# mightymightys/AttosecondRaytracing

Hardware: AMD Instinct MI355X
Metric: ray-surface intersections/s (higher is better)
Workload: dtype f64

## Files before the change

### attosecondraytracing_amd/ModuleProcessing.py

```python
import contextlib
import copy
import lzma
import os
import pickle
from datetime import datetime
from time import perf_counter

import numpy as np
import torch

from . import _abi
from . import _lib
from . import ModuleGeometry as mgeo
from . import ModuleMask as mmask
from . import ModuleOpticalElement as moe
from . import ModuleOpticalRay as mray
from . import ModuleSupport as msupp
from .bundle import RayBundle

DEFAULT_TRACE_MODE = os.environ.get("ART_TRACE_MODE", "chain")


_DESC_CACHE = {}
_DESC_F64_OFFSET = _abi.ArtElementDesc.fwd.offset
assert (_abi.ArtElementDesc.mp.offset - _DESC_F64_OFFSET) == 30 * 8 and _abi.ArtElementDesc.mp.size == 32


def element_descriptor(oe, IgnoreDefects=True, backend=None):
    key = (id(oe), bool(IgnoreDefects))
    h = hash(oe)
    hit = _DESC_CACHE.get(key)
    if hit is not None and hit[0] == h and hit[3] is oe:
        return hit[1], hit[2]
    d, keep = _build_descriptor(oe, IgnoreDefects, backend)
    if len(_DESC_CACHE) > 4096:
        _DESC_CACHE.clear()
    _DESC_CACHE[key] = (h, d, keep, oe)
    return d, keep


def _build_descriptor(oe, IgnoreDefects, backend):
    optic = oe.type
    kind = getattr(optic, "_abi_kind", None)
    tname = getattr(optic, "type", None)
    if kind is None or not isinstance(tname, str) or not ("Mirror" in tname or tname == "Mask"):
        raise NameError("I don`t recognize the type of optical element " + str(tname) + ".")
    d = _abi.ArtElementDesc()
    d.kind = int(kind)
    d.support_kind = int(optic.support._abi_kind)
    fwd, bwd = mgeo.frame_maps(oe.normal, oe.majoraxis)
    buf = np.frombuffer(d, dtype=np.float64, count=34, offset=_DESC_F64_OFFSET)
    buf[0:9] = fwd.reshape(9)
    buf[9:18] = bwd.reshape(9)
    buf[18:21] = oe.position
    buf[21:24] = optic.get_centre()
    sp = optic.support._abi_params()
    buf[24:24 + len(sp)] = sp
    mp_ = optic._abi_params()
    buf[30:30 + len(mp_)] = mp_
    d.nonfinite = bool(d.kind not in (_abi.ART_PLANE, _abi.ART_MASK)
                       and not (np.isfinite(buf[18:24]).all() and np.isfinite(buf[30:34]).all()))
    keep = None
    d.n_defects = 0
    d.n_grid = 0
    d.flags = 0
    d.zern = None
    d.grid = None
    d.grating = None
    if hasattr(optic, "lines_per_mm"):
        d.flags |= _abi.ART_FLAG_GRATING
        d.grating = optic
    if hasattr(optic, "DeformationList") and len(optic.DeformationList) > 0:
        be = backend or _lib.get_backend()
        keep = []
        zern, grids = optic._zernike_defects(), optic._grid_defects()
        if grids and not IgnoreDefects:
            grids[0].get_normal(None)
        if zern:
            table, n_tables, recurrence = optic._abi_defect_table()
            t = be.from_numpy(table)
            keep.append(t)
            d.zern = t.data_ptr()
            d.n_defects = n_tables
            if recurrence:
                d.flags |= _abi.ART_FLAG_ZERN_RECURRENCE
        if grids:
            arr = (_abi.ArtGridDefect * len(grids))()
            rect = np.asarray(optic.support._CircumRect(), dtype=float)
            for g, D in zip(arr, grids):
                half = np.array([max(abs(D._X[0]), abs(D._X[-1])), max(abs(D._Y[0]), abs(D._Y[-1]))])
                if (rect / 2 > half * (1 + 1e-12)).any():
                    raise ValueError(f"One of the requested xi is out of bounds: the mirror support ({rect[0]:g} x "
                                     f"{rect[1]:g} mm) is larger than the Fourrier map ({2 * half[0]:g} x {2 * half[1]:g} mm)")
                fields, dev = D._abi_grid(be)
                keep.append(dev)
                for k_, v_ in fields.items():
                    setattr(g, k_, v_)
            raw = np.frombuffer(bytes(arr), dtype=np.uint8).copy()
            t = be.from_numpy(raw)
            keep.append(t)
            d.grid = t.data_ptr()
            d.n_grid = len(grids)
        if not IgnoreDefects:
            d.flags |= _abi.ART_FLAG_PERTURBED_NORMAL
    return d, keep


def _as_bundle(rays, backend=None):
    if isinstance(rays, RayBundle):
        return rays
    return RayBundle.from_ray_list(rays, backend)


_CHAIN_MAX = 8
_STEPWISE_FLAGS = _abi.ART_FLAG_ZERN_RECURRENCE | _abi.ART_FLAG_GRATING


def _trace_one(be, desc, vin, vout, n, wavelength, grooves):
    if not desc.flags & _abi.ART_FLAG_GRATING:
        be.trace_element(desc, vin, vout, n)
        return grooves
    if wavelength is None:
        raise ValueError("tracing a Grating needs the wavelength of the ray bundle (RayBundle.wavelength is None)")
    G = desc.grating
    out = be.zeros(n)
    be.trace_grating(desc, G._groove_vector(), G.lines_per_mm, G.order, [wavelength], vin, [vout], n, grooves, out)
    return out


def _attach_readout(bundle, detector, path_centre, res):
    res.pop("bundle", None)
    bundle._fused_readout = (detector._readout_key(path_centre), bundle.version, res)


def _attach_sums(bundle, res):
    w = bundle.intensity
    bundle._fused_sums = (bundle.version, None if w is None else (w.data_ptr(), w._version), res)


def RayTracingCalculation(source_rays, optical_elements, IgnoreDefects=True, mode=None, history=True, detector=None,
                          path_centre=0.0, readout_lite=False, sums=False):
    if isinstance(history, str):
        if history != "lazy":
            raise ValueError("history must be True, False or 'lazy'")
        return LazyHistory(source_rays, optical_elements, IgnoreDefects, mode, detector, path_centre)
    src = _as_bundle(source_rays)
    be = src.backend
    n = src.n_slots
    m = len(optical_elements)
    if m == 0:
        return []
    descs, keep = [], []
    for oe in optical_elements:
        d, k = element_descriptor(oe, IgnoreDefects, be)
        descs.append(d)
        keep.append(k)
    mode = mode or DEFAULT_TRACE_MODE
    if any(d.flags & _STEPWISE_FLAGS for d in descs):
        mode = "element"
    bad = next((k for k, d in enumerate(descs) if d.nonfinite), None)
    if bad is not None:
        head = RayTracingCalculation(src, optical_elements[:bad], IgnoreDefects, mode, True) if bad else []
        if len(head[-1] if bad else src) > 0:
            raise np.linalg.LinAlgError("Array must not contain infs or NaNs")
        tail = RayBundle.allocate_many(n, m - bad, head[-1] if bad else src, be)
        prev = head[-1] if bad else src
        for b in tail:
            b.alive.zero_()
            b.parent = prev
            prev = b
        return (head + tail) if history else [None] * (m - 1) + [tail[-1]]
    if history:
        outs = RayBundle.allocate_many(n, m, src, be)
    else:
        outs = [None] * (m - 1) + [RayBundle.allocate(n, like=src, backend=be)]
    prev = src
    for b in outs:
        if b is not None:
            b.parent = prev
            b._keepalive = keep
            prev = b
    if mode == "chain":
        views = [b.view() if b is not None else _abi.ArtBundleView() for b in outs]
        if not history and m > _CHAIN_MAX:
            scratch = [RayBundle.allocate(n, like=src, backend=be) for _ in range(min(2, (m - 1) // _CHAIN_MAX))]
            for j, k in enumerate(range(_CHAIN_MAX - 1, m - 1, _CHAIN_MAX)):
                views[k] = scratch[j % len(scratch)].view()
            outs[-1]._keepalive = (keep, scratch)
        ro = None
        if detector is not None and 0 < n <= be.MAX_FUSED_READOUT_RAYS:
            detector._iscomplete()
            ro = be.new_chain_readout(detector._desc(), src.intensity, n, (0.0, 0.0, path_centre), lite=readout_lite)
        elif sums and detector is None and 0 < n <= be.MAX_FUSED_READOUT_RAYS and hasattr(be, "new_chain_sums"):
            ro = be.new_chain_sums(src.intensity, n)
        be.trace_chain(descs, src.view(), views, n, readout=ro)
        if ro is not None and ro.get("sums"):
            _attach_sums(outs[-1], ro)
        elif ro is not None:
            _attach_readout(outs[-1], detector, path_centre, ro)
    elif mode == "element":
        if not history and m > 1:
            cur = RayBundle.allocate(n, like=src, backend=be)
            g = _trace_one(be, descs[0], src.view(), cur.view(), n, src.wavelength, src.grooves)
            for k in range(1, m - 1):
                g = _trace_one(be, descs[k], cur.view(), cur.view(), n, src.wavelength, g)
            outs[-1].grooves = _trace_one(be, descs[m - 1], cur.view(), outs[-1].view(), n, src.wavelength, g)
        else:
            vin, g = src.view(), src.grooves
            for k in range(m):
                vout = outs[k].view()
                g = outs[k].grooves = _trace_one(be, descs[k], vin, vout, n, src.wavelength, g)
                vin = vout
    else:
        raise ValueError("mode must be 'chain' or 'element'")
    return outs


def RayTracingSpectral(source_rays, optical_elements, grating_index, Wavelengths, detector=None, IgnoreDefects=True):
    wls = [float(w) for w in np.atleast_1d(np.asarray(Wavelengths, dtype=float))]
    if not 1 <= len(wls) <= _abi.ART_GRATING_MAX_WAVELENGTHS:
        raise ValueError(f"Wavelengths: 1 to {_abi.ART_GRATING_MAX_WAVELENGTHS} values")
    if not all(np.isfinite(w) and w > 0 for w in wls):
        raise ValueError("Wavelengths must be finite and positive (mm)")
    src = _as_bundle(source_rays)
    be, n, k = src.backend, src.n_slots, int(grating_index)
    head = RayTracingCalculation(src, optical_elements[:k], IgnoreDefects, history=False)[-1] if k > 0 else src
    desc, _ = element_descriptor(optical_elements[k], IgnoreDefects, be)
    G = desc.grating
    if G is None:
        raise ValueError("RayTracingSpectral: the element at grating_index is no Grating")
    outs = [RayBundle.allocate(n, like=head, backend=be) for _ in wls]
    grooves = be.zeros(len(wls) * n).view(len(wls), n)
    keep = be.trace_grating(desc, G._groove_vector(), G.lines_per_mm, G.order, wls, head.view(), [b.view() for b in outs], n,
                            head.grooves, grooves)
    for j, b in enumerate(outs):
        b.parent, b._keepalive = head, keep
        b.wavelength, b.grooves = wls[j], grooves[j]
    tail = list(optical_elements[k + 1:])
    if not tail:
        return outs
    res = RayTracingCalculationMany(outs, [tail] * len(wls), IgnoreDefects, history=False,
                                    detectors=None if detector is None else [detector] * len(wls))
    return [r[-1] for r in res]


class _ParentResolver:
    __slots__ = ("hist", "bundle", "recipe")

    def __init__(self, hist, bundle):
        import weakref
        self.hist, self.bundle = weakref.ref(hist), weakref.ref(bundle)
        self.recipe = (hist._src, hist._els, hist._opts, hist._want, hist._scene_key)

    def __call__(self):
        h = self.hist()
        if h is None:
            b = self.bundle()
            if b is None:
                return
            src, els, (ign, mode, pc_), want, key = self.recipe
            h = LazyHistory(src, els, ign, mode, None, pc_, want, first=b)
            h._scene_key = key
        h._materialise()


class LazyHistory:

    def __init__(self, source, elements, IgnoreDefects=True, mode=None, detector=None, path_centre=0.0, want=-1, first=None):
        self._src, self._els = _as_bundle(source), list(elements)
        self._scene_key = (_hash_list_of_objects(self._els), hash(self._src))
        self._opts = (bool(IgnoreDefects), mode, path_centre)
        m = len(self._els)
        self._bundles = [None] * m
        self._full = m <= 1
        self.retraces = 0
        if m == 0:
            return
        self._want = want % m
        if first is None:
            first = RayTracingCalculation(self._src, self._els[:self._want + 1], IgnoreDefects, mode, False,
                                          detector if self._want == m - 1 else None, path_centre,
                                          sums=detector is None or self._want != m - 1)[-1]
        self._bundles[self._want] = first
        if not self._full:
            first._parent_resolver = _ParentResolver(self, first)

    def _materialise(self):
        if self._full:
            return
        if (_hash_list_of_objects(self._els), hash(self._src)) != self._scene_key:
            raise RuntimeError("lazy history: an optical element or the source bundle was modified after this history was "
                               "handed out; its remaining bundles can no longer be traced.  Ask for the full history "
                               "(get_output_rays() / history=True) before modifying the chain.")
        self._full = True
        ign, mode, pc_ = self._opts
        full = RayTracingCalculation(self._src, self._els, ign, mode, True, None, pc_)
        self.retraces += 1
        for k, b in enumerate(full):
            have = self._bundles[k]
            if have is None:
                self._bundles[k] = b
            else:
                live = b.alive.bool()
                if not (torch.equal(have.alive, b.alive)
                        and torch.equal(have.data[:, live].view(torch.int64), b.data[:, live].view(torch.int64))):
                    raise RuntimeError("lazy history: the re-trace differs from the bundle handed out earlier")
                have.parent = self._src if k == 0 else self._bundles[k - 1]
        for k in range(1, len(full)):
            if self._bundles[k] is full[k]:
                self._bundles[k].parent = self._bundles[k - 1]

    def __len__(self):
        return len(self._bundles)

    def __getitem__(self, i):
        if isinstance(i, slice):
            self._materialise()
            return self._bundles[i]
        m = len(self._bundles)
        if not -m <= i < m:
            raise IndexError("list index out of range")
        if self._bundles[i % m] is None:
            self._materialise()
        return self._bundles[i % m]

    def __iter__(self):
        self._materialise()
        return iter(self._bundles)

    def __getstate__(self):
        st = dict(self.__dict__)
        for b in st["_bundles"]:
            if b is not None and b._parent_resolver is not None:
                self._materialise()
                return dict(self.__dict__)
        return st


def RayTracingCalculationMany(source_rays_list, optical_elements_list, IgnoreDefects=True, history=True,
                              detectors=None, sums=False):
    with mgeo.frozen_hashes():
        return _RayTracingCalculationMany(source_rays_list, optical_elements_list, IgnoreDefects, history, detectors, sums)


def _RayTracingCalculationMany(source_rays_list, optical_elements_list, IgnoreDefects=True, history=True,
                               detectors=None, sums=False):
    sources = [_as_bundle(s) for s in source_rays_list]
    c = len(sources)
    if c != len(optical_elements_list):
        raise ValueError("need one element list per source bundle")
    if c == 0:
        return []
    m, n, be = len(optical_elements_list[0]), sources[0].n_slots, sources[0].backend
    descs, keep = [], []
    for els in optical_elements_list:
        for oe in els:
            d, k = element_descriptor(oe, IgnoreDefects, be)
            descs.append(d)
            keep.append(k)
    uniform = (m > 0 and n > 0 and all(len(els) == m for els in optical_elements_list)
               and all(s.n_slots == n and s.backend is be for s in sources) and not any(d.nonfinite for d in descs)
               and not any(d.flags & _STEPWISE_FLAGS for d in descs))
    if detectors is not None and len(detectors) != c:
        raise ValueError("need one detector per chain")
    if uniform and c > 1 and detectors is None and len({s.content_key() for s in sources}) == 1 \
            and sources[0].content_key()[0] != "bundle":
        L = 0
        while L < m and all(bytes(descs[ci * m + L]) == bytes(descs[L]) for ci in range(1, c)):
            L += 1
        if L > 0:
            head = RayTracingCalculation(sources[0], optical_elements_list[0][:L], IgnoreDefects, None, history,
                                         sums=sums and L == m)
            if L == m:
                return [list(head) for _ in range(c)]
            tails = RayTracingCalculationMany([head[-1]] * c, [els[L:] for els in optical_elements_list], IgnoreDefects,
                                              history, sums=sums)
            return [list(head) + t for t in tails]
    too_big = history and c * m * n * 65 > 4e9
    if c == 1 or not uniform or too_big:
        return [RayTracingCalculation(s, els, IgnoreDefects, None, history, None if detectors is None else detectors[k],
                                      sums=sums and detectors is None)
                for k, (s, els) in enumerate(zip(sources, optical_elements_list))]
    if history:
        grid = RayBundle.allocate_grid(n, c, m, sources, be)
    else:
        grid = [[None] * (m - 1) + [RayBundle.allocate(n, like=s, backend=be)] for s in sources]
    views, scratch = [], []
    for ci, outs in enumerate(grid):
        prev = sources[ci]
        for k, b in enumerate(outs):
            if b is None and (k + 1) % _CHAIN_MAX == 0:
                b = RayBundle.allocate(n, like=sources[ci], backend=be)
                scratch.append(b)
                views.append(b.view())
                continue
            if b is not None:
                b.parent = prev
                b._keepalive = (keep, scratch)
                prev = b
            views.append(b.view() if b is not None else _abi.ArtBundleView())
    ros = None
    if detectors is not None and n <= be.MAX_FUSED_READOUT_RAYS:
        areas = be.chain_readout_scratch(n, c)
        ros = []
        for d, s_, area in zip(detectors, sources, areas):
            d._iscomplete()
            ros.append(be.new_chain_readout(d._desc(), s_.intensity, n, scratch=area))
    elif sums and detectors is None and n <= be.MAX_FUSED_READOUT_RAYS and hasattr(be, "new_chain_sums"):
        ros = [be.new_chain_sums(s_.intensity, n, scratch=area) for s_, area in zip(sources, be.chain_readout_scratch(n, c))]
    host, dev = be.scene_alloc(c, m, transient=True)
    be.scene_pack(descs, [s.view() for s in sources], views, c, m, host, ros)
    be.scene_upload(host, dev)
    be.trace_scene(dev, host, n, segments=-(-m // 8))
    for ci, outs in enumerate(grid):
        outs[-1]._keepalive = (keep, scratch)
        if ros is not None and ros[ci].get("sums"):
            _attach_sums(outs[-1], ros[ci])
        elif ros is not None:
            _attach_readout(outs[-1], detectors[ci], 0.0, ros[ci])
    return grid


def _placement_source(SourceProperties, FirstOptic):
    from . import ModuleSource as msource

    Divergence = SourceProperties["Divergence"]
    SourceSize = SourceProperties["SourceSize"]
    RayNumber = SourceProperties["NumberRays"]
    Wavelength = SourceProperties["Wavelength"]
    SourcePosition = np.array([0, 0, 0])
    SourceDirection = np.array([1, 0, 0])
    if Divergence == 0:
        if SourceSize == 0:
            S0 = FirstOptic.support
            radius = 0.5 * min(S0.dimX, S0.dimY) if hasattr(S0, "dimX") else S0.radius
        else:
            radius = SourceSize / 2
        SourceRayList = msource.PlaneWaveDisk(SourcePosition, SourceDirection, radius, RayNumber,
                                              Wavelength=Wavelength)
    elif SourceSize == 0:
        SourceRayList = msource.PointSource(SourcePosition, SourceDirection, Divergence, RayNumber,
                                            Wavelength=Wavelength)
    else:
        SourceRayList = msource.ExtendedSource(SourcePosition, SourceDirection, SourceSize, Divergence, RayNumber,
                                               Wavelength=Wavelength)
    Source = msource.ApplyGaussianIntensityToRayList(SourceRayList, 1 / np.e ** 2)
    be = Source.backend
    if hasattr(be, "bundle_sums9") and Source.n_slots > 0:
        _attach_sums(Source, {"sums_dev": be.bundle_sums9(Source)})
    return Source


def _placeChains(SourceProperties, OpticsList, variants, Description):
    from . import ModuleOpticalChain as moc

    c = len(variants)
    Source = _placement_source(SourceProperties, OpticsList[0])
    be = Source.backend
    plain = not any(hasattr(O, "DeformationList") for O in OpticsList)
    guide_ctx = be.side_stream_context("guides") if (plain and hasattr(be, "side_stream_context")) else contextlib.nullcontext()
    with guide_ctx, mgeo.frozen_hashes():
        chains = _placeChainsOn(be, Source, OpticsList, variants, Description, c)
        if plain and hasattr(be, "side_stream_context"):
            torch.cuda.current_stream().synchronize()
    return chains


def _explain_lost_guide(one, element):
    G = element.type
    bare = moe.OpticalElement(G.Mirror, element.position, element.normal, element.majoraxis)
    hit = RayTracingCalculation(one, [bare])[-1]
    if len(hit) == 0:
        return
    u = one.data[3:6, 0].cpu().numpy()
    v = hit.data[3:6, 0].cpu().numpy()
    nrm = (u - v) / np.linalg.norm(u - v)
    fwd, _ = mgeo.frame_maps(element.normal, element.majoraxis)
    qx, qy = G._groove_vector()
    mlN = G.order * one.wavelength * G.lines_per_mm
    g = fwd.T @ (mlN * np.array([qx, qy, 0.0]))
    vt = (u - u.dot(nrm) * nrm) + (g - g.dot(nrm) * nrm)
    raise ValueError(f"Grating: the order m = {G.order} is evanescent for the guide ray at wavelength {one.wavelength:g} mm "
                     f"with {G.lines_per_mm:g} lines/mm: m*lambda*N = {mlN:.6g}, incidence "
                     f"{np.degrees(np.arccos(abs(u.dot(nrm)))):.6g} deg (sin = {np.sqrt(max(0.0, 1 - u.dot(nrm) ** 2)):.6g}), "
                     f"|v_t|^2 = {vt.dot(vt):.6g} > 1, so sqrt(1 - |v_t|^2) does not exist")


def _placeChainsOn(be, Source, OpticsList, variants, Description, c):
    from . import ModuleOpticalChain as moc
    plane_angles = [[np.deg2rad(a % 360) for a in v[2]] for v in variants]
    inc_angles = [[np.deg2rad(a % 360) for a in v[1]] for v in variants]
    centre = [np.array([0, 0, 0]) for _ in range(c)]
    central = [np.array([1, 0, 0]) for _ in range(c)]
    rot_axis = [np.array([0, 1, 0]) for _ in range(c)]
    elements = [[] for _ in range(c)]
    guides = be.from_numpy(np.tile(np.array([0.0, 0.0, 0.0, 1.0, 0.0, 0.0, 0.0, np.nan]), (c, 1)))
    guide_alive = be.from_numpy(np.ones(c, dtype=np.uint8))

    def advance(through, ready):
        descs = [d if d is not None else element_descriptor(oe, True, be)[0] for oe, d in zip(through, ready)]
        if any(d.nonfinite for d in descs):
            raise np.linalg.LinAlgError("Array must not contain infs or NaNs")
        slow = [j for j, d in enumerate(descs) if d.flags & _STEPWISE_FLAGS]
        if not slow:
            be.trace_guides(descs, guides, guide_alive)
            return
        host, al = guides.cpu().numpy(), guide_alive.cpu().numpy()
        for j in range(c):
            if not al[j]:
                continue
            one = RayBundle.from_arrays(host[j, 0:3], host[j, 3:6], wavelength=Source.wavelength, path0=host[j, 6], backend=be)
            out = RayTracingCalculation(one, [through[j]])[-1]
            if len(out) == 0:
                if descs[j].flags & _abi.ART_FLAG_GRATING:
                    _explain_lost_guide(one, through[j])
                al[j] = 0
            else:
                host[j] = out.data[:, 0].cpu().numpy()
        guides.copy_(be.from_numpy(host))
        guide_alive.copy_(be.from_numpy(al))

    optic_copies = [{} for _ in range(c)]
    open_mask = None
    for k, Optic in enumerate(OpticsList):
        if not ("Mirror" in Optic.type or Optic.type == "Mask"):
            raise NameError("I don`t recognize the type of optical element " + Optic.type + ".")
        convex = Optic.type in ("SphericalCX Mirror", "CylindricalCX Mirror")
        shareable = not hasattr(Optic, "DeformationList")
        groups, through, through_descs = {}, [], []
        for j in range(c):
            if convex:
                inc_angles[j][k] = np.pi - inc_angles[j][k]
            dist_ = variants[j][0][k]
            mine = optic_copies[j].get(id(Optic))
            if mine is None:
                mine = optic_copies[j][id(Optic)] = copy.deepcopy(Optic)
            key = (central[j].tobytes(), central[j].dtype.char, rot_axis[j].tobytes(), rot_axis[j].dtype.char, centre[j].tobytes(),
                   centre[j].dtype.char, type(dist_).__name__, float(dist_), plane_angles[j][k], inc_angles[j][k])
            g = groups.get(key)
            if g is None:
                ctr = central[j] * dist_ + centre[j]
                if abs(plane_angles[j][k] - np.pi) < 1e-10:
                    ra = -rot_axis[j]
                else:
                    ra = mgeo.RotationAroundAxis(central[j], -plane_angles[j][k], rot_axis[j])
                normal = mgeo.RotationAroundAxis(ra, -np.pi / 2 + inc_angles[j][k], mgeo._cross3(central[j], ra))
                major = mgeo._cross3(ra, normal)
                element = moe.OpticalElement(mine, ctr, normal, major)
                g = groups[key] = {"ctr": ctr, "ra": ra, "first": element, "desc": None, "guide": None}
                if Optic.type == "Mask":
                    if open_mask is None:
                        open_mask = mmask.Mask(msupp.SupportRoundHole(Radius=100, RadiusHole=100, CenterHoleX=0, CenterHoleY=0))
                    g["guide"] = moe.OpticalElement(open_mask, ctr, normal, major)
                if shareable:
                    d, keep = _build_descriptor(element, True, be)
                    g["desc"] = (hash(element), d, keep)
            else:
                element = moe.OpticalElement._like(g["first"], mine)
            centre[j], rot_axis[j] = g["ctr"], g["ra"]
            elements[j].append(element)
            if g["desc"] is not None:
                h, d, keep = g["desc"]
                if len(_DESC_CACHE) > 4096:
                    _DESC_CACHE.clear()
# ... 231 lines not shown
```

### attosecondraytracing_amd/ModuleSource.py

```python
import numpy as np


from . import _lib
from . import ModuleGeometry as mgeo
from .bundle import RayBundle

_EZ = np.array([0.0, 0.0, 1.0])


def _device_source(kind, size, S, Axis, n, n_total, Wavelength):
    be = _lib.get_backend()
    b = RayBundle.allocate(n, backend=be)
    b.wavelength = Wavelength
    b.number = None
    rot = mgeo.rotation_matrix(_EZ, np.asarray(Axis, dtype=float))
    be.make_source(kind, size, rot, np.asarray(S, dtype=float), 0, n, n_total, b.view())
    b.tag_content(("source", int(kind), float(size), np.asarray(S, dtype=float).tobytes(),
                   np.asarray(Axis, dtype=float).tobytes(), int(n), int(n_total), Wavelength))
    return b


def _Cone(Angle: float, NbRays: int, Wavelength=None):
    return _device_source(0, Angle, np.zeros(3), _EZ, NbRays, NbRays, Wavelength)


def PointSource(S, Axis, Divergence: float, NbRays: int, Wavelength=None):
    return _device_source(0, Divergence, S, Axis, NbRays, NbRays, Wavelength)


def PlaneWaveDisk(Centre, Axis, Radius: float, NbRays: int, Wavelength=None):
    return _device_source(1, Radius, Centre, Axis, NbRays - 1, NbRays, Wavelength)


def ExtendedSource(S, Axis, Diameter: float, Divergence: float, NbRays: int, Wavelength=None):
    n_src = min(max(30, int(250 * Diameter)), int(NbRays / 300))
    per = max(300, int(NbRays / n_src))
    be = _lib.get_backend()
    b = RayBundle.allocate(n_src * per, backend=be)
    b.wavelength = Wavelength
    b.number = None
    rot = mgeo.rotation_matrix(_EZ, np.asarray(Axis, dtype=float))
    be.make_extended_source(Diameter / 2, Divergence, n_src, per, rot, np.asarray(S, dtype=float), 0, n_src * per,
                            b.view())
    b.tag_content(("extended source", float(Diameter), float(Divergence), int(n_src), int(per),
                   np.asarray(S, dtype=float).tobytes(), np.asarray(Axis, dtype=float).tobytes(), Wavelength))
    b.rays_per_source = per
    return b


def PlaneWaveSquare(Centre, Axis, SideLength: float, NbRays: int, Wavelength=None):
    x = np.linspace(-SideLength / 2, SideLength / 2, int(np.sqrt(NbRays)))
    y = np.linspace(-SideLength / 2, SideLength / 2, int(np.sqrt(NbRays)))
    pts = [[0.0, 0.0, 0.0]]
    for i in x:
        for j in y:
            if abs(x) > 1e-4 and abs(y) > 1e-4:
                pts.append([i, j, 0.0])
    pts = np.asarray(pts, dtype=float)
    M = mgeo.rotation_matrix(_EZ, np.asarray(Axis, dtype=float))
    vec = np.tile(M @ _EZ, (len(pts), 1))
    b = RayBundle.from_arrays(pts @ M.T + np.asarray(Centre, dtype=float), vec, np.arange(len(pts)), None, Wavelength)
    return b


def ApplyGaussianIntensityToRayList(RayList, IntensityFraction=1 / np.e ** 2):
    if IntensityFraction >= 1 or IntensityFraction <= 0:
        print("When applying a Gaussian intensity profile to a ray list, the IntensityFraction should be between "
              "0 and 1! I'm setting it to 1/e^2.")
        IntensityFraction = 1 / np.e ** 2
    from . import ModuleProcessing as mp
    B = RayList if isinstance(RayList, RayBundle) else RayBundle.from_ray_list(RayList)
    before = B.content_key()
    if hasattr(B.backend, "gaussian_intensity_central") and B.n_slots > 0:
        B.intensity = B.backend.gaussian_intensity_central(B.view(), IntensityFraction, B.n_slots)
    else:
        axis = mp.FindCentralRay(B).vector
        B.intensity = B.backend.gaussian_intensity(B.view(), axis, IntensityFraction, B.n_slots)
    B.touch()
    if before[0] != "bundle":
        B.tag_content((before, "gaussian intensity", float(IntensityFraction)))
    return B
```

### attosecondraytracing_amd/_abi.py

```python
import ctypes as C

ART_ABI_VERSION = 14

ART_OK = 0
ART_ERR_BAD_ARG = -1
ART_ERR_UNSUPPORTED = -2
ART_ERR_HIP = -3
ART_ERR_NO_DEVICE = -4

ART_PLANE, ART_SPHERE, ART_PARABOLA, ART_TORUS, ART_ELLIPSOID, ART_CYLINDER, ART_MASK = range(7)
ART_SUP_ROUND, ART_SUP_ROUNDHOLE, ART_SUP_RECT, ART_SUP_RECTHOLE, ART_SUP_RECTRECTHOLE = range(5)

ART_FLAG_PERTURBED_NORMAL = 1
ART_FLAG_ZERN_RECURRENCE = 2
ART_FLAG_GRATING = 4
ART_ZERN_RECURRENCE_MAX_ORDER = 64

ART_ZERN_MAX_ORDER = 16
ART_ZERN_DIM = ART_ZERN_MAX_ORDER + 1
ART_ZERN_STRIDE = 2 + 3 * ART_ZERN_DIM * ART_ZERN_DIM
ART_MAX_DEFECTS = 16

c_double_p = C.POINTER(C.c_double)
c_uint8_p = C.POINTER(C.c_uint8)
# ... 120 lines not shown
        ("y0", C.c_double), ("dy", C.c_double),
        ("nx", C.c_int32), ("ny", C.c_int32),
        ("planes", C.c_int32),
        ("reserved", C.c_int32),
        ("shift", C.c_double * ART_FOCAL_MAX_PLANES),
    ]


ART_FOCAL_MAX_WAVENUMBERS = 1024


class ArtFocalSpectrumDesc(C.Structure):
    _fields_ = [
        ("f", ArtFocalDesc),
        ("dk", C.c_double),
        ("nk", C.c_int32),
        ("reserved", C.c_int32),
    ]


class ArtFocalChromaticDesc(C.Structure):
    _fields_ = [
        ("f", ArtFocalDesc),
        ("axis", C.c_double * 3),
        ("nk", C.c_int32),
        ("reserved", C.c_int32),
    ]


ART_WAVEFRONT_MAX_ORDER = 10
ART_WAVEFRONT_MAX_COLS = 68
ART_WAVEFRONT_DOUBLES = 2360


class ArtWavefrontJob(C.Structure):
    _fields_ = [
        ("det", ArtDetectorDesc),
        ("b", ArtBundleView),
        ("w", C.c_void_p),
        ("n", C.c_int64),
        ("ref", C.c_double * 3),
        ("L_ref", C.c_double),
        ("pupil", C.c_double * 3),
        ("order", C.c_int32),
        ("reserved", C.c_int32),
        ("opd", C.c_void_p),
        ("pupil_x", C.c_void_p),
        ("pupil_y", C.c_void_p),
        ("out", C.c_void_p),
    ]


ART_COATING_MAX_LAYERS = 256
ART_COATING_MAX_MATERIALS = 6
ART_POLARISATION_MAX_ELEMS = 64
ART_POLARISATION_DOUBLES = 16


class ArtCoatingMaterial(C.Structure):
    _fields_ = [("n", C.c_double), ("kappa", C.c_double)]


class ArtCoatingLayer(C.Structure):
    _fields_ = [("thickness", C.c_double), ("roughness", C.c_double), ("material", C.c_int32), ("reserved", C.c_int32)]


class ArtCoating(C.Structure):
    _fields_ = [
        ("ideal", C.c_int32),
        ("n_materials", C.c_int32),
        ("n_layers", C.c_int32),
        ("substrate", C.c_int32),
        ("roughness", C.c_double),
        ("reserved", C.c_double),
        ("materials", ArtCoatingMaterial * ART_COATING_MAX_MATERIALS),
        ("layers", ArtCoatingLayer * ART_COATING_MAX_LAYERS),
    ]


class ArtPolarisationJob(C.Structure):
    _fields_ = [
        ("views", C.c_void_p),
        ("coating", C.c_int32 * ART_POLARISATION_MAX_ELEMS),
        ("n_elems", C.c_int32),
        ("polarised", C.c_int32),
        ("n", C.c_int64),
        ("pol", C.c_double * 6),
        ("k", C.c_double),
        ("has_det", C.c_int32),
        ("reserved", C.c_int32),
        ("det", ArtDetectorDesc),
        ("w0", C.c_void_p),
        ("w", C.c_void_p),
        ("w_out", C.c_void_p),
        ("field", C.c_void_p),
        ("out", C.c_void_p),
    ]


ART_FOCAL_VECTOR_SCRATCH_DEFAULT = 1 << 29


class ArtFocalVectorSpectrumDesc(C.Structure):
    _fields_ = [
        ("s", ArtFocalSpectrumDesc),
        ("views", C.c_void_p),
        ("coating", C.c_int32 * ART_POLARISATION_MAX_ELEMS),
        ("n_elems", C.c_int32),
        ("n_coatings", C.c_int32),
        ("n", C.c_int64),
        ("pol", C.c_double * 6),
        ("w", C.c_void_p),
        ("materials", C.c_void_p),
        ("scratch_bound", C.c_int64),
    ]


class ArtFocalVectorChromaticDesc(C.Structure):
    _fields_ = [
        ("v", ArtFocalVectorSpectrumDesc),
        ("axis", C.c_double * 3),
    ]


ART_FOCAL_MAX_GROUPS = 1 << 20


class ArtFocalImageDesc(C.Structure):
    _fields_ = [
        ("f", ArtFocalDesc),
        ("groups", C.c_int32),
        ("reserved", C.c_int32),
        ("seg", C.c_void_p),
    ]


PROTOTYPES = {
    "art_abi_version": (C.c_int, []),
    "art_last_error": (C.c_char_p, []),
    "art_device_count": (C.c_int, []),
    "art_trace_element": (C.c_int, [C.POINTER(ArtElementDesc), C.POINTER(ArtBundleView), C.POINTER(ArtBundleView),
                                    C.c_int64, C.c_void_p]),
    "art_trace_grating": (C.c_int, [C.POINTER(ArtElementDesc), C.POINTER(ArtGratingDesc), c_double_p,
                                    C.POINTER(ArtBundleView), C.POINTER(ArtBundleView), C.c_int64, C.c_void_p]),
    "art_trace_chain": (C.c_int, [C.POINTER(ArtElementDesc), C.c_int32, C.POINTER(ArtBundleView),
                                  C.POINTER(ArtBundleView), C.c_int64, C.c_void_p]),
    "art_scene_bytes": (C.c_int64, [C.c_int32, C.c_int32]),
    "art_chain_readout_scratch_doubles": (C.c_int64, [C.c_int64]),
    "art_trace_chain_readout": (C.c_int, [C.POINTER(ArtElementDesc), C.c_int32, C.POINTER(ArtBundleView),
                                          C.POINTER(ArtBundleView), C.POINTER(ArtChainReadout), C.c_int64, C.c_void_p]),
    "art_scene_pack": (C.c_int, [C.POINTER(ArtElementDesc), C.c_int32, C.c_int32, C.POINTER(ArtBundleView),
                                 C.POINTER(ArtBundleView), C.POINTER(ArtChainReadout), C.c_void_p]),
    "art_trace_scene": (C.c_int, [C.c_void_p, C.c_void_p, C.c_int64, C.c_void_p]),
    "art_pack_rays": (C.c_int, [C.c_void_p, C.c_void_p, C.c_void_p, C.c_int64, C.POINTER(ArtBundleView), C.c_void_p]),
    "art_transform_bundle": (C.c_int, [c_double_p, c_double_p, C.c_int32, C.POINTER(ArtBundleView),
                                       C.POINTER(ArtBundleView), C.c_int64, C.c_void_p]),
    "art_detector": (C.c_int, [C.POINTER(ArtDetectorDesc), C.POINTER(ArtBundleView), C.c_int64, C.c_void_p,
                               C.c_void_p, C.c_void_p, C.c_void_p, C.c_void_p, C.c_void_p, C.c_void_p]),
    "art_detector_readout": (C.c_int, [C.POINTER(ArtDetectorDesc), C.POINTER(ArtBundleView), C.c_void_p, C.c_int64,
                                       C.c_double, C.c_double, C.c_double] + [C.c_void_p] * 9),
    "art_detector_scan_moments": (C.c_int, [C.POINTER(ArtDetectorDesc), C.POINTER(ArtBundleView), C.c_void_p,
                                            C.c_int64, C.c_double, C.c_double, C.c_void_p, C.c_void_p,
                                            C.c_void_p]),
    "art_histogram": (C.c_int, [C.POINTER(ArtHistogramDesc), C.POINTER(ArtBundleView), C.c_void_p, C.c_int64, C.c_int32,
                                C.c_void_p, C.c_void_p, C.c_void_p, C.c_void_p]),
    "art_focal_scratch_doubles": (C.c_int64, [C.c_int32, C.c_int32, C.c_int32, C.c_int64]),
    "art_focal_field": (C.c_int, [C.POINTER(ArtFocalDesc), C.POINTER(ArtBundleView), C.c_void_p, C.c_int64, C.c_void_p,
                                  C.c_void_p, C.c_void_p]),
    "art_focal_spectrum_scratch_doubles": (C.c_int64, [C.c_int32, C.c_int32, C.c_int32, C.c_int32, C.c_int64]),
    "art_focal_spectrum": (C.c_int, [C.POINTER(ArtFocalSpectrumDesc), C.POINTER(ArtBundleView), C.c_void_p, C.c_int64,
                                     C.c_void_p, C.c_void_p, C.c_void_p]),
    "art_focal_chromatic_scratch_doubles": (C.c_int64, [C.c_int32, C.c_int32, C.c_int32, C.c_int32, C.c_int64]),
    "art_focal_chromatic": (C.c_int, [C.POINTER(ArtFocalChromaticDesc), C.POINTER(ArtBundleView), C.POINTER(ArtBundleView),
                                      C.c_void_p, C.c_int64, C.c_void_p, c_double_p, C.c_void_p, C.c_void_p, C.c_void_p]),
    "art_wavefront_scratch_doubles": (C.c_int64, [C.POINTER(ArtWavefrontJob), C.c_int32]),
    "art_wavefront": (C.c_int, [C.c_void_p, C.POINTER(ArtWavefrontJob), C.c_int32, C.c_void_p, C.c_void_p]),
    "art_polarisation_scratch_doubles": (C.c_int64, [C.POINTER(ArtPolarisationJob), C.c_int32]),
    "art_polarisation": (C.c_int, [C.c_void_p, C.POINTER(ArtPolarisationJob), C.c_int32, C.c_void_p,
                                   C.POINTER(ArtCoating), C.c_int32, C.c_void_p, C.c_void_p]),
    "art_focal_vector_spectrum_scratch_doubles": (C.c_int64, [C.POINTER(ArtFocalVectorSpectrumDesc)]),
    "art_focal_vector_spectrum": (C.c_int, [C.POINTER(ArtFocalVectorSpectrumDesc), C.POINTER(ArtBundleView), C.c_void_p,
                                            C.POINTER(ArtCoating), C.POINTER(ArtCoatingMaterial), C.c_void_p,
                                            C.c_void_p, C.c_void_p]),
    "art_focal_vector_chromatic_scratch_doubles": (C.c_int64, [C.POINTER(ArtFocalVectorChromaticDesc)]),
    "art_focal_vector_chromatic": (C.c_int, [C.POINTER(ArtFocalVectorChromaticDesc), C.POINTER(ArtBundleView),
                                             C.POINTER(ArtBundleView), C.c_void_p, C.POINTER(ArtCoating),
                                             C.POINTER(ArtCoatingMaterial), C.c_void_p, c_double_p, C.c_void_p,
                                             C.c_void_p, C.c_void_p]),
    "art_focal_image_scratch_doubles": (C.c_int64, [C.c_int32, C.c_int32, C.c_int32, C.c_int32, C.c_int64]),
    "art_focal_image": (C.c_int, [C.POINTER(ArtFocalImageDesc), C.POINTER(ArtBundleView), C.c_void_p, C.c_int64,
                                  C.c_void_p, C.c_void_p, C.c_void_p]),
    "art_reduce_scratch_doubles": (C.c_int64, []),
    "art_detector_stats": (C.c_int, [C.c_void_p, C.c_void_p, C.c_void_p, C.c_void_p, C.c_void_p, C.c_int64,
                                     C.c_void_p, C.c_void_p, C.c_void_p]),
    "art_detector_moments": (C.c_int, [C.c_void_p, C.c_void_p, C.c_void_p, C.c_void_p, C.c_void_p, C.c_int64,
                                       C.c_double, C.c_double, C.c_double, C.c_void_p, C.c_void_p, C.c_void_p]),
    "art_bundle_sums": (C.c_int, [C.POINTER(ArtBundleView), C.c_void_p, C.c_int64, C.c_void_p, C.c_void_p,
                                  C.c_void_p]),
    "art_gaussian_intensity": (C.c_int, [C.POINTER(ArtBundleView), c_double_p, C.c_double, C.c_int64, C.c_void_p,
                                         C.c_void_p, C.c_void_p]),
    "art_gaussian_intensity_central": (C.c_int, [C.POINTER(ArtBundleView), C.c_double, C.c_int64, C.c_void_p, C.c_void_p,
                                                 C.c_void_p, C.c_void_p]),
    "art_bundle_max_angle": (C.c_int, [C.POINTER(ArtBundleView), c_double_p, C.c_int64, C.c_void_p, C.c_void_p,
                                       C.c_void_p]),
    "art_compact_scratch_ints": (C.c_int64, [C.c_int64]),
    "art_compact": (C.c_int, [C.c_void_p, C.c_int64, C.c_void_p, C.c_void_p, C.c_void_p, C.c_void_p]),
    "art_make_source": (C.c_int, [C.c_int32, C.c_double, c_double_p, c_double_p, C.c_int64, C.c_int64, C.c_int64,
                                  C.POINTER(ArtBundleView), C.c_void_p]),
    "art_make_source_strided": (C.c_int, [C.c_int32, C.c_double, c_double_p, c_double_p, C.c_int64, C.c_int64, C.c_int64,
                                          C.c_int64, C.POINTER(ArtBundleView), C.c_void_p]),
    "art_exchange_pack": (C.c_int, [C.c_void_p] * 6 + [C.c_int64, C.c_void_p, C.c_void_p]),
    "art_exchange_fold": (C.c_int, [C.c_void_p, C.c_int32, C.c_int64, C.c_void_p, C.c_void_p]),
    "art_survivor_bytes": (C.c_int64, [C.c_int64, C.c_int32]),
    "art_pack_survivors": (C.c_int, [C.c_void_p, C.c_int64] + [C.c_void_p] * 4 + [C.c_int64, C.c_int64, C.c_void_p,
                                                                                    C.c_void_p, C.c_int64, C.c_void_p]),
    "art_survivor_finish": (C.c_int, [C.c_void_p, C.c_int64, C.c_void_p, C.c_void_p, C.c_void_p]),
    "art_survivor_xheader": (C.c_int, [C.c_void_p, C.c_void_p, C.c_void_p, C.c_void_p]),
    "art_trace_guides": (C.c_int, [C.POINTER(ArtElementDesc), C.c_int32, C.c_void_p, C.c_void_p, C.c_void_p]),
    "art_analysis_scratch_doubles": (C.c_int64, [C.c_int32, C.c_int64]),
    "art_analyse_bundles": (C.c_int, [C.c_void_p, C.POINTER(ArtAnalysisJob), C.c_int32, C.c_int64, C.c_void_p, C.c_void_p,
                                      C.c_void_p]),
    "art_make_extended_source": (C.c_int, [C.c_double, C.c_double, C.c_int64, C.c_int64, c_double_p, c_double_p,
                                           C.c_int64, C.c_int64, C.POINTER(ArtBundleView), C.c_void_p]),
}


def bind(lib, prefix="art_"):
    fns = {}
    for name, (res, args) in PROTOTYPES.items():
        sym = name if prefix == "art_" else prefix + name[len("art_"):]
        f = getattr(lib, sym)
        f.restype = res
        f.argtypes = args
        fns[name] = f
    return fns
```

### attosecondraytracing_amd/_lib.py

```python
import ctypes as C
import os

import numpy as np
import torch

from . import _abi

_HERE = os.path.dirname(os.path.abspath(__file__))
LIB_PATH = os.path.join(_HERE, "libart_hip.so")

_BACKEND = None


class ArtError(RuntimeError):
    pass


class HipBackend:

    name = "hip"

    def __init__(self, path=LIB_PATH):
        if not os.path.exists(path):
            raise RuntimeError(
                f"{path} not found: the HIP extension has not been built. Run "
                "`python -c 'import __graft_entry__ as g; g.build()'` (needs hipcc). There is no CPU fallback.")
        self.lib = C.CDLL(path)
        self.fn = _abi.bind(self.lib)
        v = self.fn["art_abi_version"]()
        if v != _abi.ART_ABI_VERSION:
            raise RuntimeError(f"libart_hip.so ABI version {v} != expected {_abi.ART_ABI_VERSION}: rebuild it")
        if not torch.cuda.is_available():
            raise RuntimeError("No HIP device visible to PyTorch: ray tracing needs an MI355X (gfx950). "
                               "There is no CPU fallback.")
        n = self.fn["art_device_count"]()
        if n <= 0:
            raise RuntimeError("libart_hip.so found no gfx950 device (art_device_count() = %d: %s)"
                               % (n, self.last_error()))
        self.device = torch.device("cuda", torch.cuda.current_device())
        self._scratch = {}
        self._side_streams = {}
        self._scene_pool, self._scene_uploads = {}, {}
        self._job_pool = {}
        self.count_from, self.counted_launches = None, 0
        self.trace_events = None
        self.readout_events = None

    def last_error(self):
        return self.fn["art_last_error"]().decode("utf-8", "replace")

    def check(self, rc, what):
        if rc != 0:
            raise ArtError(f"{what} failed with code {rc}: {self.last_error()}")

    def stream_ptr(self):
        return C.c_void_p(torch.cuda.current_stream(self.device).cuda_stream)

    def synchronize(self):
        torch.cuda.current_stream(self.device).synchronize()

    def empty(self, n, dtype=torch.float64):
        return torch.empty(int(n), dtype=dtype, device=self.device)

    def zeros(self, n, dtype=torch.float64):
        return torch.zeros(int(n), dtype=dtype, device=self.device)

    def from_numpy(self, a, dtype=None):
        t = torch.from_numpy(np.ascontiguousarray(a))
        if dtype is not None:
            t = t.to(dtype)
        return t.to(self.device)

    def stream_key(self):
        return torch.cuda.current_stream(self.device).cuda_stream

    def side_stream_context(self, name):
        st = self._side_streams.get(name)
        if st is None:
            st = self._side_streams[name] = torch.cuda.Stream(device=self.device)
        return torch.cuda.stream(st)

    def scratch(self, key, n, dtype):
        key = (key, self.stream_key())
        t = self._scratch.get(key)
        if t is None or t.numel() < n or t.dtype != dtype:
            t = torch.empty(int(max(n, 1)), dtype=dtype, device=self.device)
            self._scratch[key] = t
        return t

    def _timed(self, call, sink="trace_events"):
        events = getattr(self, sink)
        if events is None:
            return call()
        e0, e1 = torch.cuda.Event(enable_timing=True), torch.cuda.Event(enable_timing=True)
        e0.record()
        rc = call()
        e1.record()
        events.append((e0, e1))
        return rc

    def trace_element(self, desc, view_in, view_out, n):
        sp = self.stream_ptr()
        self.check(self._timed(lambda: self.fn["art_trace_element"](C.byref(desc), C.byref(view_in),
                                                                    C.byref(view_out), n, sp)), "art_trace_element")

    def trace_grating(self, desc, q, lines_per_mm, order, wavelengths, view_in, views_out, n, grooves_in=None,
                      grooves_out=None):
        nw = len(wavelengths)
        wl_host = (C.c_double * nw)(*[float(w) for w in wavelengths])
        varr = (_abi.ArtBundleView * nw)(*views_out)
        wl_dev = self.from_numpy(np.array([float(w) for w in wavelengths], dtype=np.float64))
        v_dev = self.from_numpy(np.frombuffer(bytes(varr), dtype=np.uint8).copy())
        g = _abi.ArtGratingDesc()
        g.q[0], g.q[1] = float(q[0]), float(q[1])
        g.lines_per_mm, g.order, g.nw = float(lines_per_mm), int(order), nw
        g.wavelengths, g.outs = wl_dev.data_ptr(), v_dev.data_ptr()
        g.grooves_in = None if grooves_in is None else grooves_in.data_ptr()
        g.grooves_out = None if grooves_out is None else grooves_out.data_ptr()
        sp = self.stream_ptr()
        self.check(self._timed(lambda: self.fn["art_trace_grating"](C.byref(desc), C.byref(g), wl_host, varr,
                                                                    C.byref(view_in), n, sp)), "art_trace_grating")
        return wl_dev, v_dev

    def trace_chain(self, descs, view_in, views_out, n, readout=None):
        m = len(descs)
        if m > 1 or readout is not None:
            self.note_launches(n, -(-m // 8))
        darr = (_abi.ArtElementDesc * m)(*descs)
        varr = (_abi.ArtBundleView * m)(*views_out)
        sp = self.stream_ptr()
        if readout is None:
            self.check(self._timed(lambda: self.fn["art_trace_chain"](darr, m, C.byref(view_in), varr, n, sp)),
                       "art_trace_chain")
        else:
            ro = readout["struct"]
            self.check(self._timed(lambda: self.fn["art_trace_chain_readout"](darr, m, C.byref(view_in), varr,
                                                                              C.byref(ro), n, sp)),
                       "art_trace_chain_readout")

    MAX_FUSED_READOUT_RAYS = 1 << 28

    def new_chain_readout(self, ddesc, w, n, centres=(0.0, 0.0, 0.0), store=True, scratch=None, lite=False, targets=None):
        X = Y = opl = None
        if targets is not None:
            X, Y, opl = targets
            assert all(t.numel() >= n and t.dtype == torch.float64 and t.is_contiguous() for t in (X, Y, opl))
            store = True
        elif store:
            X, Y, opl = self.empty(n), self.empty(n), self.empty(n)
        out = self.empty(24)
        if scratch is None:
            scratch = self.scratch("chain_ro", self.fn["art_chain_readout_scratch_doubles"](n), torch.float64)
        ro = _abi.ArtChainReadout()
        ro.det = ddesc
        ro.w = None if w is None else w.data_ptr()
        ro.cx, ro.cy, ro.co = (float(v) for v in centres)
        ro.X, ro.Y, ro.opl = (None, None, None) if not store else (X.data_ptr(), Y.data_ptr(), opl.data_ptr())
        ro.scratch, ro.out24 = scratch.data_ptr(), out.data_ptr()
        ro.lite = 1 if lite else 0
        ro.sums = 0
        return {"struct": ro, "X": X, "Y": Y, "opl": opl, "P3": None, "stats_dev": out, "_keep": (w, scratch), "lite": bool(lite)}

    def new_chain_sums(self, w, n, scratch=None):
        out = self.empty(24)
        if scratch is None:
            scratch = self.scratch("chain_ro", self.fn["art_chain_readout_scratch_doubles"](n), torch.float64)
        ro = _abi.ArtChainReadout()
        ro.w = None if w is None else w.data_ptr()
        ro.X = ro.Y = ro.opl = None
        ro.scratch, ro.out24 = scratch.data_ptr(), out.data_ptr()
        ro.lite, ro.sums = 0, 1
        return {"struct": ro, "sums_dev": out, "_keep": (w, scratch), "sums": True}

    def chain_readout_scratch(self, n, count):
        per = int(self.fn["art_chain_readout_scratch_doubles"](n))
        t = torch.empty(per * count, dtype=torch.float64, device=self.device)
        return [t[k * per:(k + 1) * per] for k in range(count)]

    def scene_alloc(self, n_chains, n_elems, transient=False):
        nb = int(self.fn["art_scene_bytes"](n_chains, n_elems))
        if nb <= 0:
            raise ArtError("art_scene_bytes: bad chain or element count")
        if transient:
            pkey = (nb, self.stream_key())
            pair = self._scene_pool.get(pkey)
            if pair is None:
                pair = self._scene_pool[pkey] = (torch.empty(nb, dtype=torch.uint8, pin_memory=True),
                                                 torch.empty(nb, dtype=torch.uint8, device=self.device))
            ev = self._scene_uploads.pop(pair[0].data_ptr(), None)
            if ev is not None:
                ev.synchronize()
            return pair
        return (torch.empty(nb, dtype=torch.uint8, pin_memory=True),
                torch.empty(nb, dtype=torch.uint8, device=self.device))

    def scene_pack(self, descs, views_in, views_out, n_chains, n_elems, host_image, readouts=None):
        darr = (_abi.ArtElementDesc * (n_chains * n_elems))(*descs)
        iarr = (_abi.ArtBundleView * n_chains)(*views_in)
        oarr = (_abi.ArtBundleView * (n_chains * n_elems))(*views_out)
        rarr = None if readouts is None else (_abi.ArtChainReadout * n_chains)(*[r["struct"] for r in readouts])
        rc = self.fn["art_scene_pack"](darr, n_chains, n_elems, iarr, oarr, rarr, host_image.data_ptr())
        if rc < 0:
            self.check(rc, "art_scene_pack")
        return rc

    def scene_upload(self, host_image, dev_image):
        dev_image.copy_(host_image, non_blocking=True)
        ev = torch.cuda.Event()
        ev.record()
        self._scene_uploads[host_image.data_ptr()] = ev
        return ev

    def note_launches(self, n, k=1):
        if self.count_from is not None and n >= self.count_from:
            self.counted_launches += k

    def trace_scene(self, dev_image, host_image, n, segments=1):
        self.note_launches(n, segments)
        sp = self.stream_ptr()
        self.check(self._timed(lambda: self.fn["art_trace_scene"](dev_image.data_ptr(), host_image.data_ptr(), n, sp)),
                   "art_trace_scene")

    def pack_rays(self, points, vectors, path0, n, view):
        self.check(self.fn["art_pack_rays"](points.data_ptr(), vectors.data_ptr(),
                                            None if path0 is None else path0.data_ptr(), n, C.byref(view),
                                            self.stream_ptr()), "art_pack_rays")

    def transform_bundle(self, M, T, rotate_points, view_in, view_out, n):
        m = (C.c_double * 9)(*[float(v) for v in np.asarray(M).reshape(9)])
        t = (C.c_double * 3)(*[float(v) for v in np.asarray(T).reshape(3)])
        self.check(self.fn["art_transform_bundle"](m, t, int(bool(rotate_points)), C.byref(view_in), C.byref(view_out),
                                                   n, self.stream_ptr()), "art_transform_bundle")

    def detector(self, ddesc, view, n, p3=None, XY=None, opl=None):
        p = [t.data_ptr() for t in p3] if p3 is not None else [None, None, None]
        xy = [t.data_ptr() for t in XY] if XY is not None else [None, None]
        o = opl.data_ptr() if opl is not None else None
        self.check(self.fn["art_detector"](C.byref(ddesc), C.byref(view), n, p[0], p[1], p[2], xy[0], xy[1], o,
                                           self.stream_ptr()), "art_detector")

    def detector_readout(self, ddesc, view, w, n, centres=(0.0, 0.0, 0.0), p3=None, XY=None, opl=None, to_host=True):
        out = self.empty(24)
        p = [t.data_ptr() for t in p3] if (p3 is not None and n > 0) else [None, None, None]
        xy = [t.data_ptr() for t in XY] if (XY is not None and n > 0) else [None, None]
        sp, scratch = self.stream_ptr(), self._red_scratch()
        self.check(self._timed(lambda: self.fn["art_detector_readout"](
            C.byref(ddesc), C.byref(view), None if (w is None or n == 0) else w.data_ptr(), n, float(centres[0]),
            float(centres[1]), float(centres[2]), p[0], p[1], p[2], xy[0], xy[1],
            None if (opl is None or n == 0) else opl.data_ptr(), scratch.data_ptr(), out.data_ptr(), sp),
            "readout_events"), "art_detector_readout")
        return out.cpu().numpy() if to_host else out

    def detector_scan_moments(self, ddesc, view, w, n, co, span=0.0):
        if n == 0:
            return np.zeros(33)
        out = self.empty(33)
        self.check(self.fn["art_detector_scan_moments"](C.byref(ddesc), C.byref(view),
                                                        None if w is None else w.data_ptr(), n, float(co), float(span),
                                                        self._red_scratch().data_ptr(), out.data_ptr(),
                                                        self.stream_ptr()), "art_detector_scan_moments")
        return out.cpu().numpy()

    def histogram(self, hdesc, view, w, n, out=None, shift=None):
        from . import histogram as hist
        if shift is None:
            shift = hist.weight_shift(n, None if w is None else w[:n])
        hdesc.wshift = int(shift)
        if out is None:
            nbins = int(np.prod([hdesc.bins[k] for k in range(max(1, min(3, hdesc.ndim)))]))
            out = (self.empty(nbins, torch.int64), None if w is None else self.empty(nbins, torch.int64),
                   self.empty(4, torch.int64))
            accumulate = 0
        else:
            accumulate = 1
        counts, wsums, totals = out
        self.check(self.fn["art_histogram"](C.byref(hdesc), C.byref(view), None if (w is None or n == 0) else w.data_ptr(),
                                            n, accumulate, counts.data_ptr(), None if wsums is None else wsums.data_ptr(),
                                            totals.data_ptr(), self.stream_ptr()), "art_histogram")
        return counts, wsums, totals, shift

    def focal_field(self, fdesc, view, w, n):
        field = torch.empty((fdesc.planes, fdesc.ny, fdesc.nx), dtype=torch.complex128, device=self.device)
        ns = self.fn["art_focal_scratch_doubles"](fdesc.nx, fdesc.ny, fdesc.planes, n)
        if ns < 0:
            raise ArtError(f"art_focal_scratch_doubles failed with code {ns}: {self.last_error()}")
        scratch = self.scratch("focal", ns, torch.float64)
        self.check(self.fn["art_focal_field"](C.byref(fdesc), C.byref(view), None if (w is None or n == 0) else w.data_ptr(),
                                              n, scratch.data_ptr(), field.data_ptr(), self.stream_ptr()),
                   "art_focal_field")
        return field

    def focal_spectrum(self, sdesc, view, w, n):
        f = sdesc.f
        field = torch.empty((f.planes, sdesc.nk, f.ny, f.nx), dtype=torch.complex128, device=self.device)
        ns = self.fn["art_focal_spectrum_scratch_doubles"](f.nx, f.ny, f.planes, sdesc.nk, n)
        if ns < 0:
            raise ArtError(f"art_focal_spectrum_scratch_doubles failed with code {ns}: {self.last_error()}")
        scratch = self.scratch("focal", ns, torch.float64)
        self.check(self.fn["art_focal_spectrum"](C.byref(sdesc), C.byref(view), None if (w is None or n == 0) else
                                                 w.data_ptr(), n, scratch.data_ptr(), field.data_ptr(),
                                                 self.stream_ptr()), "art_focal_spectrum")
        return field

    def focal_chromatic(self, desc, final_view, source_view, w, n, table):
        table = np.ascontiguousarray(table, dtype=np.float64)
        if table.ndim != 2 or table.shape[1] != 4:
            raise ValueError("the chromatic table must have rows (k_j, c_j, z_j, 0)")
        f = desc.f
        desc.nk = nk = int(table.shape[0])
        ns = self.fn["art_focal_chromatic_scratch_doubles"](f.nx, f.ny, f.planes, nk, n)
        if ns < 0:
            raise ArtError(f"art_focal_chromatic_scratch_doubles failed with code {ns}: {self.last_error()}")
        field = torch.empty((f.planes, nk, f.ny, f.nx), dtype=torch.complex128, device=self.device)
        scratch = self.scratch("focal", ns, torch.float64)
        table_dev = self.from_numpy(table)
        self.check(self.fn["art_focal_chromatic"](C.byref(desc), C.byref(final_view), C.byref(source_view),
                                                  None if (w is None or n == 0) else w.data_ptr(), n,
                                                  table_dev.data_ptr(), table.ctypes.data_as(_abi.c_double_p),
                                                  scratch.data_ptr(), field.data_ptr(), self.stream_ptr()),
                   "art_focal_chromatic")
        return field

    def focal_image(self, fdesc, seg, groups, view, w, n):
        d = _abi.ArtFocalImageDesc()
        d.f = fdesc
        d.groups = int(groups)
        d.seg = seg.data_ptr()
        image = torch.empty((fdesc.planes, fdesc.ny, fdesc.nx), dtype=torch.float64, device=self.device)
        ns = self.fn["art_focal_image_scratch_doubles"](fdesc.nx, fdesc.ny, fdesc.planes, d.groups, n)
        if ns < 0:
            raise ArtError(f"art_focal_image_scratch_doubles failed with code {ns}: {self.last_error()}")
        scratch = self.scratch("focal", ns, torch.float64)
        self.check(self.fn["art_focal_image"](C.byref(d), C.byref(view), None if (w is None or n == 0) else w.data_ptr(),
                                              n, scratch.data_ptr(), image.data_ptr(), self.stream_ptr()),
                   "art_focal_image")
        return image

    def _red_scratch(self):
        return self.scratch("red", self.fn["art_reduce_scratch_doubles"](), torch.float64)

    def detector_stats(self, alive, X, Y, opl, w, n, to_host=True):
        out = self.empty(16)
        ptr = lambda t: None if (t is None or n == 0) else t.data_ptr()
        if n == 0:
            alive = self.zeros(1, torch.uint8)
        self.check(self.fn["art_detector_stats"](alive.data_ptr(), ptr(X), ptr(Y), ptr(opl), ptr(w), n,
                                                 self._red_scratch().data_ptr(), out.data_ptr(), self.stream_ptr()),
                   "art_detector_stats")
        return out.cpu().numpy() if to_host else out

    def detector_moments(self, alive, X, Y, opl, w, n, cx, cy, co):
        if n == 0:
            return np.zeros(8)
        out = self.empty(8)
        ptr = lambda t: None if t is None else t.data_ptr()
        self.check(self.fn["art_detector_moments"](alive.data_ptr(), ptr(X), ptr(Y), ptr(opl), ptr(w), n,
                                                   float(cx), float(cy), float(co), self._red_scratch().data_ptr(),
                                                   out.data_ptr(), self.stream_ptr()), "art_detector_moments")
        return out.cpu().numpy()

    def bundle_sums(self, view, w, n):
        if n == 0:
            return np.zeros(8)
        out = self.empty(8)
        self.check(self.fn["art_bundle_sums"](C.byref(view), None if w is None else w.data_ptr(), n,
                                              self._red_scratch().data_ptr(), out.data_ptr(), self.stream_ptr()),
                   "art_bundle_sums")
        return out.cpu().numpy()

    def gaussian_intensity(self, view, axis, fraction, n):
        w = self.empty(n)
        a = (C.c_double * 3)(*[float(v) for v in axis])
        self.check(self.fn["art_gaussian_intensity"](C.byref(view), a, float(fraction), n,
                                                     self._red_scratch().data_ptr(), w.data_ptr(), self.stream_ptr()),
                   "art_gaussian_intensity")
        return w

    def gaussian_intensity_central(self, view, fraction, n):
        w = self.empty(n)
        sums8 = self.empty(8)
        self.check(self.fn["art_gaussian_intensity_central"](C.byref(view), float(fraction), n, self._red_scratch().data_ptr(),
                                                             sums8.data_ptr(), w.data_ptr(), self.stream_ptr()),
                   "art_gaussian_intensity_central")
        return w

    def bundle_max_angle(self, view, axis, n):
        if n == 0:
            return 0.0, 0.0
        out = self.empty(2)
        a = (C.c_double * 3)(*[float(v) for v in axis])
        self.check(self.fn["art_bundle_max_angle"](C.byref(view), a, n, self._red_scratch().data_ptr(),
                                                   out.data_ptr(), self.stream_ptr()), "art_bundle_max_angle")
        o = out.cpu().numpy()
        return float(o[0]), float(o[1])

    def compact(self, alive, n):
        if n == 0:
            return torch.empty(0, dtype=torch.int64, device=self.device), 0
        ints = self.fn["art_compact_scratch_ints"](n)
        sc = self.scratch("compact", ints, torch.int32)
        idx = torch.empty(int(max(n, 1)), dtype=torch.int64, device=self.device)
        cnt = torch.zeros(1, dtype=torch.int64, device=self.device)
        self.check(self.fn["art_compact"](alive.data_ptr(), n, sc.data_ptr(), idx.data_ptr(), cnt.data_ptr(),
                                          self.stream_ptr()), "art_compact")
        c = int(cnt.cpu().item())
        return idx[:c], c

    def make_source(self, kind, size, rot, S, first, n, n_total, view, step=1):
        r = (C.c_double * 9)(*[float(v) for v in np.asarray(rot).reshape(9)])
        s = (C.c_double * 3)(*[float(v) for v in np.asarray(S).reshape(3)])
        self.check(self.fn["art_make_source_strided"](kind, float(size), r, s, first, int(step), n, n_total, C.byref(view),
                                                      self.stream_ptr()), "art_make_source_strided")

    def exchange_pack(self, stats, X, Y, opl, alive, slots, send):
        k = int(slots.numel())
        self.check(self.fn["art_exchange_pack"](stats.data_ptr(), X.data_ptr(), Y.data_ptr(), opl.data_ptr(),
                                                alive.data_ptr(), slots.data_ptr(), k, send.data_ptr(),
                                                self.stream_ptr()), "art_exchange_pack")

    def exchange_fold(self, recv, world, stride, out):
        self.check(self.fn["art_exchange_fold"](recv.data_ptr(), int(world), int(stride), out.data_ptr(),
                                                self.stream_ptr()), "art_exchange_fold")

    def survivor_bytes(self, count, dense=False):
        return int(self.fn["art_survivor_bytes"](int(count), 1 if dense else 0))

    def pack_survivors(self, alive, X, Y, opl, number, first, step, send):
        n = int(alive.numel())
        sc = self.scratch("compact", self.fn["art_compact_scratch_ints"](n), torch.int32)
        ptr = lambda t: None if (t is None or n == 0) else t.data_ptr()
        self.check(self.fn["art_pack_survivors"](ptr(alive), n, ptr(X), ptr(Y), ptr(opl), ptr(number), int(first),
                                                 int(step), sc.data_ptr(), send.data_ptr(), int(send.numel()),
                                                 self.stream_ptr()), "art_pack_survivors")

    def survivor_finish(self, stats_dev, n, send, xhdr=None):
        self.check(self.fn["art_survivor_finish"](stats_dev.data_ptr(), int(n), send.data_ptr(),
                                                  None if xhdr is None else xhdr.data_ptr(), self.stream_ptr()),
                   "art_survivor_finish")

    def survivor_xheader(self, send, stats_dev, xhdr):
        self.check(self.fn["art_survivor_xheader"](send.data_ptr(), None if stats_dev is None else stats_dev.data_ptr(),
                                                   xhdr.data_ptr(), self.stream_ptr()), "art_survivor_xheader")

    def trace_guides(self, descs, rays, alive):
        count = len(descs)
        sp = self.stream_ptr()
        for k0 in range(0, count, _abi.ART_GUIDES_MAX):
            m = min(_abi.ART_GUIDES_MAX, count - k0)
            darr = (_abi.ArtElementDesc * m)(*descs[k0:k0 + m])
            self.check(self.fn["art_trace_guides"](darr, m, rays.data_ptr() + 64 * k0, alive.data_ptr() + k0, sp),
                       "art_trace_guides")

    def _upload_table(self, arr, purpose=None):
        nb = C.sizeof(arr)
        pkey = (nb, self.stream_key()) if purpose is None else (purpose, nb, self.stream_key())
        pair = self._job_pool.get(pkey)
        if pair is None:
            pair = self._job_pool[pkey] = [torch.empty(nb, dtype=torch.uint8, pin_memory=True),
                                           torch.empty(nb, dtype=torch.uint8, device=self.device), None]
        host, dev, ev = pair
        if ev is not None:
            ev.synchronize()
        C.memmove(host.data_ptr(), C.addressof(arr), nb)
        dev.copy_(host, non_blocking=True)
        pair[2] = torch.cuda.Event()
        pair[2].record()
        return dev

    def wavefront(self, jobs):
        c = len(jobs)
        out = torch.empty((c, _abi.ART_WAVEFRONT_DOUBLES), dtype=torch.float64, device=self.device)
        for k, j in enumerate(jobs):
            j.out = out.data_ptr() + 8 * _abi.ART_WAVEFRONT_DOUBLES * k
        arr = (_abi.ArtWavefrontJob * c)(*jobs)
        ns = self.fn["art_wavefront_scratch_doubles"](arr, c)
        if ns < 0:
            raise ArtError(f"art_wavefront_scratch_doubles failed with code {ns}: {self.last_error()}")
        dev = self._upload_table(arr)
        scratch = self.scratch("wavefront", ns, torch.float64)
        self.check(self.fn["art_wavefront"](dev.data_ptr(), arr, c, scratch.data_ptr(), self.stream_ptr()), "art_wavefront")
        return out

    def polarisation(self, jobs, views, coatings):
        c = len(jobs)
        out = torch.empty((c, _abi.ART_POLARISATION_DOUBLES), dtype=torch.float64, device=self.device)
        blob = b"".join(bytes(v) for v in views) + b"".join(bytes(k) for k in coatings)
        dev = self._upload_table((C.c_char * len(blob)).from_buffer_copy(blob), "polarisation views")
        off = 0
        jarr = (_abi.ArtPolarisationJob * c)()
        for k, (j, v) in enumerate(zip(jobs, views)):
            jarr[k] = j
            jarr[k].views = dev.data_ptr() + off
            jarr[k].out = out.data_ptr() + 8 * _abi.ART_POLARISATION_DOUBLES * k
            off += C.sizeof(v)
        carr = (_abi.ArtCoating * max(len(coatings), 1))(*coatings)
        cdev = dev.data_ptr() + off if coatings else None
        ns = self.fn["art_polarisation_scratch_doubles"](jarr, c)
        if ns < 0:
            raise ArtError(f"art_polarisation_scratch_doubles failed with code {ns}: {self.last_error()}")
        jdev = self._upload_table(jarr)
        scratch = self.scratch("polarisation", ns, torch.float64)
        self.check(self.fn["art_polarisation"](jdev.data_ptr(), jarr, c, cdev, carr, len(coatings), scratch.data_ptr(),
                                               self.stream_ptr()), "art_polarisation")
        return out

    def focal_vector_tables(self, vdesc, views, coatings, materials):
        nk, nc = vdesc.s.nk, len(coatings)
        mats = np.ascontiguousarray(materials, dtype=np.float64)
        if mats.shape != (nk, nc, _abi.ART_COATING_MAX_MATERIALS, 2):
            raise ValueError(f"materials must be [nk, coatings, {_abi.ART_COATING_MAX_MATERIALS}, 2]")
        blob = bytes(views) + b"".join(bytes(k) for k in coatings) + mats.tobytes()
        dev = self._upload_table((C.c_char * len(blob)).from_buffer_copy(blob), "focal vector spectrum")
        vdesc.views = dev.data_ptr()
        vdesc.n_coatings = nc
        cdev = dev.data_ptr() + C.sizeof(views) if nc else None
        vdesc.materials = dev.data_ptr() + C.sizeof(views) + nc * C.sizeof(_abi.ArtCoating) if nc else None
        carr = (_abi.ArtCoating * max(nc, 1))(*coatings)
        marr = (_abi.ArtCoatingMaterial * max(mats.size // 2, 1)).from_buffer_copy(mats.tobytes() or bytes(16))
        return cdev, carr, marr

    def focal_vector_spectrum(self, vdesc, views, coatings, materials):
        f = vdesc.s.f
        field = torch.empty((f.planes, vdesc.s.nk, 3, f.ny, f.nx), dtype=torch.complex128, device=self.device)
        cdev, carr, marr = self.focal_vector_tables(vdesc, views, coatings, materials)
        ns = self.fn["art_focal_vector_spectrum_scratch_doubles"](C.byref(vdesc))
        if ns < 0:
            raise ArtError(f"art_focal_vector_spectrum_scratch_doubles failed with code {ns}: {self.last_error()}")
        scratch = self.scratch("focal vector", ns, torch.float64)
        self.check(self.fn["art_focal_vector_spectrum"](C.byref(vdesc), C.byref(views[vdesc.n_elems]), cdev, carr, marr,
                                                        scratch.data_ptr(), field.data_ptr(), self.stream_ptr()),
                   "art_focal_vector_spectrum")
        return field

    def focal_vector_chromatic(self, vcdesc, views, coatings, materials, table):
        table = np.ascontiguousarray(table, dtype=np.float64)
        if table.ndim != 2 or table.shape[1] != 4:
            raise ValueError("the chromatic table must have rows (k_j, c_j, z_j, 0)")
        v = vcdesc.v
        v.s.nk = nk = int(table.shape[0])
        f = v.s.f
        cdev, carr, marr = self.focal_vector_tables(v, views, coatings, materials)
        ns = self.fn["art_focal_vector_chromatic_scratch_doubles"](C.byref(vcdesc))
        if ns < 0:
            raise ArtError(f"art_focal_vector_chromatic_scratch_doubles failed with code {ns}: {self.last_error()}")
        field = torch.empty((f.planes, nk, 3, f.ny, f.nx), dtype=torch.complex128, device=self.device)
        scratch = self.scratch("focal vector", ns, torch.float64)
        table_dev = self.from_numpy(table)
        self.check(self.fn["art_focal_vector_chromatic"](C.byref(vcdesc), C.byref(views[v.n_elems]), C.byref(views[0]),
                                                         cdev, carr, marr, table_dev.data_ptr(),
                                                         table.ctypes.data_as(_abi.c_double_p), scratch.data_ptr(),
                                                         field.data_ptr(), self.stream_ptr()),
                   "art_focal_vector_chromatic")
        return field

    def analyse_bundles(self, jobs, n):
        c = len(jobs)
        arr = (_abi.ArtAnalysisJob * c)(*jobs)
        dev = self._upload_table(arr)
        out = torch.empty((c, _abi.ART_ANALYSIS_DOUBLES), dtype=torch.float64, device=self.device)
        scratch = self.scratch("analysis", self.fn["art_analysis_scratch_doubles"](c, int(n)), torch.float64)
        self.check(self.fn["art_analyse_bundles"](dev.data_ptr(), arr, c, int(n), scratch.data_ptr(), out.data_ptr(),
                                                  self.stream_ptr()), "art_analyse_bundles")
        return out

    def bundle_sums9(self, bundle):
        j = _abi.ArtAnalysisJob()
        j.b = bundle.view()
        j.w = None if bundle.intensity is None else bundle.intensity.data_ptr()
        j.mode = _abi.ART_JOB_SUMS
        return self.analyse_bundles([j], bundle.n_slots)[0]

    def make_extended_source(self, radius, divergence, n_points, per, rot, S, first, n, view):
        r = (C.c_double * 9)(*[float(v) for v in np.asarray(rot).reshape(9)])
        s = (C.c_double * 3)(*[float(v) for v in np.asarray(S).reshape(3)])
        self.check(self.fn["art_make_extended_source"](float(radius), float(divergence), int(n_points), int(per), r, s,
                                                       first, n, C.byref(view), self.stream_ptr()),
                   "art_make_extended_source")


def get_backend():
    global _BACKEND
    if _BACKEND is None:
        _BACKEND = HipBackend()
    return _BACKEND
```

### attosecondraytracing_amd/bundle.py

```python

import os

import numpy as np
import torch

from . import _abi
from . import _lib
from .ModuleOpticalRay import Ray

import itertools

ROW_OX, ROW_OY, ROW_OZ, ROW_DX, ROW_DY, ROW_DZ, ROW_PATH, ROW_INC = range(8)
_SERIAL = itertools.count(1)


class RayBundle:
    def __init__(self, data, alive, number=None, intensity=None, wavelength=None, parent=None, backend=None, grooves=None):
        self.data = data
        self.alive = alive
        self.number = number
        self.intensity = intensity
        self.wavelength = wavelength
        self.grooves = grooves
        self._parent = parent
        self._parent_resolver = None
        self._backend = backend or _lib.get_backend()
        self._index = None
        self._count = None
        self.version = 0
        self._serial = next(_SERIAL)
        self.path_head = None
        self._fused_readout = None
        self._fused_sums = None
        self._content = None

    @property
    def parent(self):
        if self._parent_resolver is not None:
            resolve, self._parent_resolver = self._parent_resolver, None
            resolve()
        return self._parent

    @parent.setter
    def parent(self, value):
        self._parent = value
        self._parent_resolver = None

    def fused_sums(self):
        fs = getattr(self, "_fused_sums", None)
        if fs is None or fs[0] != self.version:
            return None
        w = self.intensity
        if (None if w is None else (w.data_ptr(), w._version)) != fs[1]:
            return None
        return fs[2]["sums_dev"]

    def _share_parent(self, other):
        if self._parent_resolver is not None:
            import weakref
            wo = weakref.ref(other)

            def resolve(s=self, wo=wo):
                o = wo()
                if o is not None:
                    o._parent = s.parent
            other._parent_resolver = resolve

    @property
    def backend(self):
        if self._backend is None:
            be = _lib.get_backend()
            data, alive = self._rows(self.alive.numel(), be.device)
            data.copy_(self.data)
            alive.copy_(self.alive)
            self.data, self.alive = data, alive
            self.number = None if self.number is None else self.number.to(be.device)
            self.intensity = None if self.intensity is None else self.intensity.to(be.device)
            self.grooves = None if self.grooves is None else self.grooves.to(be.device)
            self._backend = be
        return self._backend

    def __getstate__(self):
        host = lambda t: None if t is None else t.detach().cpu().numpy()
        return {"data": host(self.data), "alive": host(self.alive), "number": host(self.number),
                "intensity": host(self.intensity), "wavelength": self.wavelength, "parent": self.parent,
                "version": self.version, "path_head": self.path_head, "grooves": host(self.grooves)}

    def __setstate__(self, st):
        t = lambda a: None if a is None else torch.from_numpy(np.ascontiguousarray(a))
        self.data, self.alive = t(st["data"]), t(st["alive"])
        self.number, self.intensity = t(st["number"]), t(st["intensity"])
        self._parent_resolver = None
        self.wavelength, self.parent, self.version = st["wavelength"], st["parent"], st["version"]
        self.path_head = st.get("path_head")
        self.grooves = t(st.get("grooves"))
        self._backend = None
        self._index = None
        self._count = None
        self._fused_readout = None
        self._fused_sums = None
        self._content = None
        self._serial = next(_SERIAL)

    @staticmethod
    def _pitch(n, unit=64):
        return max(unit, -(-int(n) // unit) * unit) + unit * int(os.environ.get("ART_PITCH_EXTRA", "0"))

    @classmethod
    def _rows(cls, n, device, count=None):
        n = int(n)
        pd, pa = cls._pitch(n), cls._pitch(n, 512)
        if count is None:
            return (torch.empty((8, pd), dtype=torch.float64, device=device)[:, :n],
                    torch.empty(pa, dtype=torch.uint8, device=device)[:n])
        lead = tuple(count) if isinstance(count, (tuple, list)) else (count,)
        return (torch.empty(lead + (8, pd), dtype=torch.float64, device=device)[..., :n],
                torch.empty(lead + (pa,), dtype=torch.uint8, device=device)[..., :n])

    @classmethod
    def allocate(cls, n, like=None, backend=None):
        be = backend or (like.backend if like is not None else _lib.get_backend())
        data, alive = cls._rows(n, be.device)
        if like is not None:
            return cls(data, alive, like.number, like.intensity, like.wavelength, like, be, like.grooves)
        return cls(data, alive, backend=be)

    @classmethod
    def allocate_many(cls, n, count, like, backend=None):
        be = backend or like.backend
        data, alive = cls._rows(n, be.device, count)
        return [cls(data[k], alive[k], like.number, like.intensity, like.wavelength, like, be, like.grooves)
                for k in range(count)]

    @classmethod
    def allocate_grid(cls, n, chains, count, likes, backend=None):
        be = backend or likes[0].backend
        data, alive = cls._rows(n, be.device, (chains, count))
        return [[cls(data[c, k], alive[c, k], likes[c].number, likes[c].intensity, likes[c].wavelength, likes[c], be,
                     likes[c].grooves)
                 for k in range(count)] for c in range(chains)]

    @classmethod
    def from_arrays(cls, point, vector, number=None, intensity=None, wavelength=None, path0=None, backend=None):
        be = backend or _lib.get_backend()
        point = np.ascontiguousarray(point, dtype=np.float64).reshape(-1, 3)
        vector = np.ascontiguousarray(vector, dtype=np.float64).reshape(-1, 3)
        n = point.shape[0]
        b = cls.allocate(n, backend=be)
        if n > 0:
            p0 = None
            if path0 is not None:
                p0 = be.from_numpy(np.broadcast_to(np.asarray(path0, dtype=np.float64), (n,)).copy())
            be.pack_rays(be.from_numpy(point), be.from_numpy(vector), p0, n, b.view())
        b.number = None if number is None else be.from_numpy(np.asarray(number, dtype=np.int64))
        b.intensity = None if intensity is None else be.from_numpy(np.asarray(intensity, dtype=np.float64))
        b.wavelength = wavelength
        return b

    @classmethod
    def from_ray_list(cls, rays, backend=None):
        rays = list(rays)
        pts = np.array([r.point for r in rays], dtype=np.float64).reshape(-1, 3)
        vec = np.array([r.vector for r in rays], dtype=np.float64).reshape(-1, 3)
        nums = [r.number for r in rays]
        number = None if any(v is None for v in nums) else np.array(nums, dtype=np.int64)
        ints = [r.intensity for r in rays]
        intensity = None if any(v is None for v in ints) else np.array(ints, dtype=np.float64)
        path0 = np.array([float(np.sum(r.path)) for r in rays])
        wl = rays[0].wavelength if rays else None
        b = cls.from_arrays(pts, vec, number, intensity, wl, path0, backend)
        k = {len(r.path) for r in rays}
        if len(k) == 1 and k != {1}:
            b.path_head = np.array([r.path for r in rays], dtype=np.float64)
        return b

    def _share_grouping(self, other):
        if hasattr(self, "rays_per_source"):
            other.rays_per_source = self.rays_per_source

    @property
    def n_slots(self):
        return int(self.alive.numel())

    def view(self):
        p = self.data.data_ptr()
        stride = self.data.stride(0) * 8
        v = _abi.ArtBundleView()
        v.ox, v.oy, v.oz = p, p + stride, p + 2 * stride
        v.dx, v.dy, v.dz = p + 3 * stride, p + 4 * stride, p + 5 * stride
        v.path, v.incidence = p + 6 * stride, p + 7 * stride
        v.alive = self.alive.data_ptr()
        return v

    def phase_path_view(self, wavelength=None):
        v = self.view()
        if self.grooves is None:
            return v, None
        wavelength = self.wavelength if wavelength is None else wavelength
        if wavelength is None:
            raise ValueError("a bundle that crossed a grating needs a wavelength for a coherent analysis")
        eff = torch.add(self.data[ROW_PATH], self.grooves, alpha=float(wavelength)).contiguous()
        v.path = eff.data_ptr()
        return v, eff

    def phase_ref_offset(self, wavelength=None):
        if self.grooves is None:
            return 0.0
        wavelength = self.wavelength if wavelength is None else wavelength
        alive = self.alive != 0
        cnt = int(alive.sum())
        if cnt == 0 or wavelength is None:
            return 0.0
        return float(wavelength) * float(torch.where(alive, self.grooves, 0.0).sum()) / cnt

    def slots(self, lo, hi):
        lo, hi = int(lo), int(hi)
        cut = lambda t: None if t is None else t[lo:hi]
        out = RayBundle(self.data[:, lo:hi], self.alive[lo:hi], cut(self.number), cut(self.intensity), self.wavelength, None,
                        self._backend, cut(self.grooves))
        if self.number is None and lo != 0:
            out.number = torch.arange(lo, hi, dtype=torch.int64, device=self.alive.device)
        return out

    def tag_content(self, key):
        self._content = (key, self.version)

    def content_key(self):
        if self._content is not None and self._content[1] == self.version:
            return self._content[0]
        return ("bundle", self._serial, self.version)

    def touch(self):
        self.version += 1
        self._index = None
        self._count = None

    def index(self):
        if self._index is None:
            self._index, self._count = self.backend.compact(self.alive, self.n_slots)
        return self._index

    def __len__(self):
        if self._count is None:
            self.index()
        return self._count

    def _gather(self, row):
        return self.data[row].index_select(0, self.index()).cpu().numpy()

    def points(self):
        idx = self.index()
        return self.data[0:3].index_select(1, idx).cpu().numpy().T.copy()

    def vectors(self):
        idx = self.index()
        return self.data[3:6].index_select(1, idx).cpu().numpy().T.copy()

    def paths_total(self):
        return self._gather(ROW_PATH)

    def incidences(self):
        return self._gather(ROW_INC)

    def numbers(self):
        idx = self.index()
        if self.number is None:
            return idx.cpu().numpy()
        return self.number.index_select(0, idx).cpu().numpy()

    def intensities(self):
        if self.intensity is None:
            return None
        return self.intensity.index_select(0, self.index()).cpu().numpy()

    def path_segments(self):
        idx = self.index()
        cum = []
        b = self
        while b is not None:
            b.backend
            cum.append(b.data[ROW_PATH].index_select(0, idx).cpu().numpy())
            b = b.parent
        cum = cum[::-1]
        head = self._head_segments(idx.cpu().numpy())
        segs = (list(head.T) if head is not None else [cum[0]]) + [cum[j] - cum[j - 1] for j in range(1, len(cum))]
        return np.stack(segs, axis=1)

    def _head_segments(self, slots):
        b = self
        while b.parent is not None:
            b = b.parent
        return None if b.path_head is None else b.path_head[slots]

    def _ray_at(self, slots):
        slots = np.atleast_1d(np.asarray(slots, dtype=np.int64))
        st = torch.from_numpy(slots).to(self.backend.device)
        cols = self.data.index_select(1, st).cpu().numpy()
        nums = slots if self.number is None else self.number.index_select(0, st).cpu().numpy()
        ints = None if self.intensity is None else self.intensity.index_select(0, st).cpu().numpy()
        cum = []
        b = self
        while b is not None:
            b.backend
            cum.append(b.data[ROW_PATH].index_select(0, st).cpu().numpy())
            b = b.parent
        cum = cum[::-1]
        head = self._head_segments(slots)
        rays = []
        for j in range(len(slots)):
            first = (float(cum[0][j]),) if head is None else tuple(float(v) for v in head[j])
            path = first + tuple(float(cum[k][j] - cum[k - 1][j]) for k in range(1, len(cum)))
            inc = cols[ROW_INC, j]
            rays.append(Ray(cols[0:3, j].copy(), cols[3:6, j].copy(), path, int(nums[j]), self.wavelength,
                            None if np.isnan(inc) else np.float64(inc),
                            None if ints is None else np.float64(ints[j])))
        return rays

    def __getitem__(self, i):
        idx = self.index()
        if isinstance(i, slice):
            sel = idx[i].cpu().numpy()
            return self._ray_at(sel) if len(sel) else []
        m = len(self)
        if i < 0:
            i += m
        if not 0 <= i < m:
            raise IndexError("list index out of range")
        return self._ray_at([int(idx[i].item())])[0]

    def __iter__(self):
        idx = self.index().cpu().numpy()
        for lo in range(0, len(idx), 4096):
            for r in self._ray_at(idx[lo:lo + 4096]):
                yield r

    def subset(self, positions):
        idx = self.index()
        pos = torch.as_tensor(np.asarray(positions, dtype=np.int64), device=self.backend.device)
        alive = torch.zeros_like(self.alive)
        alive[idx.index_select(0, pos)] = 1
        out = RayBundle(self.data, alive, self.number, self.intensity, self.wavelength, self._parent, self.backend, self.grooves)
        self._share_parent(out)
        out.path_head = self.path_head
        self._share_grouping(out)
        return out

    def transformed(self, M, T, rotate_points=True):
        out = RayBundle.allocate(self.n_slots, like=self, backend=self.backend)
        out._parent = self._parent
        self._share_parent(out)
        out.path_head = self.path_head
        self._share_grouping(out)
        self.backend.transform_bundle(M, T, rotate_points, self.view(), out.view(), self.n_slots)
        return out

    def copy(self):
        data, alive = self._rows(self.n_slots, self.data.device)
        data.copy_(self.data)
        alive.copy_(self.alive)
        out = RayBundle(data, alive, self.number, self.intensity, self.wavelength, self._parent, self.backend, self.grooves)
        self._share_parent(out)
        out.path_head = self.path_head
        self._share_grouping(out)
        out.tag_content(self.content_key())
        return out

    def alias(self):
        out = RayBundle(self.data, self.alive, self.number, self.intensity, self.wavelength, self._parent, self.backend,
                        self.grooves)
        self._share_parent(out)
        out.path_head = self.path_head
        self._share_grouping(out)
        out.tag_content(self.content_key())
        hit = getattr(self, "_sum_w", None)
        if hit is not None and hit[0] == self.version:
            out._sum_w = (out.version, hit[1])
        fs = self._fused_sums
        if fs is not None and fs[0] == self.version:
            out._fused_sums = (out.version, fs[1], fs[2])
        return out

    def __deepcopy__(self, memo):
        return self.copy()

    def __hash__(self):
        return hash((self._serial, self.version))
```

### attosecondraytracing_amd/csrc/art_kernels.hip

```cpp
#include <hip/hip_runtime.h>

#include <math.h>
#include <stdio.h>
#include <stdlib.h>
#include <string.h>
#include <type_traits>

#include "art_device.h"
#include "art_coating.h"
#include "art_scene.h"

#if defined(ART_ZERN_LDS) && !defined(ART_STORE_DIRECT)
#define ART_STORE_DIRECT 1
#endif

namespace {

constexpr int kBlock = 256;
constexpr int kMaxBlocks = 256 * 8;
constexpr int kReadoutBlocks = kMaxBlocks;

thread_local char g_err[512] = "";

int fail(int code, const char* msg) {
// ... 403 lines not shown
    double v = s[0];
    for (int j = 1; j < (int)((B ? B : blockDim.x) >> 6); ++j) v = fold_op(v, s[j], op_k);
    *out = v;
  }
}

template <int NS, int kU, int (*OP)(int)>
__global__ __launch_bounds__(kBlock) void k_fold_partials(const double* scratch, const int nblocks, double* out) {
  fold_range<kU, kBlock>(scratch + blockIdx.x, 0, nblocks, OP(blockIdx.x), out + blockIdx.x, NS);
}

__device__ __forceinline__ void readout_accumulate(double (&acc)[kReadoutSlots], const bool live, const double x,
                                                   const double y, const double o, const double wi, const bool has_w,
                                                   const double cx, const double cy, const double co) {
  const double ww = live ? (has_w ? wi : 1.0) : 0.0, one = live ? 1.0 : 0.0;
  const double xs = live ? x : 0.0, ys = live ? y : 0.0, os = live ? o : 0.0;
  acc[0] += one; acc[1] += os;
  acc[2] = fmin(acc[2], live ? x : INFINITY); acc[3] = fmax(acc[3], live ? x : -INFINITY);
  acc[4] = fmin(acc[4], live ? y : INFINITY); acc[5] = fmax(acc[5], live ? y : -INFINITY);
  acc[6] += xs; acc[7] += ys;
  acc[8] += ww; acc[9] = fma(ww, xs, acc[9]); acc[10] = fma(ww, ys, acc[10]); acc[11] = fma(ww, os, acc[11]);
  acc[12] = fmin(acc[12], live ? o : INFINITY); acc[13] = fmax(acc[13], live ? o : -INFINITY);
  const double ex = live ? x - cx : 0.0, ey = live ? y - cy : 0.0, eo = live ? o - co : 0.0;
  acc[16] = fma(ex, ex, acc[16]); acc[17] = fma(ey, ey, acc[17]); acc[18] = fma(eo, eo, acc[18]);
  acc[19] = fma(ww * ex, ex, acc[19]); acc[20] = fma(ww * ey, ey, acc[20]); acc[21] = fma(ww * eo, eo, acc[21]);
}
__device__ __forceinline__ void readout_single(double (&acc)[kReadoutSlots], const bool live, const double x,
                                               const double y, const double o, const double wi, const bool has_w,
                                               const double cx, const double cy, const double co) {
  const double ww = live ? (has_w ? wi : 1.0) : 0.0;
  const double xs = live ? x : 0.0, ys = live ? y : 0.0, os = live ? o : 0.0;
  acc[0] = live ? 1.0 : 0.0; acc[1] = os;
  acc[2] = live ? x : INFINITY; acc[3] = live ? x : -INFINITY;
  acc[4] = live ? y : INFINITY; acc[5] = live ? y : -INFINITY;
  acc[6] = xs; acc[7] = ys;
  acc[8] = ww; acc[9] = ww * xs; acc[10] = ww * ys; acc[11] = ww * os;
  acc[12] = live ? o : INFINITY; acc[13] = live ? o : -INFINITY;
  acc[14] = 0.0; acc[15] = 0.0;
  const double ex = live ? x - cx : 0.0, ey = live ? y - cy : 0.0, eo = live ? o - co : 0.0;
  acc[16] = ex * ex; acc[17] = ey * ey; acc[18] = eo * eo;
  acc[19] = ww * ex * ex; acc[20] = ww * ey * ey; acc[21] = ww * eo * eo;
  acc[22] = 0.0; acc[23] = 0.0;
}
__device__ __forceinline__ void readout_single_lite(double (&acc)[kReadoutSlots], const bool live, const double x,
                                                    const double y, const double o) {
  acc[0] = live ? 1.0 : 0.0; acc[1] = live ? o : 0.0;
  acc[2] = live ? x : INFINITY; acc[3] = live ? x : -INFINITY;
  acc[4] = live ? y : INFINITY; acc[5] = live ? y : -INFINITY;
  acc[12] = live ? o : INFINITY; acc[13] = live ? o : -INFINITY;
}
__device__ __forceinline__ void readout_accumulate_lite(double (&acc)[kReadoutSlots], const bool live, const double x,
                                                        const double y, const double o) {
  acc[0] += live ? 1.0 : 0.0; acc[1] += live ? o : 0.0;
  acc[2] = fmin(acc[2], live ? x : INFINITY); acc[3] = fmax(acc[3], live ? x : -INFINITY);
  acc[4] = fmin(acc[4], live ? y : INFINITY); acc[5] = fmax(acc[5], live ? y : -INFINITY);
  acc[12] = fmin(acc[12], live ? o : INFINITY); acc[13] = fmax(acc[13], live ? o : -INFINITY);
}

struct ElemArg {
  ArtElementDesc e[1];
};

#ifdef ART_ZERN_LDS
constexpr bool kDefectLoop = true;
__device__ __forceinline__ void stage_tables(const double* src, double* dst, int doubles) {
  for (int j = threadIdx.x; j < doubles; j += kBlock) dst[j] = src[j];
}
#else
constexpr bool kDefectLoop = false;
#endif

template <int KIND, bool DEFECT>
__global__ __launch_bounds__(kBlock) void k_trace_element(const ElemArg ea, const ArtBundleView in,
                                                          const ArtBundleView out, const int64_t n, const int xmap) {
  const ArtElementDesc& e = ea.e[blockIdx.y];
  const double* zern = e.zern;
#ifdef ART_ZERN_LDS
  __shared__ double s_zern[DEFECT ? 4 * ART_ZERN_STRIDE : 2];
  if (DEFECT) {
    stage_tables(e.zern, s_zern, e.n_defects * ART_ZERN_STRIDE);
    __syncthreads();
    zern = s_zern;
  }
#endif
  const BundleRsrc bi = make_rsrc(in, n), bo = make_rsrc(out, n);
  const int64_t stride = (int64_t)gridDim.x * kBlock;
  int64_t i = tile_of(blockIdx.x, gridDim.x, xmap) * kBlock + threadIdx.x;
  do {
    art::Ray r;
    r.inc = 0.0;
    uint8_t a;
    load_slot(bi, i, r, a);
    bool ok = a != 0;
#ifdef ART_DIAG_NOCOMPUTE
    r.path += e.mp[0];
#else
    if (ok) ok = art::trace_ray<KIND, DEFECT>(e, zern, r);
#endif
    store_slot(bo, i, r, ok);
    i += stride;
  } while (DEFECT && kDefectLoop && i < n);
}

__global__ __launch_bounds__(kBlock) void k_trace_element_zrec(const ElemArg ea, const ArtBundleView in,
                                                               const ArtBundleView out, const int64_t n) {
  const ArtElementDesc& e = ea.e[blockIdx.y];
  const BundleRsrc bi = make_rsrc(in, n), bo = make_rsrc(out, n);
  const int64_t i = (int64_t)blockIdx.x * kBlock + threadIdx.x;
  art::Ray r;
  r.inc = 0.0;
  uint8_t a;
  load_slot(bi, i, r, a);
  bool ok = a != 0;
  if (ok) ok = art::trace_ray<ART_KIND_DYN, true, true>(e, e.zern, r);
  store_slot(bo, i, r, ok);
}

__global__ __launch_bounds__(kBlock) void k_trace_grating(const ElemArg ea, const ArtGratingDesc g, const ArtBundleView in,
                                                          const int64_t n) {
  const ArtElementDesc& e = ea.e[blockIdx.y];
  const BundleRsrc bi = make_rsrc(in, n);
  const int64_t i = (int64_t)blockIdx.x * kBlock + threadIdx.x;
  const unsigned o8 = (unsigned)i * 8u, nb8 = (unsigned)(n * 8);
  art::Ray r;
  r.inc = 0.0;
  uint8_t a;
  load_slot(bi, i, r, a);
  const double g_in = ld_f64(rsrc_of(g.grooves_in, g.grooves_in ? nb8 : 0u), o8);
  art::GratingHit h = {};
  bool hit = a != 0;
  if (hit) hit = art::grating_hit<ART_KIND_DYN>(e, r, g.q[0], g.q[1], g.lines_per_mm, h);
  const double g_out = g_in + (double)g.order * h.G;
  const art::zuni_t wl = ART_ZUNI(g.wavelengths);
  typedef const uint64_t __attribute__((address_space(4)))* uview_t;
  const uview_t vp = (uview_t)(const void*)g.outs;
  static_assert(sizeof(ArtBundleView) == 9 * sizeof(uint64_t), "ArtBundleView is nine pointers");
  for (int j = 0; j < g.nw; ++j) {
    const double sc = (double)g.order * wl[j] * g.lines_per_mm;
    ArtBundleView v;
    v.ox = (double*)vp[9 * j + 0]; v.oy = (double*)vp[9 * j + 1]; v.oz = (double*)vp[9 * j + 2];
    v.dx = (double*)vp[9 * j + 3]; v.dy = (double*)vp[9 * j + 4]; v.dz = (double*)vp[9 * j + 5];
    v.path = (double*)vp[9 * j + 6]; v.incidence = (double*)vp[9 * j + 7]; v.alive = (uint8_t*)vp[9 * j + 8];
    art::Ray o;
    const bool ok = art::grating_diffract(e, h, sc * g.q[0], sc * g.q[1], r.path, o) && hit;
    store_slot(make_rsrc(v, n), i, o, ok);
    double* go = g.grooves_out ? g.grooves_out + (int64_t)j * n : nullptr;
    st_f64(rsrc_of(go, go ? nb8 : 0u), ok ? o8 : kDropOffset, g_out);
  }
}

using art::ChainArgs;
using art::kChainMax;

#ifndef ART_STORE_DIRECT
__device__ __forceinline__ void store_tile_lds4(const ArtBundleView& v, const int64_t n, const int64_t first,
                                                const int64_t tile0, const unsigned t, const art::Ray& r, const bool ok,
                                                double (*s_out)[kBlock], uint8_t* s_al) {
  s_out[0][t] = r.ox; s_out[1][t] = r.oy; s_out[2][t] = r.oz;
  s_out[3][t] = r.dx; s_out[4][t] = r.dy; s_out[5][t] = r.dz;
  s_out[6][t] = r.path; s_out[7][t] = r.inc;
  s_al[t] = (uint8_t)(ok ? 1 : 0);
  const unsigned nb = (unsigned)(v.alive != nullptr ? n : 0);
  __builtin_amdgcn_raw_buffer_store_b8((uint8_t)(ok ? 1 : 0), rsrc_of(v.alive + first, nb), (int)(unsigned)(tile0 + t), 0,
                                       ART_ST_AUX);
  __syncthreads();
  const int w = __builtin_amdgcn_readfirstlane((int)(t >> 6)), l = (int)(t & 63);
  double* const* rows = &v.ox;
  bool keep[2];
#pragma unroll
  for (int h = 0; h < 2; ++h) keep[h] = (s_al[h * 128 + 2 * l] | s_al[h * 128 + 2 * l + 1]) != 0;
#pragma unroll
  for (int js = 0; js < 2; ++js) {
    const int j = 2 * w + js;
    const __amdgpu_buffer_rsrc_t rs = rsrc_of(rows[j] + first, nb * 8u);
#pragma unroll
    for (int h = 0; h < 2; ++h) {
      const int s0 = h * 128 + 2 * l;
      st_2f64(rs, keep[h] ? (unsigned)(tile0 + s0) * 8u : kDropOffset, s_out[j][s0], s_out[j][s0 + 1]);
    }
  }
  __syncthreads();
}
#endif

__device__ __forceinline__ void tail_partial(const ChainArgs& a, const double tot[3], double (*s_part)[kReadoutSlots],
                                             const unsigned lane, const unsigned bx, const unsigned nbx) {
  if ((lane & 7) == 0) {
    const int stat = (lane & 63) >> 3, w = lane >> 6;
    s_part[w][stat] = tot[0];
    s_part[w][8 + stat] = tot[1];
    if (stat < 6) s_part[w][16 + stat] = tot[2];
  }
  asm volatile("s_waitcnt lgkmcnt(0)\n\ts_barrier" ::: "memory");
#ifdef ART_DIAG_RO_NOSCRATCH
  if (tot[0] + tot[1] + tot[2] == -1.2345e300) {
#else
  if (lane < kUsedSlots) {
#endif
    double v = s_part[0][lane];
#pragma unroll
    for (int j = 1; j < kBlock / 64; ++j) {
      const double q = s_part[j][lane];
      v = (lane < 16) ? v + q : (lane < 19 ? fmin(v, q) : fmax(v, q));
    }
    a.ro.scratch[(int64_t)lane * nbx + bx] = v;
  }
}

template <bool DEFECT, int KIND1 = ART_KIND_DYN>
__device__ __forceinline__ void chain_body(const ChainArgs& a, const int64_t first, const int64_t n, const int xmap,
                                           double* s_zern, const unsigned bx, const unsigned nbx, const bool keep_in = false) {
#ifdef ART_ZERN_LDS
  if (DEFECT) {
    int off = 0;
    for (int k = 0; k < a.n_elems; ++k) {
      stage_tables(a.e[k].zern, s_zern + off, a.e[k].n_defects * ART_ZERN_STRIDE);
      off += a.e[k].n_defects * ART_ZERN_STRIDE;
    }
    __syncthreads();
  }
#endif
  __shared__ double s_w[kBlock];
  __shared__ __attribute__((aligned(16))) double s_red[(kBlock / 64) * 8 * kTileStride];
#ifndef ART_STORE_DIRECT
  double (*s_out)[kBlock] = reinterpret_cast<double (*)[kBlock]>(s_red);
  static_assert(sizeof(double) * 8 * kBlock <= sizeof(double) * (kBlock / 64) * 8 * kTileStride, "staging tile fits");
  __shared__ uint8_t s_al[kBlock];
#endif
  __shared__ double s_part[kBlock / 64][kReadoutSlots];
  const int64_t tile = tile_of(bx, nbx, xmap);
  const BundleRsrc bi = make_rsrc(a.in, n, first);
  const int64_t stride = (int64_t)nbx * kBlock;
  int64_t i0 = tile * kBlock + threadIdx.x;
  do {
    unsigned slot = (unsigned)i0;
    asm volatile("" : "+v"(slot));
    const int64_t i = slot;
    const unsigned lane = slot & (kBlock - 1);
    art::Ray r;
    r.inc = 0.0;
    uint8_t al;
    if (keep_in) load_slot_keep(bi, i, r, al);
    else load_slot(bi, i, r, al);
    s_w[lane] = ld_f64(rsrc_of(const_cast<double*>(a.ro.w) + first,
                                      ((a.flags & art::kFlagReadout) && a.ro.w && !a.ro.lite) ? (unsigned)(n * 8) : 0u),
                       (unsigned)i * 8u);
    bool ok = al != 0;
    const double* zk = s_zern;
    int k = 0;
    do {
#ifdef ART_DIAG_NOCOMPUTE
      r.path += a.e[k].mp[0];
#else
#ifdef ART_ZERN_LDS
      if (ok) ok = art::trace_ray_dyn<DEFECT>(a.e[k], zk, r);
      zk += a.e[k].n_defects * ART_ZERN_STRIDE;
#else
      if (KIND1 != ART_KIND_DYN) {
        if (ok) ok = art::trace_ray<(KIND1 < 0 ? 0 : KIND1), DEFECT>(a.e[0], a.e[0].zern, r);
      } else {
        if (ok) ok = art::trace_ray_dyn<DEFECT>(a.e[k], a.e[k].zern, r);
      }
#endif
#endif
#ifndef ART_STORE_DIRECT
      store_tile_lds4(a.out[k], n, first, (int64_t)(slot - lane), lane, r, ok, s_out, s_al);
#else
      store_slot(make_rsrc(a.out[k], a.out[k].alive != nullptr ? n : 0, first), i, r, ok);
#endif
    } while (KIND1 == ART_KIND_DYN && ++k < a.n_elems);
    if (a.flags & art::kFlagReadout) {
      if (a.ro.sums) {
        double v[8];
        sums_values(v, ok, r, a.ro.w ? s_w[lane ^ ((unsigned)a.flags >> 30)] : 1.0);
        const double tot = run_sums8(v, s_red + (lane >> 6) * (8 * kTileStride), lane & 63);
        tile_sums_store(tot, __ballot(ok), &s_part[0][0], lane, a.ro.scratch, (n + kBlock - 1) / kBlock, tile);
      } else {
      double acc[kReadoutSlots];
      double Ix, Iy, Iz, x = 0.0, y = 0.0, o = 0.0;
      if (ok) art::detector_ray(a.ro.det, r, Ix, Iy, Iz, x, y, o);
      const unsigned nb8 = (unsigned)(n * 8);
      const unsigned o8 = ok ? (unsigned)i * 8u : kDropOffset;
#ifndef ART_DIAG_RO_NOXYO
      st_f64(rsrc_of(a.ro.X + first, a.ro.X ? nb8 : 0u), o8, x);
      st_f64(rsrc_of(a.ro.Y + first, a.ro.Y ? nb8 : 0u), o8, y);
      st_f64(rsrc_of(a.ro.opl + first, a.ro.opl ? nb8 : 0u), o8, o);
#endif
      double tot[3];
      if (a.ro.lite) {
        readout_single_lite(acc, ok, x, y, o);
        wave_reduce_lite(acc, s_red + (lane >> 6) * (8 * kTileStride), lane & 63, tot);
      } else {
      readout_single(acc, ok, x, y, o, s_w[lane ^ ((unsigned)a.flags >> 30)], a.ro.w != nullptr, a.ro.cx, a.ro.cy,
                     a.ro.co);
#ifdef ART_DIAG_RO_NOREDUCE
      tot[0] = acc[0] + acc[1] + acc[6] + acc[7] + acc[8] + acc[9] + acc[10] + acc[11];
      tot[1] = acc[16] + acc[17] + acc[18] + acc[19] + acc[20] + acc[21];
      tot[2] = acc[2] + acc[3] + acc[4] + acc[5] + acc[12] + acc[13];
#else
      wave_reduce24(acc, s_red + (lane >> 6) * (8 * kTileStride), lane & 63, tot);
#endif
      }
      tail_partial(a, tot, s_part, lane, bx, nbx);
      }
    }
    i0 += stride;
  } while (DEFECT && kDefectLoop && i0 < n);
}

template <bool DEFECT>
__device__ __forceinline__ void chain_body2(const ChainArgs& a, const int64_t first, const int64_t n, const int xmap,
                                            const unsigned bx, const unsigned nbx, const bool keep_in = false) {
  __shared__ double s_w[2][kBlock];
  __shared__ __attribute__((aligned(16))) double s_red[(kBlock / 64) * 8 * kTileStride];
  __shared__ double s_part[kBlock / 64][kReadoutSlots];
  const int64_t tile = tile_of(bx, nbx, xmap);
  const BundleRsrc bi = make_rsrc(a.in, n, first);
  unsigned pair = (unsigned)(tile * kBlock + threadIdx.x);
  asm volatile("" : "+v"(pair));
  const unsigned lane = pair & (kBlock - 1);
  const unsigned o16 = pair * 16u, o2 = pair * 2u;
  art::Ray r[2];
  bool ok[2];
  {
    D2 ox, oy, oz, dx, dy, dz, pa;
    if (keep_in) {
      ox = ld_2f64_keep(bi.ox, o16); oy = ld_2f64_keep(bi.oy, o16); oz = ld_2f64_keep(bi.oz, o16);
      dx = ld_2f64_keep(bi.dx, o16); dy = ld_2f64_keep(bi.dy, o16); dz = ld_2f64_keep(bi.dz, o16);
      pa = ld_2f64_keep(bi.path, o16);
    } else {
      ox = ld_2f64(bi.ox, o16); oy = ld_2f64(bi.oy, o16); oz = ld_2f64(bi.oz, o16);
      dx = ld_2f64(bi.dx, o16); dy = ld_2f64(bi.dy, o16); dz = ld_2f64(bi.dz, o16);
      pa = ld_2f64(bi.path, o16);
    }
    unsigned al2 = __builtin_amdgcn_raw_buffer_load_b16(bi.alive, (int)o2, 0, ART_LD_AUX);
    if (n & 1) al2 |= __builtin_amdgcn_raw_buffer_load_b8(bi.alive, (o2 + 1u == (unsigned)n) ? (int)o2 : (int)kDropOffset, 0, ART_LD_AUX);
    ok[0] = (al2 & 0xffu) != 0;
    ok[1] = (al2 & 0xff00u) != 0;
    const D2 wv = ld_2f64(rsrc_of(const_cast<double*>(a.ro.w) + first,
                                  ((a.flags & art::kFlagReadout) && a.ro.w && !a.ro.lite) ? (unsigned)(n * 8) : 0u), o16);
    s_w[0][lane] = wv.a; s_w[1][lane] = wv.b;
    r[0].ox = ox.a; r[0].oy = oy.a; r[0].oz = oz.a; r[0].dx = dx.a; r[0].dy = dy.a; r[0].dz = dz.a; r[0].path = pa.a;
    r[1].ox = ox.b; r[1].oy = oy.b; r[1].oz = oz.b; r[1].dx = dx.b; r[1].dy = dy.b; r[1].dz = dz.b; r[1].path = pa.b;
    r[0].inc = 0.0; r[1].inc = 0.0;
  }
  int k = 0;
  do {
#pragma unroll
    for (int h = 0; h < 2; ++h)
      if (ok[h]) ok[h] = art::trace_ray_dyn<DEFECT>(a.e[k], a.e[k].zern, r[h]);
    const ArtBundleView& v = a.out[k];
    const unsigned nb = (unsigned)(v.alive != nullptr ? n : 0);
    const unsigned off = (ok[0] || ok[1]) ? o16 : kDropOffset;
    st_2f64(rsrc_of(v.ox + first, nb * 8u), off, r[0].ox, r[1].ox);
    st_2f64(rsrc_of(v.oy + first, nb * 8u), off, r[0].oy, r[1].oy);
    st_2f64(rsrc_of(v.oz + first, nb * 8u), off, r[0].oz, r[1].oz);
    st_2f64(rsrc_of(v.dx + first, nb * 8u), off, r[0].dx, r[1].dx);
    st_2f64(rsrc_of(v.dy + first, nb * 8u), off, r[0].dy, r[1].dy);
    st_2f64(rsrc_of(v.dz + first, nb * 8u), off, r[0].dz, r[1].dz);
    st_2f64(rsrc_of(v.path + first, nb * 8u), off, r[0].path, r[1].path);
    st_2f64(rsrc_of(v.incidence + first, nb * 8u), off, r[0].inc, r[1].inc);
    const __amdgpu_buffer_rsrc_t ra = rsrc_of(v.alive + first, nb);
    __builtin_amdgcn_raw_buffer_store_b16((unsigned short)((ok[0] ? 1u : 0u) | (ok[1] ? 0x100u : 0u)), ra, (int)o2, 0, ART_ST_AUX);
    if (n & 1)
      __builtin_amdgcn_raw_buffer_store_b8((uint8_t)(ok[0] ? 1 : 0), ra, (o2 + 1u == (unsigned)n) ? (int)o2 : (int)kDropOffset, 0, ART_ST_AUX);
  } while (++k < a.n_elems);
  if ((a.flags & art::kFlagReadout) && a.ro.sums) {
    const unsigned li = lane ^ ((unsigned)a.flags >> 30);
    double v0[8], v1[8], totA, totB;
    sums_values(v0, ok[0], r[0], a.ro.w ? s_w[0][li] : 1.0);
    sums_values(v1, ok[1], r[1], a.ro.w ? s_w[1][li] : 1.0);
    run_sums8_pairs(v0, v1, s_red + (lane >> 6) * (8 * kTileStride), lane & 63, totA, totB);
    static_assert(sizeof(s_part) >= sizeof(double) * 8 * kSumRows, "eight runs fit the partial area");
    tile_sums_store_pairs(totA, totB, __ballot(ok[0]), __ballot(ok[1]), &s_part[0][0], lane, a.ro.scratch,
                          (n + kBlock - 1) / kBlock, tile);
  } else if (a.flags & art::kFlagReadout) {
    double acc[kReadoutSlots];
    double Ix, Iy, Iz, x[2] = {0.0, 0.0}, y[2] = {0.0, 0.0}, o[2] = {0.0, 0.0};
#pragma unroll
    for (int h = 0; h < 2; ++h)
      if (ok[h]) art::detector_ray(a.ro.det, r[h], Ix, Iy, Iz, x[h], y[h], o[h]);
    const unsigned nb8 = (unsigned)(n * 8);
    const unsigned off = (ok[0] || ok[1]) ? o16 : kDropOffset;
    st_2f64(rsrc_of(a.ro.X + first, a.ro.X ? nb8 : 0u), off, x[0], x[1]);
    st_2f64(rsrc_of(a.ro.Y + first, a.ro.Y ? nb8 : 0u), off, y[0], y[1]);
    st_2f64(rsrc_of(a.ro.opl + first, a.ro.opl ? nb8 : 0u), off, o[0], o[1]);
    const unsigned li = lane ^ ((unsigned)a.flags >> 30);
    double tot[3];
    if (a.ro.lite) {
      readout_single_lite(acc, ok[0], x[0], y[0], o[0]);
      readout_accumulate_lite(acc, ok[1], x[1], y[1], o[1]);
      wave_reduce_lite(acc, s_red + (lane >> 6) * (8 * kTileStride), lane & 63, tot);
    } else {
      readout_single(acc, ok[0], x[0], y[0], o[0], s_w[0][li], a.ro.w != nullptr, a.ro.cx, a.ro.cy, a.ro.co);
      readout_accumulate(acc, ok[1], x[1], y[1], o[1], s_w[1][li], a.ro.w != nullptr, a.ro.cx, a.ro.cy, a.ro.co);
      wave_reduce24(acc, s_red + (lane >> 6) * (8 * kTileStride), lane & 63, tot);
    }
    tail_partial(a, tot, s_part, lane, bx, nbx);
  }
}

constexpr int kFoldChunks = 64;
constexpr int64_t kFoldDirect = 65536;
__device__ __forceinline__ double* fold_mid(double* scratch, const int64_t nparts) {
  return scratch + (int64_t)kReadoutSlots * nparts;
}
__device__ __forceinline__ int fold_row_of(const int slot) {
  int row = 0;
#pragma unroll
  for (int k = 0; k < kUsedSlots; ++k) row = (slot == k) ? row_of_slot(k) : row;
  return row;
}
__device__ __forceinline__ void fold_stage1(double* scratch, const int64_t nparts) {
  if (blockIdx.x >= kUsedSlots) return;
  const int64_t per = (nparts + kFoldChunks - 1) / kFoldChunks;
  const int64_t lo = (int64_t)blockIdx.y * per, hi = (lo + per < nparts) ? lo + per : nparts;
  fold_range(scratch + (int64_t)fold_row_of(blockIdx.x) * nparts, lo, hi, stat_op(blockIdx.x),
             fold_mid(scratch, nparts) + blockIdx.x * kFoldChunks + blockIdx.y);
}
__device__ __forceinline__ void fold_stage2(double* scratch, const int64_t nparts, double* out24, const int direct) {
  if (blockIdx.x >= kUsedSlots) {
    if (threadIdx.x == 0) out24[blockIdx.x] = 0.0;
    return;
  }
  if (direct) {
    fold_range(scratch + (int64_t)fold_row_of(blockIdx.x) * nparts, 0, nparts, stat_op(blockIdx.x), out24 + blockIdx.x);
    return;
  }
  fold_range(fold_mid(scratch, nparts) + blockIdx.x * kFoldChunks, 0, kFoldChunks, stat_op(blockIdx.x), out24 + blockIdx.x);
}
__global__ __launch_bounds__(kFoldBlock) void k_chain_readout_fold1(const ChainArgs* __restrict__ tab, const int64_t nparts) {
  fold_stage1(tab[blockIdx.z].ro.scratch, nparts);
}
__global__ __launch_bounds__(kFoldBlock) void k_chain_readout_fold2(const ChainArgs* __restrict__ tab, const int64_t nparts,
                                                                    const int direct) {
  fold_stage2(tab[blockIdx.z].ro.scratch, nparts, tab[blockIdx.z].ro.out24, direct);
}
__global__ __launch_bounds__(kFoldBlock) void k_chain_readout_fold1_one(double* scratch, const int64_t nparts) {
  fold_stage1(scratch, nparts);
}
__global__ __launch_bounds__(kFoldBlock) void k_chain_readout_fold2_one(double* scratch, double* out24, const int64_t nparts,
                                                                        const int direct) {
  fold_stage2(scratch, nparts, out24, direct);
}

inline int fold_threads(int64_t nparts) { return nparts <= 4096 ? kBlock : kFoldBlock; }

__device__ __forceinline__ void sums_fold1(double* rows, const int64_t ntiles) {
  const int64_t per = (ntiles + kFoldChunks - 1) / kFoldChunks;
  const int64_t lo = (int64_t)blockIdx.y * per, hi = (lo + per < ntiles) ? lo + per : ntiles;
  fold_range(rows + (int64_t)blockIdx.x * ntiles, lo < hi ? lo : hi, hi, RSUM,
             rows + (int64_t)kSumRows * ntiles + blockIdx.x * kFoldChunks + blockIdx.y);
}
__device__ __forceinline__ void sums_fold2(double* rows, const int64_t ntiles, double* out, const int direct) {
  if (direct) fold_range(rows + (int64_t)blockIdx.x * ntiles, 0, ntiles, RSUM, out + blockIdx.x);
  else fold_range(rows + (int64_t)kSumRows * ntiles + blockIdx.x * kFoldChunks, 0, kFoldChunks, RSUM, out + blockIdx.x);
}
__global__ __launch_bounds__(kFoldBlock) void k_chain_sums_fold1(const ChainArgs* __restrict__ tab, const int64_t ntiles) {
  sums_fold1(tab[blockIdx.z].ro.scratch, ntiles);
}
__global__ __launch_bounds__(kFoldBlock) void k_chain_sums_fold2(const ChainArgs* __restrict__ tab, const int64_t ntiles,
                                                                 const int direct) {
  sums_fold2(tab[blockIdx.z].ro.scratch, ntiles, tab[blockIdx.z].ro.out24, direct);
  if (blockIdx.x == 0 && threadIdx.x < kReadoutSlots - kSumRows) tab[blockIdx.z].ro.out24[kSumRows + threadIdx.x] = 0.0;
}
__global__ __launch_bounds__(kFoldBlock) void k_chain_sums_fold1_one(double* scratch, const int64_t ntiles) {
  sums_fold1(scratch, ntiles);
}
__global__ __launch_bounds__(kFoldBlock) void k_chain_sums_fold2_one(double* scratch, double* out24, const int64_t ntiles,
                                                                     const int direct) {
  sums_fold2(scratch, ntiles, out24, direct);
  if (blockIdx.x == 0 && threadIdx.x < kReadoutSlots - kSumRows) out24[kSumRows + threadIdx.x] = 0.0;
}
void launch_fold(const bool sums, const ChainArgs* seg, const int n_chains, double* scratch, double* out24,
                 const int64_t nparts, hipStream_t s) {
  const int direct = nparts <= kFoldDirect;
  const unsigned rows = sums ? kSumRows : kReadoutSlots, z = seg ? n_chains : 1;
  if (!direct) {
    if (seg) hipLaunchKernelGGL(sums ? k_chain_sums_fold1 : k_chain_readout_fold1, dim3(rows, kFoldChunks, z), dim3(kFoldBlock),
                                0, s, seg, nparts);
    else hipLaunchKernelGGL(sums ? k_chain_sums_fold1_one : k_chain_readout_fold1_one, dim3(rows, kFoldChunks), dim3(kFoldBlock),
                            0, s, scratch, nparts);
  }
  const dim3 g2(rows, 1, z), b2(direct ? fold_threads(nparts) : kBlock);
  if (seg) hipLaunchKernelGGL(sums ? k_chain_sums_fold2 : k_chain_readout_fold2, g2, b2, 0, s, seg, nparts, direct);
  else hipLaunchKernelGGL(sums ? k_chain_sums_fold2_one : k_chain_readout_fold2_one, g2, b2, 0, s, scratch, out24, nparts, direct);
}

template <bool DEFECT, int WAVES>
__global__ __launch_bounds__(kBlock, WAVES) void k_trace_chain(const ChainArgs, const int64_t n, const int xmap) {
  extern __shared__ __attribute__((aligned(16))) double s_dyn[];
  typedef const ChainArgs __attribute__((address_space(4)))* kernarg_t;
  chain_body<DEFECT>(*(const ChainArgs*)(kernarg_t)__builtin_amdgcn_kernarg_segment_ptr(), 0, n, xmap, s_dyn, blockIdx.x,
                     gridDim.x);
}

template <bool DEFECT, int WAVES>
// ... 2021 lines not shown
  if (e && e[0] == 'x') return 4;
  return shared_in ? 4 : 0;
}
inline bool scene_keep(const int64_t n, const bool xcd_grouped) {
  const char* e = getenv("ART_SCENE_KEEP");
  if (e && (e[0] == '0' || e[0] == '1')) return e[0] == '1';
  return xcd_grouped || n * 57 <= ((int64_t)256 << 20);
}
inline size_t chain_dyn_lds() {
  static const size_t v = [] {
    const char* e = getenv("ART_CHAIN_DYN_LDS");
    const long x = e ? atol(e) : 0;
    return (size_t)(x < 0 ? 0 : (x > 100000 ? 100000 : x));
  }();
  return v;
}

inline int special_waves() {
  const char* e = getenv("ART_CHAIN_SPECIAL");
  if (e && e[0] == '0') return 0;
  const char* w = getenv("ART_CHAIN_SPECIAL_WAVES");
  return (w && atoi(w) == 5) ? 5 : 4;
}
inline bool special_kind(const int kind) { return kind == ART_PLANE || kind == ART_SPHERE || kind == ART_PARABOLA; }
static_assert(ART_PLANE == 0 && ART_SPHERE == 1 && ART_PARABOLA == 2, "special kinds index the dispatchers' tables");

enum class Body { kSpecial, kDefect, kTwoRay, kOneRay };
struct BodyChoice {
  Body body;
  int waves;
  int kind;
};
BodyChoice choose_body(const bool defects, const bool has_mask, const int kind1) {
  if (defects) {
    const int sw = special_kind(kind1) ? special_waves() : 0;
    if (sw) return {Body::kSpecial, sw, kind1};
    return {Body::kDefect, 4, ART_KIND_DYN};
  }
  if (chain_rpl(has_mask) == 2) return {Body::kTwoRay, 4, ART_KIND_DYN};
  return {Body::kOneRay, chain_waves() == 6 ? 6 : 5, ART_KIND_DYN};
}

void launch_chain_body(const BodyChoice& c, const ChainArgs& a, const int64_t n, const int tiles, const int xm,
                       const size_t zern_lds, hipStream_t s) {
  typedef void (*K)(const ChainArgs, const int64_t, const int);
  const K special[2][3] = {{k_trace_chain1<ART_PLANE, 4>, k_trace_chain1<ART_SPHERE, 4>, k_trace_chain1<ART_PARABOLA, 4>},
                           {k_trace_chain1<ART_PLANE, 5>, k_trace_chain1<ART_SPHERE, 5>, k_trace_chain1<ART_PARABOLA, 5>}};
  const K k = (c.body == Body::kSpecial) ? special[c.waves - 4][c.kind]
              : (c.body == Body::kDefect) ? k_trace_chain<true, 4>
              : (c.body == Body::kTwoRay) ? k_trace_chain2<false, 4>
              : (c.waves == 6) ? k_trace_chain<false, 6> : k_trace_chain<false, 5>;
  const bool loop = kDefectLoop && c.body == Body::kDefect;
  const size_t lds = (c.body == Body::kSpecial) ? 0 : (c.body == Body::kDefect ? zern_lds : chain_dyn_lds());
  hipLaunchKernelGGL(k, dim3(loop ? grid_for(n) : tiles), dim3(kBlock), lds, s, a, n, loop ? 0 : xm);
}
void launch_scene_body(const BodyChoice& c, const dim3 g, const ChainArgs* seg, const int64_t first, const int64_t n,
                       const int xarg, const int shape, hipStream_t s) {
  typedef void (*K)(const ChainArgs*, const int64_t, const int64_t, const int, const int);
  const K special[2][3] = {{k_trace_scene1<ART_PLANE, 4>, k_trace_scene1<ART_SPHERE, 4>, k_trace_scene1<ART_PARABOLA, 4>},
                           {k_trace_scene1<ART_PLANE, 5>, k_trace_scene1<ART_SPHERE, 5>, k_trace_scene1<ART_PARABOLA, 5>}};
  const K k = (c.body == Body::kSpecial) ? special[c.waves - 4][c.kind]
              : (c.body == Body::kDefect) ? k_trace_scene<true, 4>
              : (c.body == Body::kTwoRay) ? k_trace_scene2<false, 4>
              : (c.waves == 6) ? k_trace_scene<false, 6> : k_trace_scene<false, 5>;
  hipLaunchKernelGGL(k, g, dim3(kBlock), 0, s, seg, first, n, xarg, shape);
}

}

extern "C" {

int art_abi_version(void) { return ART_ABI_VERSION; }

const char* art_last_error(void) { return g_err; }

int art_device_count(void) {
  int n = 0;
  hipError_t e = hipGetDeviceCount(&n);
  if (e != hipSuccess) {
    (void)hipGetLastError();
    return fail_hip(e, "hipGetDeviceCount");
  }
  int good = 0;
  for (int i = 0; i < n; ++i) {
    hipDeviceProp_t p;
    if (hipGetDeviceProperties(&p, i) == hipSuccess && strncmp(p.gcnArchName, "gfx950", 6) == 0) ++good;
  }
  return good;
}

int art_trace_element(const ArtElementDesc* e, const ArtBundleView* in, const ArtBundleView* out, int64_t n,
                      void* stream) {
  int rc = check_elem(e);
  if (rc) return rc;
  if (e->flags & ART_FLAG_GRATING) return fail(ART_ERR_UNSUPPORTED, kGratingRefusal);
  if (n < 0) return fail(ART_ERR_BAD_ARG, "negative ray count");
  if (n == 0) return ART_OK;
  if (!view_ok(in) || !view_ok(out)) return fail(ART_ERR_BAD_ARG, "bundle view has a NULL array");
  hipStream_t s = (hipStream_t)stream;
  ArtElementDesc ec = *e;
  art::prepare_element(ec);
  per_launch(n, [&](const int64_t off, const int64_t m) {
    const ArtBundleView vi = view_at(*in, off), vo = view_at(*out, off);
    if (ec.flags & ART_FLAG_ZERN_RECURRENCE) {
      ElemArg ea;
      ea.e[0] = ec;
      hipLaunchKernelGGL(k_trace_element_zrec, dim3(grid_stream(m)), dim3(kBlock), 0, s, ea, vi, vo, m);
      return ART_OK;
    }
    switch (ec.kind) {
      case ART_PLANE: launch_element<ART_PLANE>(ec, vi, vo, m, s); break;
      case ART_SPHERE: launch_element<ART_SPHERE>(ec, vi, vo, m, s); break;
      case ART_PARABOLA: launch_element<ART_PARABOLA>(ec, vi, vo, m, s); break;
      case ART_TORUS: launch_element<ART_TORUS>(ec, vi, vo, m, s); break;
      case ART_ELLIPSOID: launch_element<ART_ELLIPSOID>(ec, vi, vo, m, s); break;
      case ART_CYLINDER: launch_element<ART_CYLINDER>(ec, vi, vo, m, s); break;
      default: launch_element<ART_MASK>(ec, vi, vo, m, s); break;
    }
    return ART_OK;
  });
  return launched("art_trace_element launch");
}

int art_trace_grating(const ArtElementDesc* e, const ArtGratingDesc* g, const double* wavelengths_host,
                      const ArtBundleView* outs_host, const ArtBundleView* in, int64_t n, void* stream) {
  int rc = check_elem(e);
  if (rc) return rc;
  if (e->kind == ART_MASK) return fail(ART_ERR_BAD_ARG, "art_trace_grating: a mask cannot be a grating");
  if (e->n_defects > 0 || e->n_grid > 0) return fail(ART_ERR_BAD_ARG, "art_trace_grating: mirrors with defects are not supported as substrates");
  if (!g || !wavelengths_host || !outs_host) return fail(ART_ERR_BAD_ARG, "art_trace_grating: NULL argument");
  if (!(fabs(g->q[0] * g->q[0] + g->q[1] * g->q[1] - 1.0) <= 1e-12)) return fail(ART_ERR_BAD_ARG, "art_trace_grating: q must be a unit vector");
  if (!(isfinite(g->lines_per_mm) && g->lines_per_mm >= 0.0)) return fail(ART_ERR_BAD_ARG, "art_trace_grating: lines_per_mm must be finite and >= 0");
  if (g->nw < 1 || g->nw > ART_GRATING_MAX_WAVELENGTHS) return fail(ART_ERR_BAD_ARG, "art_trace_grating: nw must be in 1..ART_GRATING_MAX_WAVELENGTHS");
  for (int j = 0; j < g->nw; ++j)
    if (!(isfinite(wavelengths_host[j]) && wavelengths_host[j] > 0.0)) return fail(ART_ERR_BAD_ARG, "art_trace_grating: every wavelength must be finite and > 0");
  if (n < 0) return fail(ART_ERR_BAD_ARG, "negative ray count");
  if (n > kMaxRaysPerLaunchHw) return fail(ART_ERR_UNSUPPORTED, "art_trace_grating: more rays than one launch covers");
  if (n == 0) return ART_OK;
  if (!g->wavelengths || !g->outs) return fail(ART_ERR_BAD_ARG, "art_trace_grating: device arrays of wavelengths / views missing");
  if (!view_ok(in)) return fail(ART_ERR_BAD_ARG, "bundle view has a NULL array");
  for (int j = 0; j < g->nw; ++j) {
    if (!view_ok(&outs_host[j])) return fail(ART_ERR_BAD_ARG, "an output view has a NULL array");
    if (g->nw > 1 && (outs_host[j].ox == in->ox || outs_host[j].alive == in->alive))
      return fail(ART_ERR_BAD_ARG, "art_trace_grating: an output may alias the input only when nw == 1");
  }
  ElemArg ea;
  ea.e[0] = *e;
  art::prepare_element(ea.e[0]);
  hipLaunchKernelGGL(k_trace_grating, dim3(grid_stream(n)), dim3(kBlock), 0, (hipStream_t)stream, ea, *g, *in, n);
  return launched("art_trace_grating launch");
}

static int trace_chain_impl(const ArtElementDesc* elems, int32_t n_elems, const ArtBundleView* in,
                            const ArtBundleView* outs, const ArtChainReadout* ro, int64_t n, void* stream) {
  if (!elems || !outs || n_elems <= 0) return fail(ART_ERR_BAD_ARG, "empty chain");
  if (n < 0) return fail(ART_ERR_BAD_ARG, "negative ray count");
  for (int k = 0; k < n_elems; ++k) {
    int rc = check_elem(&elems[k]);
    if (rc) return rc;
    if (elems[k].flags & ART_FLAG_ZERN_RECURRENCE)
      return fail(ART_ERR_UNSUPPORTED, "an element carries Zernike tables in the recurrence layout: trace it with art_trace_element");
    if (elems[k].flags & ART_FLAG_GRATING) return fail(ART_ERR_UNSUPPORTED, kGratingRefusal);
  }
  hipStream_t s = (hipStream_t)stream;
  if (ro) {
    if (!art::readout_ok(*ro)) return fail(ART_ERR_BAD_ARG, "read-out: scratch/out24 missing, X/Y/opl partially NULL, or outputs / lite with sums");
    if (n > max_rays_per_launch()) return fail(ART_ERR_UNSUPPORTED, "fused read-out: more rays than one launch covers");
#ifdef ART_ZERN_LDS
    return fail(ART_ERR_UNSUPPORTED, "ART_ZERN_LDS comparison build: no fused read-out");
#endif
  }
  if (n == 0) {
    if (ro) {
      launch_fold(ro->sums, nullptr, 1, ro->scratch, ro->out24, 0, s);
      return launched("art_trace_chain_readout launch");
    }
    return ART_OK;
  }
  if (!view_ok(in)) return fail(ART_ERR_BAD_ARG, "input bundle view has a NULL array");
  for (int k = 0; k < n_elems; ++k)
    if (outs[k].alive != nullptr && !view_ok(&outs[k])) return fail(ART_ERR_BAD_ARG, "history view partially NULL");
  if (!view_ok(&outs[n_elems - 1])) return fail(ART_ERR_BAD_ARG, "the last output view is mandatory");
  if (n_elems == 1 && !ro) return art_trace_element(&elems[0], in, &outs[0], n, stream);
  for (int k0 = 0; k0 < n_elems; k0 += kChainMax) {
    const int m = (n_elems - k0 < kChainMax) ? n_elems - k0 : kChainMax;
    if (!view_ok(&outs[k0 + m - 1])) return fail(ART_ERR_BAD_ARG, "chains longer than 8 need a view every 8th element");
  }
  const int rc = per_launch(n, [&](const int64_t off, const int64_t cnt) {
    ArtBundleView cur = view_at(*in, off);
    for (int k0 = 0; k0 < n_elems; k0 += kChainMax) {
      ChainArgs a;
      memset(&a, 0, sizeof(a));
      const int m = (n_elems - k0 < kChainMax) ? n_elems - k0 : kChainMax;
      a.n_elems = m;
      a.in = cur;
      bool has_mask = false;
      for (int k = 0; k < m; ++k) {
        a.e[k] = elems[k0 + k];
        art::prepare_element(a.e[k]);
        a.out[k] = view_at(outs[k0 + k], off);
        if (a.e[k].n_defects > 0 || a.e[k].n_grid > 0) a.flags |= art::kFlagDefects;
        has_mask = has_mask || a.e[k].kind == ART_MASK;
      }
      const bool tail = ro && k0 + m == n_elems;
      if (tail) {
        a.ro = *ro;
        a.flags |= art::kFlagReadout;
      }
      size_t lds = 0;
#ifdef ART_ZERN_LDS
      lds = zern_lds_bytes(a);
      if (lds > 64 * 1024) return fail(ART_ERR_UNSUPPORTED, "ART_ZERN_LDS build: Zernike tables of one fused launch exceed 64 KiB");
#endif
      const BodyChoice c = choose_body((a.flags & art::kFlagDefects) != 0, has_mask,
                                       (!kDefectLoop && m == 1) ? a.e[0].kind : ART_KIND_DYN);
      const int xm = xcd_map();
      const int tiles = grid_stream_mapped(c.body == Body::kTwoRay ? (cnt + 1) / 2 : cnt, xm);
      launch_chain_body(c, a, cnt, tiles, xm, lds, s);
      if (tail) launch_fold(ro->sums, nullptr, 1, ro->scratch, ro->out24, ro->sums ? analysis_tiles(cnt) : tiles, s);
      cur = a.out[m - 1];
    }
    return ART_OK;
  });
  return rc ? rc : launched("art_trace_chain launch");
}

int art_trace_chain(const ArtElementDesc* elems, int32_t n_elems, const ArtBundleView* in, const ArtBundleView* outs,
                    int64_t n, void* stream) {
  return trace_chain_impl(elems, n_elems, in, outs, nullptr, n, stream);
}

int64_t art_chain_readout_scratch_doubles(int64_t n) {
  if (n < 0) n = 0;
  if (n > kMaxRaysPerLaunchHw) n = kMaxRaysPerLaunchHw;
  return (((n + kBlock - 1) / kBlock + 1024) + kFoldChunks) * kReadoutSlots;
}

int art_trace_chain_readout(const ArtElementDesc* elems, int32_t n_elems, const ArtBundleView* in,
                            const ArtBundleView* outs, const ArtChainReadout* readout, int64_t n, void* stream) {
  if (!readout) return fail(ART_ERR_BAD_ARG, "read-out descriptor is NULL");
  return trace_chain_impl(elems, n_elems, in, outs, readout, n, stream);
}

int64_t art_scene_bytes(int32_t n_chains, int32_t n_elems) {
  if (n_chains <= 0 || n_elems <= 0) return 0;
  return art::scene_bytes(n_chains, n_elems);
}

int art_scene_pack(const ArtElementDesc* elems, int32_t n_chains, int32_t n_elems, const ArtBundleView* ins,
                   const ArtBundleView* outs, const ArtChainReadout* readouts, void* image) {
  const char* msg = "";
  const int rc = art::scene_pack(elems, n_chains, n_elems, ins, outs, readouts, image, &msg);
  if (rc < 0) return fail(rc, msg);
  return rc;
}

int art_trace_scene(const void* image_dev, const void* image_host, int64_t n, void* stream) {
  if (!image_dev || !image_host) return fail(ART_ERR_BAD_ARG, "scene image is NULL");
  art::SceneHeader h;
  memcpy(&h, image_host, sizeof(h));
  if (h.magic != art::kSceneMagic) return fail(ART_ERR_BAD_ARG, "host image was not written by art_scene_pack");
  const int32_t n_chains = h.n_chains, n_elems = h.n_elems, flags = h.flags;
  if (n_chains <= 0 || n_chains > 65535 || n_elems <= 0 || h.n_segments != art::scene_segments(n_elems) ||
      (flags & ~(art::kFlagDefects | art::kFlagReadout | art::kFlagMask | art::kFlagSharedIn | art::kFlagSums)))
    return fail(ART_ERR_BAD_ARG, "scene header is corrupt");
  if (n < 0) return fail(ART_ERR_BAD_ARG, "negative ray count");
#ifdef ART_ZERN_LDS
  if (flags & 1) return fail(ART_ERR_UNSUPPORTED, "ART_ZERN_LDS build: scenes with defects go through art_trace_chain");
#endif
  if ((flags & art::kFlagReadout) && n > max_rays_per_launch())
    return fail(ART_ERR_UNSUPPORTED, "fused read-out: more rays than one launch covers");
  hipStream_t s = (hipStream_t)stream;
  const ChainArgs* tab = art::scene_table(image_dev);
  const int S = art::scene_segments(n_elems);
  const bool sums = (flags & art::kFlagSums) != 0, tails = sums || (flags & art::kFlagReadout);
  if (n == 0) {
    if (tails) launch_fold(sums, tab + (int64_t)(S - 1) * n_chains, n_chains, nullptr, nullptr, 0, s);
    return ART_OK;
  }
  int kind1 = ART_KIND_DYN;
  if ((flags & 1) && n_elems == 1) {
    const ChainArgs* ht = art::scene_table(image_host);
    kind1 = ht[0].e[0].kind;
    for (int c = 1; c < n_chains; ++c) kind1 = (ht[c].e[0].kind == kind1) ? kind1 : ART_KIND_DYN;
  }
  const BodyChoice c = choose_body((flags & 1) != 0, (flags & art::kFlagMask) != 0 ||
                                   ((flags & art::kFlagSharedIn) != 0 && n_chains > 1 && S == 1), kind1);
  per_launch(n, [&](const int64_t off, const int64_t cnt) {
    const int xm = xcd_map();
    const int tiles = grid_stream_mapped(c.body == Body::kTwoRay ? (cnt + 1) / 2 : cnt, xm);
    for (int sg = 0; sg < S; ++sg) {
      const ChainArgs* seg = tab + (int64_t)sg * n_chains;
      int tr = scene_order((flags & art::kFlagSharedIn) != 0 && sg == 0 && n_chains > 1);
      const int tiles8 = (tiles + 7) / 8 * 8;
      if (tr == 4 && (int64_t)tiles8 * n_chains >= ((int64_t)1 << 24)) tr = 1;
      if (tr == 1 && tiles > 65535) tr = 0;
      if (tr && scene_keep(cnt, (tr & 4) != 0)) tr |= 2;
      if (tr & 4) tr |= n_chains << 8;
      const dim3 g = (tr & 4) ? dim3((unsigned)(tiles8 * n_chains)) : ((tr & 1) ? dim3(n_chains, tiles) : dim3(tiles, n_chains));
      const int xarg = (tr & 4) ? tiles : xm;
      launch_scene_body(c, g, seg, off, cnt, xarg, tr, s);
      if (tails && sg == S - 1) launch_fold(sums, seg, n_chains, nullptr, nullptr, sums ? analysis_tiles(cnt) : tiles, s);
    }
    return ART_OK;
  });
  return launched("art_trace_scene launch");
}

int art_pack_rays(const double* points, const double* vectors, const double* path0, int64_t n, const ArtBundleView* out,
                  void* stream) {
  if (n < 0) return fail(ART_ERR_BAD_ARG, "negative ray count");
  if (n == 0) return ART_OK;
  if (!points || !vectors || !view_ok(out)) return fail(ART_ERR_BAD_ARG, "NULL argument");
  hipLaunchKernelGGL(k_pack_rays, dim3(grid_for(n)), dim3(kBlock), 0, (hipStream_t)stream, points, vectors, path0, n,
                     *out);
  return launched("art_pack_rays launch");
}

int art_transform_bundle(const double M[9], const double T[3], int32_t rotate_points, const ArtBundleView* in,
                         const ArtBundleView* out, int64_t n, void* stream) {
  if (!M || !T) return fail(ART_ERR_BAD_ARG, "NULL matrix or translation");
  if (n < 0) return fail(ART_ERR_BAD_ARG, "negative ray count");
  if (n == 0) return ART_OK;
  if (!view_ok(in) || !view_ok(out)) return fail(ART_ERR_BAD_ARG, "bundle view has a NULL array");
  ArtDetectorDesc mt;
  memset(&mt, 0, sizeof(mt));
  memcpy(mt.rot, M, 9 * sizeof(double));
  memcpy(mt.centre, T, 3 * sizeof(double));
  hipLaunchKernelGGL(k_transform, dim3(grid_stream(n)), dim3(kBlock), 0, (hipStream_t)stream, mt, (int)rotate_points, *in,
                     *out, n);
  return launched("art_transform_bundle launch");
}

int art_detector(const ArtDetectorDesc* d, const ArtBundleView* b, int64_t n, double* p3x, double* p3y, double* p3z,
                 double* X, double* Y, double* opl, void* stream) {
  if (!d) return fail(ART_ERR_BAD_ARG, "detector descriptor is NULL");
  if (n == 0) return ART_OK;
  if (!view_ok(b)) return fail(ART_ERR_BAD_ARG, "bundle view has a NULL array");
  if ((p3x || p3y || p3z) && !(p3x && p3y && p3z)) return fail(ART_ERR_BAD_ARG, "p3x/p3y/p3z must be all set or all NULL");
  if ((X || Y) && !(X && Y)) return fail(ART_ERR_BAD_ARG, "X/Y must be both set or both NULL");
  if (n < 0) return fail(ART_ERR_BAD_ARG, "negative ray count");
  if (n == 0) return ART_OK;
  hipLaunchKernelGGL(k_detector, dim3(grid_for(n)), dim3(kBlock), 0, (hipStream_t)stream, *d, *b, n, p3x, p3y, p3z, X,
                     Y, opl);
  return launched("art_detector launch");
}

int art_detector_readout(const ArtDetectorDesc* d, const ArtBundleView* b, const double* w, int64_t n, double cx,
                         double cy, double co, double* p3x, double* p3y, double* p3z, double* X, double* Y,
                         double* opl, double* scratch, double* out24, void* stream) {
  if (!d || !scratch || !out24) return fail(ART_ERR_BAD_ARG, "descriptor/scratch/out24 must not be NULL");
  if ((p3x || p3y || p3z) && !(p3x && p3y && p3z)) return fail(ART_ERR_BAD_ARG, "p3x/p3y/p3z must be all set or all NULL");
  if ((X || Y) && !(X && Y)) return fail(ART_ERR_BAD_ARG, "X/Y must be both set or both NULL");
  if (n < 0) return fail(ART_ERR_BAD_ARG, "negative ray count");
  hipStream_t s = (hipStream_t)stream;
  if (n == 0) {
    return fold_partials<kReadoutSlots, stat_op>(scratch, 0, out24, s, "art_detector_readout launch");
  }
  if (!view_ok(b)) return fail(ART_ERR_BAD_ARG, "bundle view has a NULL array");
  const int64_t chunk = max_rays_per_launch();
  const int64_t launches = (n + chunk - 1) / chunk;
  if (launches > 8) return fail(ART_ERR_UNSUPPORTED, "more than 2^31 rays in one read-out");
  int nb_total = 0;
  per_launch(n, [&](const int64_t off, const int64_t m) {
    const int64_t want = ((m + 1) / 2 + kBlock - 1) / kBlock;
    const int64_t cap = readout_block_cap(launches);
    const int nb = (int)(want < 1 ? 1 : (want > cap ? cap : want));
    const ArtBundleView v = view_at(*b, off);
    hipLaunchKernelGGL(k_detector_readout, dim3(nb), dim3(kBlock), 0, s, *d, v, w ? w + off : nullptr, m, cx, cy, co,
                       p3x ? p3x + off : nullptr, p3y ? p3y + off : nullptr, p3z ? p3z + off : nullptr,
                       X ? X + off : nullptr, Y ? Y + off : nullptr, opl ? opl + off : nullptr,
                       scratch + (int64_t)nb_total * kReadoutSlots);
    nb_total += nb;
    return ART_OK;
  });
  return fold_partials<kReadoutSlots, stat_op>(scratch, nb_total, out24, s, "art_detector_readout launch");
}

int art_detector_scan_moments(const ArtDetectorDesc* d, const ArtBundleView* b, const double* w, int64_t n, double co,
                              double span, double* scratch, double* out32, void* stream) {
  if (!d || !scratch || !out32) return fail(ART_ERR_BAD_ARG, "descriptor/scratch/out32 must not be NULL");
  if (n < 0) return fail(ART_ERR_BAD_ARG, "negative ray count");
  hipStream_t s = (hipStream_t)stream;
  if (n == 0) {
    hipError_t e0 = hipMemsetAsync(out32, 0, kScanSlots * sizeof(double), s);
    if (e0 != hipSuccess) return fail_hip(e0, "hipMemsetAsync");
    return ART_OK;
  }
  if (!view_ok(b)) return fail(ART_ERR_BAD_ARG, "bundle view has a NULL array");
  const int nb = red_blocks(n);
  if (w) hipLaunchKernelGGL(k_scan_moments_partial<true>, dim3(nb), dim3(kBlock), 0, s, *d, *b, w, n, co, span, scratch);
  else hipLaunchKernelGGL(k_scan_moments_partial<false>, dim3(nb), dim3(kBlock), 0, s, *d, *b, w, n, co, span, scratch);
  return fold_partials<kScanSlots, sum_op>(scratch, nb, out32, s, "art_detector_scan_moments launch");
}

int art_histogram(const ArtHistogramDesc* h, const ArtBundleView* b, const double* w, int64_t n, int32_t accumulate,
                  int64_t* counts, int64_t* wsums, int64_t* totals4, void* stream) {
#pragma clang fp contract(off)
  if (!h) return fail(ART_ERR_BAD_ARG, "histogram descriptor is NULL");
  if (h->source != ART_HIST_DETECTOR && h->source != ART_HIST_FRAME) return fail(ART_ERR_BAD_ARG, "unknown histogram source");
  if (h->ndim < 1 || h->ndim > 3) return fail(ART_ERR_BAD_ARG, "histogram ndim must be 1, 2 or 3");
  HistArg a;
  memset(&a, 0, sizeof(a));
  a.map = h->map;
  a.delay_centre = h->delay_centre;
// ... 890 lines not shown
```

### attosecondraytracing_amd/csrc/art_scene.h

```cpp
#pragma once
#include <stdint.h>
#include <string.h>

#include "art_device.h"

namespace art {

constexpr int kChainMax = 8;

struct ChainArgs {
  ArtElementDesc e[kChainMax];
  ArtBundleView out[kChainMax];
  ArtBundleView in;
  ArtChainReadout ro;
  int32_t n_elems;
  int32_t flags;
};
constexpr int kFlagDefects = 1, kFlagReadout = 2;
constexpr int kFlagMask = 4;
constexpr int kFlagSharedIn = 8;
constexpr int kFlagSums = 16;

inline bool readout_ok(const ArtChainReadout& r) {
  const int outs = (r.X != nullptr) + (r.Y != nullptr) + (r.opl != nullptr);
  if (r.sums && (outs != 0 || r.lite)) return false;
  return r.scratch && r.out24 && (outs == 0 || outs == 3);
}

constexpr uint32_t kSceneMagic = 0x41525453u;
struct SceneHeader {
  uint32_t magic;
  int32_t n_chains, n_elems, n_segments, flags;
  int32_t reserved[11];
};
static_assert(sizeof(SceneHeader) == 64, "scene header is 64 bytes");

inline int scene_segments(int n_elems) { return (n_elems + kChainMax - 1) / kChainMax; }
inline int64_t scene_bytes(int n_chains, int n_elems) {
  return (int64_t)sizeof(SceneHeader) + (int64_t)scene_segments(n_elems) * n_chains * (int64_t)sizeof(ChainArgs);
}
inline const ChainArgs* scene_table(const void* image) {
  return reinterpret_cast<const ChainArgs*>(static_cast<const char*>(image) + sizeof(SceneHeader));
}

inline bool scene_view_ok(const ArtBundleView& v) {
  return v.ox && v.oy && v.oz && v.dx && v.dy && v.dz && v.path && v.incidence && v.alive;
}

inline int scene_pack(const ArtElementDesc* elems, int n_chains, int n_elems, const ArtBundleView* ins,
                      const ArtBundleView* outs, const ArtChainReadout* ros, void* image, const char** err) {
  static const char* none = "";
  *err = none;
  if (!elems || !ins || !outs || !image) { *err = "NULL argument"; return ART_ERR_BAD_ARG; }
  if (n_chains <= 0 || n_chains > 65535) { *err = "n_chains must be in 1..65535"; return ART_ERR_BAD_ARG; }
  if (n_elems <= 0) { *err = "empty chain"; return ART_ERR_BAD_ARG; }
  const int S = scene_segments(n_elems);
  SceneHeader h;
  memset(&h, 0, sizeof(h));
  h.magic = kSceneMagic; h.n_chains = n_chains; h.n_elems = n_elems; h.n_segments = S;
  ChainArgs* tab = reinterpret_cast<ChainArgs*>(static_cast<char*>(image) + sizeof(SceneHeader));
  for (int c = 0; c < n_chains; ++c) {
    if (!scene_view_ok(ins[c])) { *err = "input bundle view has a NULL array"; return ART_ERR_BAD_ARG; }
    for (int s = 0; s < S; ++s) {
      ChainArgs& a = tab[(int64_t)s * n_chains + c];
      memset(&a, 0, sizeof(a));
      const int k0 = s * kChainMax;
      const int m = (n_elems - k0 < kChainMax) ? n_elems - k0 : kChainMax;
      a.n_elems = m;
      a.in = (s == 0) ? ins[c] : outs[(int64_t)c * n_elems + k0 - 1];
      for (int k = 0; k < m; ++k) {
        const ArtElementDesc& e = elems[(int64_t)c * n_elems + k0 + k];
        if (e.kind < 0 || e.kind >= ART_NUM_KINDS) { *err = "unknown optic kind"; return ART_ERR_BAD_ARG; }
        if (e.support_kind < 0 || e.support_kind > ART_SUP_RECTRECTHOLE) { *err = "unknown support kind"; return ART_ERR_BAD_ARG; }
        if (e.n_defects < 0 || e.n_defects > ART_MAX_DEFECTS || e.n_grid < 0 || e.n_grid > ART_MAX_DEFECTS) {
          *err = "too many defects on one mirror"; return ART_ERR_UNSUPPORTED;
        }
        if ((e.n_defects > 0 || e.n_grid > 0) && e.kind == ART_MASK) { *err = "a mask cannot carry defects"; return ART_ERR_BAD_ARG; }
        if ((e.n_defects > 0 && !e.zern) || (e.n_grid > 0 && !e.grid)) { *err = "defect count > 0 but its table is NULL"; return ART_ERR_BAD_ARG; }
        if (e.flags & ART_FLAG_ZERN_RECURRENCE) { *err = "an element carries Zernike tables in the recurrence layout: trace it with art_trace_element"; return ART_ERR_UNSUPPORTED; }
        if (e.flags & ART_FLAG_GRATING) { *err = "an element is a grating: trace it with art_trace_grating"; return ART_ERR_UNSUPPORTED; }
        a.e[k] = e;
        prepare_element(a.e[k]);
        if (e.n_defects > 0 || e.n_grid > 0) { a.flags |= kFlagDefects; h.flags |= kFlagDefects; }
        if (e.kind == ART_MASK) h.flags |= kFlagMask;
        const ArtBundleView& o = outs[(int64_t)c * n_elems + k0 + k];
        if (o.alive != nullptr && !scene_view_ok(o)) { *err = "history view partially NULL"; return ART_ERR_BAD_ARG; }
        a.out[k] = o;
      }
      if (ros && s == S - 1) {
        if (!readout_ok(ros[c])) { *err = "read-out: scratch/out24 missing, X/Y/opl partially NULL, or outputs / lite with sums"; return ART_ERR_BAD_ARG; }
        if ((ros[c].sums != 0) != (ros[0].sums != 0)) { *err = "read-outs of one scene must all be read-outs or all sums"; return ART_ERR_BAD_ARG; }
        a.ro = ros[c];
        a.flags |= kFlagReadout;
        h.flags |= kFlagReadout;
        if (ros[c].sums) h.flags |= kFlagSums;
      }
      if (!scene_view_ok(a.out[m - 1])) {
        *err = (s == S - 1) ? "the last output view is mandatory" : "chains longer than 8 need a view every 8th element";
        return ART_ERR_BAD_ARG;
      }
    }
  }
  bool shared = n_chains > 1;
  for (int c = 1; c < n_chains && shared; ++c) shared = memcmp(&ins[c], &ins[0], sizeof(ArtBundleView)) == 0;
  if (shared) h.flags |= kFlagSharedIn;
  memcpy(image, &h, sizeof(h));
  return h.flags;
}

}
```

### attosecondraytracing_amd/graph.py

```python
import torch


class CapturedStep:

    def __init__(self, fn, warmup=3):
        side = torch.cuda.Stream()
        side.wait_stream(torch.cuda.current_stream())
        with torch.cuda.stream(side):
            for _ in range(warmup):
                fn()
        torch.cuda.current_stream().wait_stream(side)
        self.graph = torch.cuda.CUDAGraph()
        with torch.cuda.graph(self.graph):
            self.outputs = fn()

    def replay(self):
        self.graph.replay()
        return self.outputs


class SceneProgram:

    def __init__(self, sources, element_lists, IgnoreDefects=True, post=None, capture=True, detectors=None, history=True,
                 placement_tries=None, readout_lite=False, readout_targets=None, outputs=None):
# ... 39 lines not shown
        if capture and self.be.name == "hip" and not self._stepwise:
            side = torch.cuda.Stream()
            side.wait_stream(torch.cuda.current_stream())
            with torch.cuda.stream(side):
                for _ in range(2):
                    self._launch()
            torch.cuda.current_stream().wait_stream(side)
            self.graph = torch.cuda.CUDAGraph()
            counted = getattr(self.be, "counted_launches", 0)
            with torch.cuda.graph(self.graph):
                self._launch()
            if hasattr(self.be, "counted_launches"):
                self.be.counted_launches = counted

    def _alloc_outputs(self):
        from .bundle import RayBundle
        if self._history:
            return RayBundle.allocate_grid(self.n, self.c, self.m, self.sources, self.be)
        return [[None] * (self.m - 1) + [RayBundle.allocate(self.n, like=s, backend=self.be)] for s in self.sources]

    def _bind(self, outputs):
        self.outputs = outputs
        for ci, outs in enumerate(outputs):
            prev = self.sources[ci]
            for b in outs:
                if b is not None:
                    b.parent = prev
                    prev = b
        self._views_out = [b.view() if b is not None else self._abi.ArtBundleView() for outs in outputs for b in outs]

    def _time_launch(self, reps=2):
        seg = -(-self.m // 8)
        self.be.trace_scene(self.dev, self.host, self.n, segments=seg)
        e0, e1 = torch.cuda.Event(enable_timing=True), torch.cuda.Event(enable_timing=True)
        e0.record()
        for _ in range(reps):
            self.be.trace_scene(self.dev, self.host, self.n, segments=seg)
        e1.record()
        e1.synchronize()
        return e0.elapsed_time(e1) / reps

    @staticmethod
    def _placement_budget(free):
        import os
        cap = float(os.environ.get("ART_PLACEMENT_MEM_CAP", "0.25"))
        return int(cap * free) if cap < 1.0 else int(min(cap, free))

    def _tune_placement(self, element_lists, tries):
        import time
        rows = sum(b is not None for outs in self.outputs for b in outs)
        nbytes = rows * 65 * self.n
        if nbytes < (64 << 20) or tries <= 1:
            return
        free, _ = torch.cuda.mem_get_info()
        budget = self._placement_budget(free)
        asked, tries = tries, max(1, min(tries, 1 + budget // max(nbytes, 1)))
        if tries <= 1:
            self.placement = {"tries": 1, "asked": asked, "chosen": 0, "note": "memory cap: no room for a second candidate"}
            return
        t0 = time.perf_counter()
        while time.perf_counter() - t0 < 0.08:
            self._time_launch(reps=4)
        spacer = max(0, min(8 << 30, (budget - (tries - 1) * nbytes) // (tries - 1)))
        spacer = spacer if spacer >= (256 << 20) else 0
        pool, spacers, oom = [self.outputs], [], False
        for _ in range(tries - 1):
            try:
                if spacer:
                    spacers.append(torch.empty(spacer, dtype=torch.uint8, device=self.be.device))
                pool.append(self._alloc_outputs())
            except torch.OutOfMemoryError:
                oom = True
                break
        del spacers
        times = [float("inf")] * len(pool)
        passes = 0
        for order in (range(len(pool)), reversed(range(len(pool)))):
            for j in order:
                self._bind(pool[j])
                self.update(element_lists)
                times[j] = min(times[j], self._time_launch(reps=3))
            passes += 1
            if max(times) < 1.03 * min(times):
                break
        best = min(range(len(pool)), key=times.__getitem__)
        if times[0] < 1.03 * times[best]:
            best = 0
        self._bind(pool[best])
        self.update(element_lists)
        self.placement = {"tries": len(pool), "asked": asked, "launch_ms": [round(t, 4) for t in times], "chosen": best,
                          "gain_vs_first": round(times[0] / times[best], 4), "passes": passes,
                          "spacer_bytes": spacer, "budget_bytes": budget, "allocation_failed": oom}
        del pool

    def set_detectors(self, detectors):
        if self.readouts is None and getattr(self, "_signature", None) is not None:
            raise ValueError("this SceneProgram was built without detectors")
        self.detectors = list(detectors)
        if self.readouts is None:
            self.readouts = []
            for ci, (d, s, area) in enumerate(zip(self.detectors, self.sources, self._ro_scratch)):
                d._iscomplete()
                kw = {} if (self._ro_targets is None or self._ro_targets[ci] is None) else {"targets": self._ro_targets[ci]}
                self.readouts.append(self.be.new_chain_readout(d._desc(), s.intensity, self.n, scratch=area,
                                                               lite=self._readout_lite, **kw))
        else:
            for d, ro in zip(self.detectors, self.readouts):
                d._iscomplete()
                ro["struct"].det = d._desc()
                ro.pop("stats", None)

    def _structure(self, element_lists, descs):
        return (len(element_lists), len(element_lists[0]), tuple(d.kind for d in descs),
                tuple((d.n_defects > 0 or d.n_grid > 0) for d in descs))

    def matches(self, sources, element_lists, kwargs=None):
        kwargs = kwargs or {}
        if set(kwargs) - {"IgnoreDefects"} or bool(kwargs.get("IgnoreDefects", True)) != self.IgnoreDefects:
            return False
        if len(sources) != self.c or any(a is not b for a, b in zip(sources, self.sources)):
            return False
        if len(element_lists) != self.c or any(len(e) != self.m for e in element_lists):
            return False
        descs = [self._mp.element_descriptor(oe, self.IgnoreDefects, self.be)[0] for els in element_lists for oe in els]
        return (self._structure(element_lists, descs) == self._signature and not any(d.nonfinite for d in descs)
                and any(d.flags & self._mp._STEPWISE_FLAGS for d in descs) == self._stepwise)

    def update(self, element_lists):
        descs, keep = [], []
        for els in element_lists:
            for oe in els:
                d, k = self._mp.element_descriptor(oe, self.IgnoreDefects, self.be)
                if d.nonfinite:
                    raise ValueError("an element has non-finite parameters")
                descs.append(d)
                keep.append(k)
        sig = self._structure(element_lists, descs)
        if self._signature is not None and sig != self._signature:
            raise ValueError("SceneProgram.update: the optics changed (kinds / counts / defects); build a new program")
        self._signature = sig
        stepwise = any(d.flags & self._mp._STEPWISE_FLAGS for d in descs)
        if stepwise and (not self._history or self.readouts is not None):
            raise ValueError("a SceneProgram with a Zernike defect above order 16 or a grating is traced element by element: it needs "
                             "history=True and cannot carry fused read-outs (detectors=None; Detector.readout works)")
        if self._stepwise is not None and stepwise != self._stepwise:
            raise ValueError("SceneProgram.update: the optics changed (a Zernike order crossed 16, or a grating); build a new program")
        self._stepwise = stepwise
        if stepwise:
            self._descs, self._keep = descs, keep
            for outs in self.outputs:
                for b in outs:
                    b.touch()
            return
        if self._uploaded is not None:
            self._uploaded.synchronize()
        self.flags = self.be.scene_pack(descs, self._views_in, self._views_out, self.c, self.m, self.host, self.readouts)
        self._uploaded = self.be.scene_upload(self.host, self.dev)
        self._keep = keep
        for outs in self.outputs:
            for b in outs:
                if b is not None:
                    b.touch()

    def _mark(self):
        for ci, outs in enumerate(self.outputs):
            for b in outs:
                if b is not None:
                    b.touch()
            if self.readouts is not None:
                self.readouts[ci].pop("stats", None)
                self._mp._attach_readout(outs[-1], self.detectors[ci], 0.0, self.readouts[ci])

    def _launch(self):
        if self._stepwise:
            for ci in range(self.c):
                vin, src = self._views_in[ci], self.sources[ci]
                g = src.grooves
                for k in range(self.m):
                    vout = self._views_out[ci * self.m + k]
                    g = self._mp._trace_one(self.be, self._descs[ci * self.m + k], vin, vout, self.n, src.wavelength, g)
                    self.outputs[ci][k].grooves = g
                    vin = vout
        else:
            self.be.trace_scene(self.dev, self.host, self.n, segments=-(-self.m // 8))
        self._mark()
        if self.post is not None:
            self.post_result = self.post(self.outputs)

    def run(self):
        if self.graph is not None:
            self.graph.replay()
            if hasattr(self.be, "note_launches"):
                self.be.note_launches(self.n, -(-self.m // 8))
            self._mark()
        else:
            self._launch()
        return self.outputs
```

### include/art_hip.h

```cpp
#ifndef ART_HIP_H
#define ART_HIP_H

#include <stdint.h>

#ifdef __cplusplus
extern "C" {
#endif

#define ART_ABI_VERSION 14

#define ART_OK 0
#define ART_ERR_BAD_ARG (-1)
#define ART_ERR_UNSUPPORTED (-2)
#define ART_ERR_HIP (-3)
#define ART_ERR_NO_DEVICE (-4)

enum ArtOpticKind {
  ART_PLANE = 0,
  ART_SPHERE = 1,
  ART_PARABOLA = 2,
  ART_TORUS = 3,
  ART_ELLIPSOID = 4,
  ART_CYLINDER = 5,
  ART_MASK = 6,
  ART_NUM_KINDS = 7
};

enum ArtSupportKind {
  ART_SUP_ROUND = 0,
  ART_SUP_ROUNDHOLE = 1,
  ART_SUP_RECT = 2,
  ART_SUP_RECTHOLE = 3,
  ART_SUP_RECTRECTHOLE = 4
};

#define ART_FLAG_PERTURBED_NORMAL 1u
#define ART_FLAG_ZERN_RECURRENCE 2u
#define ART_FLAG_GRATING 4u

#define ART_ZERN_RECURRENCE_MAX_ORDER 64
#define ART_ZERN_MAX_ORDER 16
#define ART_ZERN_DIM (ART_ZERN_MAX_ORDER + 1)
#define ART_ZERN_STRIDE (2 + 3 * ART_ZERN_DIM * ART_ZERN_DIM)
#define ART_MAX_DEFECTS 16

typedef struct ArtGridDefect {
  const double* h;
  int32_t nx, ny;
  double x0, y0, dx, dy;
} ArtGridDefect;

typedef struct ArtElementDesc {
  int32_t kind;
  int32_t support_kind;
  int32_t n_defects;
  uint32_t flags;
  double fwd[9];
  double bwd[9];
  double pos[3];
  double centre[3];
  double sp[6];
  double mp[4];
  const double* zern;
  const ArtGridDefect* grid;
  int32_t n_grid;
  int32_t reserved;
} ArtElementDesc;

typedef struct ArtBundleView {
  double* ox; double* oy; double* oz;
  double* dx; double* dy; double* dz;
  double* path;
  double* incidence;
  uint8_t* alive;
} ArtBundleView;

typedef struct ArtDetectorDesc {
  double centre[3];
  double normal[3];
  double rot[9];
} ArtDetectorDesc;

int art_abi_version(void);
const char* art_last_error(void);
int art_device_count(void);

int art_trace_element(const ArtElementDesc* e, const ArtBundleView* in, const ArtBundleView* out,
                      int64_t n, void* stream);

#define ART_GRATING_MAX_WAVELENGTHS 1024
typedef struct ArtGratingDesc {
  double q[2];
  double lines_per_mm;
  int32_t order;
  int32_t nw;
  const double* wavelengths;
  const ArtBundleView* outs;
  double* grooves_in;
  double* grooves_out;
} ArtGratingDesc;
int art_trace_grating(const ArtElementDesc* e, const ArtGratingDesc* g, const double* wavelengths_host,
                      const ArtBundleView* outs_host, const ArtBundleView* in, int64_t n, void* stream);

int art_trace_chain(const ArtElementDesc* elems, int32_t n_elems, const ArtBundleView* in,
                    const ArtBundleView* outs, int64_t n, void* stream);

typedef struct ArtChainReadout {
  ArtDetectorDesc det;
  const double* w;
  double cx, cy, co;
  double* X;
  double* Y;
  double* opl;
  double* scratch;
  double* out24;
  int32_t lite;
  int32_t sums;
} ArtChainReadout;
int64_t art_chain_readout_scratch_doubles(int64_t n);
int art_trace_chain_readout(const ArtElementDesc* elems, int32_t n_elems, const ArtBundleView* in,
                            const ArtBundleView* outs, const ArtChainReadout* readout, int64_t n, void* stream);

int64_t art_scene_bytes(int32_t n_chains, int32_t n_elems);
int art_scene_pack(const ArtElementDesc* elems, int32_t n_chains, int32_t n_elems, const ArtBundleView* ins,
                   const ArtBundleView* outs, const ArtChainReadout* readouts, void* image_host);
int art_trace_scene(const void* image_dev, const void* image_host, int64_t n, void* stream);

int art_pack_rays(const double* points, const double* vectors, const double* path0, int64_t n,
                  const ArtBundleView* out, void* stream);

int art_transform_bundle(const double M[9], const double T[3], int32_t rotate_points, const ArtBundleView* in,
                         const ArtBundleView* out, int64_t n, void* stream);

int art_detector(const ArtDetectorDesc* d, const ArtBundleView* b, int64_t n,
                 double* p3x, double* p3y, double* p3z, double* X, double* Y, double* opl, void* stream);

int art_detector_readout(const ArtDetectorDesc* d, const ArtBundleView* b, const double* w, int64_t n, double cx,
                         double cy, double co, double* p3x, double* p3y, double* p3z, double* X, double* Y,
                         double* opl, double* scratch, double* out24, void* stream);

int art_detector_scan_moments(const ArtDetectorDesc* d, const ArtBundleView* b, const double* w, int64_t n, double co,
                              double span, double* scratch, double* out33, void* stream);

enum ArtHistSource { ART_HIST_DETECTOR = 0, ART_HIST_FRAME = 1 };
enum ArtHistAxis { ART_HAXIS_X = 0, ART_HAXIS_Y = 1, ART_HAXIS_DELAY = 3 };
#define ART_HIST_MAX_BINS (1 << 24)
typedef struct ArtHistogramDesc {
  int32_t source, ndim;
  int32_t axis[3];
  int32_t bins[3];
  int32_t wshift;
  int32_t reserved;
  double lo[3], hi[3];
  double delay_centre;
  ArtDetectorDesc map;
} ArtHistogramDesc;
int art_histogram(const ArtHistogramDesc* h, const ArtBundleView* b, const double* w, int64_t n, int32_t accumulate,
                  int64_t* counts, int64_t* wsums, int64_t* totals4, void* stream);

#define ART_FOCAL_MAX_PIXELS 2048
#define ART_FOCAL_MAX_PLANES 64
typedef struct ArtFocalDesc {
  ArtDetectorDesc det;
  double k;
  double L_ref;
  double x0, dx;
  double y0, dy;
  int32_t nx, ny;
  int32_t planes;
  int32_t reserved;
  double shift[ART_FOCAL_MAX_PLANES];
} ArtFocalDesc;
int64_t art_focal_scratch_doubles(int32_t nx, int32_t ny, int32_t planes, int64_t n);
int art_focal_field(const ArtFocalDesc* f, const ArtBundleView* b, const double* w, int64_t n, double* scratch,
                    double* field, void* stream);

#define ART_FOCAL_MAX_WAVENUMBERS 1024
typedef struct ArtFocalSpectrumDesc {
  ArtFocalDesc f;
  double dk;
  int32_t nk;
  int32_t reserved;
} ArtFocalSpectrumDesc;
int64_t art_focal_spectrum_scratch_doubles(int32_t nx, int32_t ny, int32_t planes, int32_t nk, int64_t n);
int art_focal_spectrum(const ArtFocalSpectrumDesc* s, const ArtBundleView* b, const double* w, int64_t n,
                       double* scratch, double* field, void* stream);

typedef struct ArtFocalChromaticDesc {
  ArtFocalDesc f;
  double axis[3];
  int32_t nk;
  int32_t reserved;
} ArtFocalChromaticDesc;
int64_t art_focal_chromatic_scratch_doubles(int32_t nx, int32_t ny, int32_t planes, int32_t nk, int64_t n);
int art_focal_chromatic(const ArtFocalChromaticDesc* d, const ArtBundleView* b, const ArtBundleView* src, const double* w,
                        int64_t n, const double* table_dev, const double* table_host, double* scratch, double* field,
                        void* stream);

#define ART_WAVEFRONT_MAX_ORDER 10
#define ART_WAVEFRONT_MAX_COLS 68
#define ART_WAVEFRONT_DOUBLES 2360
typedef struct ArtWavefrontJob {
  ArtDetectorDesc det;
  ArtBundleView b;
  const double* w;
  int64_t n;
  double ref[3];
  double L_ref;
  double pupil[3];
  int32_t order;
  int32_t reserved;
  double* opd;
  double* pupil_x;
  double* pupil_y;
  double* out;
} ArtWavefrontJob;
int64_t art_wavefront_scratch_doubles(const ArtWavefrontJob* jobs_host, int32_t n_jobs);
int art_wavefront(const ArtWavefrontJob* jobs_dev, const ArtWavefrontJob* jobs_host, int32_t n_jobs, double* scratch,
                  void* stream);

#define ART_COATING_MAX_LAYERS 256
#define ART_COATING_MAX_MATERIALS 6
#define ART_POLARISATION_MAX_ELEMS 64
#define ART_POLARISATION_DOUBLES 16
typedef struct ArtCoatingMaterial {
  double n;
  double kappa;
} ArtCoatingMaterial;
typedef struct ArtCoatingLayer {
  double thickness;
  double roughness;
  int32_t material;
  int32_t reserved;
} ArtCoatingLayer;
typedef struct ArtCoating {
  int32_t ideal;
  int32_t n_materials;
  int32_t n_layers;
  int32_t substrate;
  double roughness;
  double reserved;
  ArtCoatingMaterial materials[ART_COATING_MAX_MATERIALS];
  ArtCoatingLayer layers[ART_COATING_MAX_LAYERS];
} ArtCoating;
typedef struct ArtPolarisationJob {
  const ArtBundleView* views;
  int32_t coating[ART_POLARISATION_MAX_ELEMS];
  int32_t n_elems;
  int32_t polarised;
  int64_t n;
  double pol[6];
  double k;
  int32_t has_det;
  int32_t reserved;
  ArtDetectorDesc det;
  const double* w0;
  const double* w;
  double* w_out;
  double* field;
  double* out;
} ArtPolarisationJob;
int64_t art_polarisation_scratch_doubles(const ArtPolarisationJob* jobs_host, int32_t n_jobs);
int art_polarisation(const ArtPolarisationJob* jobs_dev, const ArtPolarisationJob* jobs_host, int32_t n_jobs,
                     const ArtCoating* coatings_dev, const ArtCoating* coatings_host, int32_t n_coatings, double* scratch,
                     void* stream);

#define ART_FOCAL_VECTOR_SCRATCH_DEFAULT ((int64_t)1 << 29)
typedef struct ArtFocalVectorSpectrumDesc {
  ArtFocalSpectrumDesc s;
  const ArtBundleView* views;
  int32_t coating[ART_POLARISATION_MAX_ELEMS];
  int32_t n_elems;
  int32_t n_coatings;
  int64_t n;
  double pol[6];
  const double* w;
  const ArtCoatingMaterial* materials;
  int64_t scratch_bound;
} ArtFocalVectorSpectrumDesc;
// ... 95 lines not shown
```

Measured before the change: 62.75 billion.

## Skip loading source rows that are uniform across all rays in the first chain kernel

Sources now record which of their seven input rows (origin, direction, path) hold the same value for every ray, for example the common origin of a point source or the shared direction of a plane wave. Every write path invalidates that record. When the record is valid, the chain and scene kernels receive a mask and the constant values. They give those rows a zero-size buffer resource and substitute the constants, cutting global-memory reads for the first element. In exchange it adds bookkeeping across bundles and graphs, a host sync to read the values back when a source is created, and a risk of stale uniform state if some write path is missed.

```diff
diff --git a/attosecondraytracing_amd/ModuleProcessing.py b/attosecondraytracing_amd/ModuleProcessing.py
--- a/attosecondraytracing_amd/ModuleProcessing.py
+++ b/attosecondraytracing_amd/ModuleProcessing.py
@@ -138,6 +138,10 @@
     bundle._fused_sums = (bundle.version, None if w is None else (w.data_ptr(), w._version), res)
 
 
+def _uniform_rows(be, src):
+    return src.uniform_rows() if getattr(be, "elides_uniform_rows", False) else None
+
+
 def RayTracingCalculation(source_rays, optical_elements, IgnoreDefects=True, mode=None, history=True, detector=None,
                           path_centre=0.0, readout_lite=False, sums=False):
     if isinstance(history, str):
@@ -193,7 +197,8 @@
             ro = be.new_chain_readout(detector._desc(), src.intensity, n, (0.0, 0.0, path_centre), lite=readout_lite)
         elif sums and detector is None and 0 < n <= be.MAX_FUSED_READOUT_RAYS and hasattr(be, "new_chain_sums"):
             ro = be.new_chain_sums(src.intensity, n)
-        be.trace_chain(descs, src.view(), views, n, readout=ro)
+        u = _uniform_rows(be, src)
+        be.trace_chain(descs, src.view(), views, n, readout=ro, **({} if u is None else {"uniform": u}))
         if ro is not None and ro.get("sums"):
             _attach_sums(outs[-1], ro)
         elif ro is not None:
@@ -409,7 +414,9 @@
     elif sums and detectors is None and n <= be.MAX_FUSED_READOUT_RAYS and hasattr(be, "new_chain_sums"):
         ros = [be.new_chain_sums(s_.intensity, n, scratch=area) for s_, area in zip(sources, be.chain_readout_scratch(n, c))]
     host, dev = be.scene_alloc(c, m, transient=True)
-    be.scene_pack(descs, [s.view() for s in sources], views, c, m, host, ros)
+    us = [_uniform_rows(be, s) for s in sources]
+    be.scene_pack(descs, [s.view() for s in sources], views, c, m, host, ros,
+                  **({} if all(u is None for u in us) else {"uniforms": us}))
     be.scene_upload(host, dev)
     be.trace_scene(dev, host, n, segments=-(-m // 8))
     for ci, outs in enumerate(grid):
diff --git a/attosecondraytracing_amd/ModuleSource.py b/attosecondraytracing_amd/ModuleSource.py
--- a/attosecondraytracing_amd/ModuleSource.py
+++ b/attosecondraytracing_amd/ModuleSource.py
@@ -76,7 +76,9 @@
     else:
         axis = mp.FindCentralRay(B).vector
         B.intensity = B.backend.gaussian_intensity(B.view(), axis, IntensityFraction, B.n_slots)
+    rows = B._uniform_record()
     B.touch()
+    B._adopt_uniform(rows)
     if before[0] != "bundle":
         B.tag_content((before, "gaussian intensity", float(IntensityFraction)))
     return B
diff --git a/attosecondraytracing_amd/_abi.py b/attosecondraytracing_amd/_abi.py
--- a/attosecondraytracing_amd/_abi.py
+++ b/attosecondraytracing_amd/_abi.py
@@ -296,6 +296,12 @@
     "art_scene_pack": (C.c_int, [C.POINTER(ArtElementDesc), C.c_int32, C.c_int32, C.POINTER(ArtBundleView),
                                  C.POINTER(ArtBundleView), C.POINTER(ArtChainReadout), C.c_void_p]),
     "art_trace_scene": (C.c_int, [C.c_void_p, C.c_void_p, C.c_int64, C.c_void_p]),
+    "art_trace_chain_uniform": (C.c_int, [C.POINTER(ArtElementDesc), C.c_int32, C.POINTER(ArtBundleView),
+                                          C.POINTER(ArtBundleView), C.c_uint32, c_double_p, C.c_int64, C.c_void_p]),
+    "art_trace_chain_readout_uniform": (C.c_int, [C.POINTER(ArtElementDesc), C.c_int32, C.POINTER(ArtBundleView),
+                                                  C.POINTER(ArtBundleView), C.POINTER(ArtChainReadout), C.c_uint32,
+                                                  c_double_p, C.c_int64, C.c_void_p]),
+    "art_scene_set_uniform": (C.c_int, [C.c_void_p, C.c_int32, C.c_uint32, c_double_p]),
     "art_pack_rays": (C.c_int, [C.c_void_p, C.c_void_p, C.c_void_p, C.c_int64, C.POINTER(ArtBundleView), C.c_void_p]),
     "art_transform_bundle": (C.c_int, [c_double_p, c_double_p, C.c_int32, C.POINTER(ArtBundleView),
                                        C.POINTER(ArtBundleView), C.c_int64, C.c_void_p]),
@@ -369,10 +375,12 @@
 }
 
 
-def bind(lib, prefix="art_"):
+def bind(lib, prefix="art_", missing_ok=False):
     fns = {}
     for name, (res, args) in PROTOTYPES.items():
         sym = name if prefix == "art_" else prefix + name[len("art_"):]
+        if missing_ok and not hasattr(lib, sym):
+            continue
         f = getattr(lib, sym)
         f.restype = res
         f.argtypes = args
diff --git a/attosecondraytracing_amd/_lib.py b/attosecondraytracing_amd/_lib.py
--- a/attosecondraytracing_amd/_lib.py
+++ b/attosecondraytracing_amd/_lib.py
@@ -11,6 +11,20 @@
 
 _BACKEND = None
 
+UNIFORM_POINT, UNIFORM_PLANE, UNIFORM_EXTENDED = 0b1000111, 0b1111000, 0b1000000
+
+
+def _owner(view):
+    ref = getattr(view, "_owner", None)
+    return None if ref is None else ref()
+
+
+def _written(*views):
+    for v in views:
+        b = _owner(v)
+        if b is not None:
+            b._drop_uniform()
+
 
 class ArtError(RuntimeError):
     pass
@@ -19,14 +33,16 @@
 class HipBackend:
 
     name = "hip"
-
-    def __init__(self, path=LIB_PATH):
+    elide_shared_input = False
+
+    def __init__(self, path=LIB_PATH, diagnostic=False):
         if not os.path.exists(path):
             raise RuntimeError(
                 f"{path} not found: the HIP extension has not been built. Run "
                 "`python -c 'import __graft_entry__ as g; g.build()'` (needs hipcc). There is no CPU fallback.")
         self.lib = C.CDLL(path)
-        self.fn = _abi.bind(self.lib)
+        self.fn = _abi.bind(self.lib, missing_ok=diagnostic)
+        self.elides_uniform_rows = "art_trace_chain_uniform" in self.fn and "art_scene_set_uniform" in self.fn
         v = self.fn["art_abi_version"]()
         if v != _abi.ART_ABI_VERSION:
             raise RuntimeError(f"libart_hip.so ABI version {v} != expected {_abi.ART_ABI_VERSION}: rebuild it")
@@ -100,6 +116,7 @@
         return rc
 
     def trace_element(self, desc, view_in, view_out, n):
+        _written(view_out)
         sp = self.stream_ptr()
         self.check(self._timed(lambda: self.fn["art_trace_element"](C.byref(desc), C.byref(view_in),
                                                                     C.byref(view_out), n, sp)), "art_trace_element")
@@ -107,6 +124,7 @@
     def trace_grating(self, desc, q, lines_per_mm, order, wavelengths, view_in, views_out, n, grooves_in=None,
                       grooves_out=None):
         nw = len(wavelengths)
+        _written(*views_out)
         wl_host = (C.c_double * nw)(*[float(w) for w in wavelengths])
         varr = (_abi.ArtBundleView * nw)(*views_out)
         wl_dev = self.from_numpy(np.array([float(w) for w in wavelengths], dtype=np.float64))
@@ -122,14 +140,24 @@
                                                                     C.byref(view_in), n, sp)), "art_trace_grating")
         return wl_dev, v_dev
 
-    def trace_chain(self, descs, view_in, views_out, n, readout=None):
+    def trace_chain(self, descs, view_in, views_out, n, readout=None, uniform=None):
         m = len(descs)
+        _written(*views_out)
         if m > 1 or readout is not None:
             self.note_launches(n, -(-m // 8))
         darr = (_abi.ArtElementDesc * m)(*descs)
         varr = (_abi.ArtBundleView * m)(*views_out)
         sp = self.stream_ptr()
-        if readout is None:
+        if uniform is not None and uniform[0]:
+            mask, vals = int(uniform[0]), (C.c_double * 7)(*uniform[1])
+            if readout is None:
+                self.check(self._timed(lambda: self.fn["art_trace_chain_uniform"](darr, m, C.byref(view_in), varr, mask,
+                                                                                  vals, n, sp)), "art_trace_chain_uniform")
+            else:
+                ro = readout["struct"]
+                self.check(self._timed(lambda: self.fn["art_trace_chain_readout_uniform"](
+                    darr, m, C.byref(view_in), varr, C.byref(ro), mask, vals, n, sp)), "art_trace_chain_readout_uniform")
+        elif readout is None:
             self.check(self._timed(lambda: self.fn["art_trace_chain"](darr, m, C.byref(view_in), varr, n, sp)),
                        "art_trace_chain")
         else:
@@ -194,7 +222,8 @@
         return (torch.empty(nb, dtype=torch.uint8, pin_memory=True),
                 torch.empty(nb, dtype=torch.uint8, device=self.device))
 
-    def scene_pack(self, descs, views_in, views_out, n_chains, n_elems, host_image, readouts=None):
+    def scene_pack(self, descs, views_in, views_out, n_chains, n_elems, host_image, readouts=None, uniforms=None):
+        _written(*views_out)
         darr = (_abi.ArtElementDesc * (n_chains * n_elems))(*descs)
         iarr = (_abi.ArtBundleView * n_chains)(*views_in)
         oarr = (_abi.ArtBundleView * (n_chains * n_elems))(*views_out)
@@ -202,6 +231,12 @@
         rc = self.fn["art_scene_pack"](darr, n_chains, n_elems, iarr, oarr, rarr, host_image.data_ptr())
         if rc < 0:
             self.check(rc, "art_scene_pack")
+        if uniforms and n_chains > 1 and not self.elide_shared_input and all(bytes(v) == bytes(views_in[0]) for v in views_in[1:]):
+            uniforms = None
+        for c, u in enumerate(uniforms or ()):
+            if u is not None and u[0]:
+                self.check(self.fn["art_scene_set_uniform"](host_image.data_ptr(), c, int(u[0]), (C.c_double * 7)(*u[1])),
+                           "art_scene_set_uniform")
         return rc
 
     def scene_upload(self, host_image, dev_image):
@@ -222,11 +257,13 @@
                    "art_trace_scene")
 
     def pack_rays(self, points, vectors, path0, n, view):
+        _written(view)
         self.check(self.fn["art_pack_rays"](points.data_ptr(), vectors.data_ptr(),
                                             None if path0 is None else path0.data_ptr(), n, C.byref(view),
                                             self.stream_ptr()), "art_pack_rays")
 
     def transform_bundle(self, M, T, rotate_points, view_in, view_out, n):
+        _written(view_out)
         m = (C.c_double * 9)(*[float(v) for v in np.asarray(M).reshape(9)])
         t = (C.c_double * 3)(*[float(v) for v in np.asarray(T).reshape(3)])
         self.check(self.fn["art_transform_bundle"](m, t, int(bool(rotate_points)), C.byref(view_in), C.byref(view_out),
@@ -407,10 +444,18 @@
         return idx[:c], c
 
     def make_source(self, kind, size, rot, S, first, n, n_total, view, step=1):
+        _written(view)
         r = (C.c_double * 9)(*[float(v) for v in np.asarray(rot).reshape(9)])
         s = (C.c_double * 3)(*[float(v) for v in np.asarray(S).reshape(3)])
         self.check(self.fn["art_make_source_strided"](kind, float(size), r, s, first, int(step), n, n_total, C.byref(view),
                                                       self.stream_ptr()), "art_make_source_strided")
+        self._record_uniform(view, UNIFORM_POINT if kind == 0 else UNIFORM_PLANE, n)
+
+    def _record_uniform(self, view, mask, n):
+        b = _owner(view)
+        if b is None or n <= 0:
+            return
+        b._set_uniform(mask, b.data[:7, 0].cpu().tolist())
 
     def exchange_pack(self, stats, X, Y, opl, alive, slots, send):
         k = int(slots.numel())
@@ -571,11 +616,13 @@
         return self.analyse_bundles([j], bundle.n_slots)[0]
 
     def make_extended_source(self, radius, divergence, n_points, per, rot, S, first, n, view):
+        _written(view)
         r = (C.c_double * 9)(*[float(v) for v in np.asarray(rot).reshape(9)])
         s = (C.c_double * 3)(*[float(v) for v in np.asarray(S).reshape(3)])
         self.check(self.fn["art_make_extended_source"](float(radius), float(divergence), int(n_points), int(per), r, s,
                                                        first, n, C.byref(view), self.stream_ptr()),
                    "art_make_extended_source")
+        self._record_uniform(view, UNIFORM_EXTENDED, n)
 
 
 def get_backend():
diff --git a/attosecondraytracing_amd/bundle.py b/attosecondraytracing_amd/bundle.py
--- a/attosecondraytracing_amd/bundle.py
+++ b/attosecondraytracing_amd/bundle.py
@@ -9,9 +9,19 @@
 from .ModuleOpticalRay import Ray
 
 import itertools
+import weakref
 
 ROW_OX, ROW_OY, ROW_OZ, ROW_DX, ROW_DY, ROW_DZ, ROW_PATH, ROW_INC = range(8)
 _SERIAL = itertools.count(1)
+UNIFORM_ROWS = 7
+
+
+class _UniformRecord:
+    __slots__ = ("mask", "values", "data_version", "valid")
+
+    def __init__(self, mask, values, data_version):
+        self.mask, self.values = int(mask), tuple(float(v) for v in values)
+        self.data_version, self.valid = data_version, True
 
 
 class RayBundle:
@@ -33,6 +43,7 @@
         self._fused_readout = None
         self._fused_sums = None
         self._content = None
+        self._uniform = None
 
     @property
     def parent(self):
@@ -100,6 +111,7 @@
         self._fused_readout = None
         self._fused_sums = None
         self._content = None
+        self._uniform = None
         self._serial = next(_SERIAL)
 
     @staticmethod
@@ -190,7 +202,40 @@
         v.dx, v.dy, v.dz = p + 3 * stride, p + 4 * stride, p + 5 * stride
         v.path, v.incidence = p + 6 * stride, p + 7 * stride
         v.alive = self.alive.data_ptr()
+        v._owner = weakref.ref(self)
         return v
+
+    def _uniform_record(self):
+        u = getattr(self, "_uniform", None)
+        if u is None:
+            return None
+        rec, version = u
+        if not rec.valid or version != self.version or rec.data_version != self.data._version:
+            return None
+        return rec
+
+    def uniform_rows(self):
+        rec = self._uniform_record()
+        return None if rec is None else (rec.mask, rec.values)
+
+    def _set_uniform(self, mask, values):
+        mask = int(mask)
+        if mask >> UNIFORM_ROWS or mask < 0:
+            raise ValueError("uniform mask has bits beyond the seven rows ox oy oz dx dy dz path")
+        if mask == 0:
+            self._uniform = None
+            return
+        vals = [float(values[j]) if (mask >> j) & 1 else 0.0 for j in range(UNIFORM_ROWS)]
+        self._adopt_uniform(_UniformRecord(mask, vals, self.data._version))
+
+    def _adopt_uniform(self, rec):
+        self._uniform = None if rec is None else (rec, self.version)
+
+    def _drop_uniform(self):
+        u = getattr(self, "_uniform", None)
+        if u is not None:
+            u[0].valid = False
+            self._uniform = None
 
     def phase_path_view(self, wavelength=None):
         v = self.view()
@@ -220,6 +265,7 @@
                         self._backend, cut(self.grooves))
         if self.number is None and lo != 0:
             out.number = torch.arange(lo, hi, dtype=torch.int64, device=self.alive.device)
+        out._adopt_uniform(self._uniform_record())
         return out
 
     def tag_content(self, key):
@@ -363,6 +409,9 @@
         out.path_head = self.path_head
         self._share_grouping(out)
         out.tag_content(self.content_key())
+        rec = self._uniform_record()
+        if rec is not None:
+            out._set_uniform(rec.mask, rec.values)
         return out
 
     def alias(self):
@@ -372,6 +421,7 @@
         out.path_head = self.path_head
         self._share_grouping(out)
         out.tag_content(self.content_key())
+        out._adopt_uniform(self._uniform_record())
         hit = getattr(self, "_sum_w", None)
         if hit is not None and hit[0] == self.version:
             out._sum_w = (out.version, hit[1])
diff --git a/attosecondraytracing_amd/csrc/art_kernels.hip b/attosecondraytracing_amd/csrc/art_kernels.hip
--- a/attosecondraytracing_amd/csrc/art_kernels.hip
+++ b/attosecondraytracing_amd/csrc/art_kernels.hip
@@ -579,6 +579,28 @@
 using art::ChainArgs;
 using art::kChainMax;
 
+__device__ __forceinline__ BundleRsrc make_rsrc_in(const ChainArgs& a, const int64_t n, const int64_t first) {
+  const unsigned u = a.in_uniform, b8 = (unsigned)(n * 8);
+  const ArtBundleView& v = a.in;
+  BundleRsrc r;
+  r.ox = rsrc_of(v.ox + first, (u & 1u) ? 0u : b8); r.oy = rsrc_of(v.oy + first, (u & 2u) ? 0u : b8);
+  r.oz = rsrc_of(v.oz + first, (u & 4u) ? 0u : b8); r.dx = rsrc_of(v.dx + first, (u & 8u) ? 0u : b8);
+  r.dy = rsrc_of(v.dy + first, (u & 16u) ? 0u : b8); r.dz = rsrc_of(v.dz + first, (u & 32u) ? 0u : b8);
+  r.path = rsrc_of(v.path + first, (u & 64u) ? 0u : b8);
+  r.inc = rsrc_of(v.incidence + first, b8);
+  r.alive = rsrc_of(v.alive + first, (unsigned)n);
+  return r;
+}
+template <int J>
+__device__ __forceinline__ double in_pick(const ChainArgs& a, const double loaded) {
+  return ((a.in_uniform >> J) & 1u) ? a.in_value[J] : loaded;
+}
+__device__ __forceinline__ void in_pick_ray(const ChainArgs& a, art::Ray& r) {
+  r.ox = in_pick<0>(a, r.ox); r.oy = in_pick<1>(a, r.oy); r.oz = in_pick<2>(a, r.oz);
+  r.dx = in_pick<3>(a, r.dx); r.dy = in_pick<4>(a, r.dy); r.dz = in_pick<5>(a, r.dz);
+  r.path = in_pick<6>(a, r.path);
+}
+
 #ifndef ART_STORE_DIRECT
 __device__ __forceinline__ void store_tile_lds4(const ArtBundleView& v, const int64_t n, const int64_t first,
                                                 const int64_t tile0, const unsigned t, const art::Ray& r, const bool ok,
@@ -656,7 +678,7 @@
 #endif
   __shared__ double s_part[kBlock / 64][kReadoutSlots];
   const int64_t tile = tile_of(bx, nbx, xmap);
-  const BundleRsrc bi = make_rsrc(a.in, n, first);
+  const BundleRsrc bi = make_rsrc_in(a, n, first);
   const int64_t stride = (int64_t)nbx * kBlock;
   int64_t i0 = tile * kBlock + threadIdx.x;
   do {
@@ -669,6 +691,7 @@
     uint8_t al;
     if (keep_in) load_slot_keep(bi, i, r, al);
     else load_slot(bi, i, r, al);
+    in_pick_ray(a, r);
     s_w[lane] = ld_f64(rsrc_of(const_cast<double*>(a.ro.w) + first,
                                       ((a.flags & art::kFlagReadout) && a.ro.w && !a.ro.lite) ? (unsigned)(n * 8) : 0u),
                        (unsigned)i * 8u);
@@ -742,7 +765,7 @@
   __shared__ __attribute__((aligned(16))) double s_red[(kBlock / 64) * 8 * kTileStride];
   __shared__ double s_part[kBlock / 64][kReadoutSlots];
   const int64_t tile = tile_of(bx, nbx, xmap);
-  const BundleRsrc bi = make_rsrc(a.in, n, first);
+  const BundleRsrc bi = make_rsrc_in(a, n, first);
   unsigned pair = (unsigned)(tile * kBlock + threadIdx.x);
   asm volatile("" : "+v"(pair));
   const unsigned lane = pair & (kBlock - 1);
@@ -770,6 +793,8 @@
     r[0].ox = ox.a; r[0].oy = oy.a; r[0].oz = oz.a; r[0].dx = dx.a; r[0].dy = dy.a; r[0].dz = dz.a; r[0].path = pa.a;
     r[1].ox = ox.b; r[1].oy = oy.b; r[1].oz = oz.b; r[1].dx = dx.b; r[1].dy = dy.b; r[1].dz = dz.b; r[1].path = pa.b;
     r[0].inc = 0.0; r[1].inc = 0.0;
+    in_pick_ray(a, r[0]);
+    in_pick_ray(a, r[1]);
   }
   int k = 0;
   do {
@@ -3097,8 +3122,11 @@
 }
 
 static int trace_chain_impl(const ArtElementDesc* elems, int32_t n_elems, const ArtBundleView* in,
-                            const ArtBundleView* outs, const ArtChainReadout* ro, int64_t n, void* stream) {
+                            const ArtBundleView* outs, const ArtChainReadout* ro, int64_t n, void* stream,
+                            const uint32_t uniform_mask = 0, const double* uniform_values = nullptr) {
   if (!elems || !outs || n_elems <= 0) return fail(ART_ERR_BAD_ARG, "empty chain");
+  if (uniform_mask >> art::kInRows) return fail(ART_ERR_BAD_ARG, "uniform mask has bits beyond the seven input rows");
+  if (uniform_mask && !uniform_values) return fail(ART_ERR_BAD_ARG, "uniform values missing");
   if (n < 0) return fail(ART_ERR_BAD_ARG, "negative ray count");
   for (int k = 0; k < n_elems; ++k) {
     int rc = check_elem(&elems[k]);
@@ -3139,6 +3167,10 @@
       const int m = (n_elems - k0 < kChainMax) ? n_elems - k0 : kChainMax;
       a.n_elems = m;
       a.in = cur;
+      if (k0 == 0 && uniform_mask) {
+        a.in_uniform = uniform_mask;
+        for (int j = 0; j < art::kInRows; ++j) a.in_value[j] = ((uniform_mask >> j) & 1u) ? uniform_values[j] : 0.0;
+      }
       bool has_mask = false;
       for (int k = 0; k < m; ++k) {
         a.e[k] = elems[k0 + k];
@@ -3175,6 +3207,18 @@
   return trace_chain_impl(elems, n_elems, in, outs, nullptr, n, stream);
 }
 
+int art_trace_chain_uniform(const ArtElementDesc* elems, int32_t n_elems, const ArtBundleView* in, const ArtBundleView* outs,
+                            uint32_t uniform_mask, const double* uniform_values, int64_t n, void* stream) {
+  return trace_chain_impl(elems, n_elems, in, outs, nullptr, n, stream, uniform_mask, uniform_values);
+}
+
+int art_trace_chain_readout_uniform(const ArtElementDesc* elems, int32_t n_elems, const ArtBundleView* in,
+                                    const ArtBundleView* outs, const ArtChainReadout* readout, uint32_t uniform_mask,
+                                    const double* uniform_values, int64_t n, void* stream) {
+  if (!readout) return fail(ART_ERR_BAD_ARG, "read-out descriptor is NULL");
+  return trace_chain_impl(elems, n_elems, in, outs, readout, n, stream, uniform_mask, uniform_values);
+}
+
 int64_t art_chain_readout_scratch_doubles(int64_t n) {
   if (n < 0) n = 0;
   if (n > kMaxRaysPerLaunchHw) n = kMaxRaysPerLaunchHw;
@@ -3196,6 +3240,13 @@
                    const ArtBundleView* outs, const ArtChainReadout* readouts, void* image) {
   const char* msg = "";
   const int rc = art::scene_pack(elems, n_chains, n_elems, ins, outs, readouts, image, &msg);
+  if (rc < 0) return fail(rc, msg);
+  return rc;
+}
+
+int art_scene_set_uniform(void* image, int32_t chain, uint32_t uniform_mask, const double* uniform_values) {
+  const char* msg = "";
+  const int rc = art::scene_set_uniform(image, chain, uniform_mask, uniform_values, &msg);
   if (rc < 0) return fail(rc, msg);
   return rc;
 }
diff --git a/attosecondraytracing_amd/csrc/art_scene.h b/attosecondraytracing_amd/csrc/art_scene.h
--- a/attosecondraytracing_amd/csrc/art_scene.h
+++ b/attosecondraytracing_amd/csrc/art_scene.h
@@ -15,7 +15,12 @@
   ArtChainReadout ro;
   int32_t n_elems;
   int32_t flags;
+  uint32_t in_uniform;
+  uint32_t reserved_;
+  double in_value[7];
 };
+static_assert(sizeof(ChainArgs) + 16 <= 4096, "ChainArgs no longer fits the kernel-argument segment");
+constexpr int kInRows = 7;
 constexpr int kFlagDefects = 1, kFlagReadout = 2;
 constexpr int kFlagMask = 4;
 constexpr int kFlagSharedIn = 8;
@@ -108,4 +113,20 @@
   return h.flags;
 }
 
+inline int scene_set_uniform(void* image, int chain, uint32_t mask, const double* values, const char** err) {
+  static const char* none = "";
+  *err = none;
+  if (!image) { *err = "scene image is NULL"; return ART_ERR_BAD_ARG; }
+  SceneHeader h;
+  memcpy(&h, image, sizeof(h));
+  if (h.magic != kSceneMagic) { *err = "image was not written by art_scene_pack"; return ART_ERR_BAD_ARG; }
+  if (chain < 0 || chain >= h.n_chains) { *err = "chain index out of range"; return ART_ERR_BAD_ARG; }
+  if (mask >> kInRows) { *err = "uniform mask has bits beyond the seven input rows"; return ART_ERR_BAD_ARG; }
+  if (mask && !values) { *err = "uniform values missing"; return ART_ERR_BAD_ARG; }
+  ChainArgs& a = reinterpret_cast<ChainArgs*>(static_cast<char*>(image) + sizeof(SceneHeader))[chain];
+  a.in_uniform = mask;
+  for (int j = 0; j < kInRows; ++j) a.in_value[j] = ((mask >> j) & 1u) ? values[j] : 0.0;
+  return 0;
 }
+
+}
diff --git a/attosecondraytracing_amd/graph.py b/attosecondraytracing_amd/graph.py
--- a/attosecondraytracing_amd/graph.py
+++ b/attosecondraytracing_amd/graph.py
@@ -215,15 +215,32 @@
                 for b in outs:
                     b.touch()
             return
-        if self._uploaded is not None:
-            self._uploaded.synchronize()
-        self.flags = self.be.scene_pack(descs, self._views_in, self._views_out, self.c, self.m, self.host, self.readouts)
-        self._uploaded = self.be.scene_upload(self.host, self.dev)
+        self._packed_descs = descs
+        self._pack()
         self._keep = keep
         for outs in self.outputs:
             for b in outs:
                 if b is not None:
                     b.touch()
+
+    def _pack(self):
+        if self._uploaded is not None:
+            self._uploaded.synchronize()
+        elide = getattr(self.be, "elides_uniform_rows", False)
+        self._uniform_records = [s._uniform_record() if elide else None for s in self.sources]
+        kw = {}
+        if any(r is not None for r in self._uniform_records):
+            kw["uniforms"] = [None if r is None else (r.mask, r.values) for r in self._uniform_records]
+        self.flags = self.be.scene_pack(self._packed_descs, self._views_in, self._views_out, self.c, self.m, self.host,
+                                        self.readouts, **kw)
+        self._uploaded = self.be.scene_upload(self.host, self.dev)
+
+    def _check_uniform(self):
+        if self._stepwise:
+            return
+        if any(a is not None or b._uniform is not None for a, b in zip(self._uniform_records, self.sources)):
+            if any(s._uniform_record() is not r for s, r in zip(self.sources, self._uniform_records)):
+                self._pack()
 
     def _mark(self):
         for ci, outs in enumerate(self.outputs):
@@ -251,6 +268,7 @@
             self.post_result = self.post(self.outputs)
 
     def run(self):
+        self._check_uniform()
         if self.graph is not None:
             self.graph.replay()
             if hasattr(self.be, "note_launches"):
diff --git a/include/art_hip.h b/include/art_hip.h
--- a/include/art_hip.h
+++ b/include/art_hip.h
@@ -125,6 +125,14 @@
 int art_scene_pack(const ArtElementDesc* elems, int32_t n_chains, int32_t n_elems, const ArtBundleView* ins,
                    const ArtBundleView* outs, const ArtChainReadout* readouts, void* image_host);
 int art_trace_scene(const void* image_dev, const void* image_host, int64_t n, void* stream);
+
+int art_trace_chain_uniform(const ArtElementDesc* elems, int32_t n_elems, const ArtBundleView* in,
+                            const ArtBundleView* outs, uint32_t uniform_mask, const double* uniform_values, int64_t n,
+                            void* stream);
+int art_trace_chain_readout_uniform(const ArtElementDesc* elems, int32_t n_elems, const ArtBundleView* in,
+                                    const ArtBundleView* outs, const ArtChainReadout* readout, uint32_t uniform_mask,
+                                    const double* uniform_values, int64_t n, void* stream);
+int art_scene_set_uniform(void* image_host, int32_t chain, uint32_t uniform_mask, const double* uniform_values);
 
 int art_pack_rays(const double* points, const double* vectors, const double* path0, int64_t n,
                   const ArtBundleView* out, void* stream);
```

Result: no change. 64.07 billion (median of 6 runs) (+2.1%).
